# haowenz/chromap

Measured on AMD Instinct MI355X. Metric: M paired reads mapped/s (ATAC preset, GRCh38 index), higher is better.
Workload: dtype u64

## Files before the change

### chromap_amd/csrc/cm_api.hip

```cpp
#include <hip/hip_runtime.h>
#include <math.h>
#include <stdio.h>
#include <stdlib.h>
#include <string.h>

#include <string>
#include <vector>

#include "../../include/chromap_amd.h"
#include "cm_barcode_translate.h"
#include "cm_ctx.h"
#include "cm_kernels.h"
#include "cm_classes.h"
#include "cm_summary.h"
#include "cm_coop.h"
#include <chrono>
#include <mutex>
#include "cm_mapq_tables.h"

static thread_local std::string g_last_error;

static bool cm_debug_pool() { static const bool on = getenv("CM_DEBUG_POOL") != nullptr; return on; }
static thread_local std::string t_last_error;
void cm_set_error(cmgpu_ctx *ctx, const std::string &msg) {
// ... 18 lines not shown
    fprintf(stderr, "[alloc] %10.3f MB (had %10.3f) %8.3f ms\n", (double)want / 1e6, (double)had / 1e6,
            std::chrono::duration<double, std::milli>(std::chrono::steady_clock::now() - t0).count());
  if (e != hipSuccess) {
    (void)hipGetLastError();
    want = bytes;
    e = hipMalloc(&p, want);
    if (e != hipSuccess) { p = nullptr; return -1; }
  }
  cap = want;
  return 0;
}
void DevBuf::release() {
  if (p && owned) (void)hipFree(p);
  p = nullptr;
  cap = 0;
}

static int cm_ensure_candidate_arrays(cmgpu_ctx *c, uint64_t n_m) {
  return c->mbuf.ensure((size_t)n_m * 8 + 8) || c->mcnt.ensure((size_t)n_m + 4) || c->fbuf.ensure((size_t)n_m * 8 + 8) ||
         c->fcnt.ensure((size_t)n_m + 4) || c->dpos.ensure((size_t)n_m * 8 + 8) || c->derr.ensure((size_t)n_m * 2 + 4) ||
         c->dsplit.ensure((size_t)n_m * 4 + 4) || c->v_err.ensure((size_t)n_m * 2 + 4) || c->v_end.ensure((size_t)n_m * 2 + 4);
}
extern "C" int cmgpu_set_option(cmgpu_ctx *c, const char *name, int64_t value) {
  if (!c || !name) return CMGPU_EINVAL;
  const std::string n(name);
  if (n == "probe_lookups_per_lane") {
    if (value != 1 && value != 2 && value != 4 && value != 8) { cm_set_error(c, "probe_lookups_per_lane: 1, 2, 4 or 8"); return CMGPU_EINVAL; }
    c->opt.probe_variant = (int)value | (c->opt.probe_variant & 16);
  } else if (n == "probe_pair_prefetch") {
    c->opt.probe_variant = (c->opt.probe_variant & 15) | (value ? 16 : 0);
  } else if (n == "h2d_copy_blocks") {
    if (value < 0 || value > 4096) { cm_set_error(c, "h2d_copy_blocks: 0..4096"); return CMGPU_EINVAL; }
    c->opt.h2d_kernel = (int)value;
  } else if (n == "d2h_copy_blocks") {
    if (value < 0 || value > 4096) { cm_set_error(c, "d2h_copy_blocks: 0..4096"); return CMGPU_EINVAL; }
    c->opt.d2h_kernel = (int)value;
  } else if (n == "mm_chunks") {
    if (value < 1 || value > CM_MM_CHUNKS) { cm_set_error(c, "mm_chunks: 1.." + std::to_string(CM_MM_CHUNKS)); return CMGPU_EINVAL; }
    c->opt.mm_chunks = (int)value;
  } else if (n == "prep_kernel") {
    c->opt.prep_kernel = (int)value;
  } else if (n == "prep_tile_reads") {
    if (value < 8 || value > 128) { cm_set_error(c, "prep_tile_reads: 8..128"); return CMGPU_EINVAL; }
    c->opt.prep_tile_reads = (int)value;
  } else if (n == "heavy_wave_max" || n == "heavy_block_max" || n == "heavy_big_max") {
    c->opt.heavy_max[n == "heavy_wave_max" ? 0 : n == "heavy_block_max" ? 1 : 2] = (int)value;
  } else if (n == "s3b_lane_cap") {
    if (value < 0 || value > 64) { cm_set_error(c, "s3b_lane_cap: 0 (by read length) or 1..64"); return CMGPU_EINVAL; }
    c->opt.s3b_cap = (int)value;
  } else if (n == "exchange_overlap") {
    c->opt.exchange_overlap = value ? 1 : 0;
  } else if (n == "lanes") {
    if (value < 1 || value > 8) { cm_set_error(c, "lanes: 1..8"); return CMGPU_EINVAL; }
    c->opt.lanes = (int)value;
  } else if (n == "first_read_id") {
    if (value < 0 || value > 0xffffffffll) { cm_set_error(c, "first_read_id: 0..2^32-1"); return CMGPU_EINVAL; }
    c->first_read_id = (uint32_t)value;
  } else if (n == "heavy_mid_max") {
    c->opt.heavy_mid = (int)value;
  } else if (n == "heavy_last") {
    c->opt.heavy_last = (int)value;
  } else if (n == "probe_table_shift") {
    if (value < 0 || value > 4) { cm_set_error(c, "probe_table_shift: 0..4"); return CMGPU_EINVAL; }
    return cm_build_fast_table(c, (int)value);
  } else if (n == "long_read_fused") {
    c->opt.long_fused = value ? 1 : 0;
  } else if (n == "sam_format_group") {
    if (value != 8 && value != 16 && value != 64) { cm_set_error(c, "sam_format_group: 8, 16 or 64"); return CMGPU_EINVAL; }
    c->opt.sam_group = (int)value;
  } else if (n == "verify_planes") {
    c->opt.planes = value ? 1 : 0;
  } else if (n == "speculative_sizes") {
    c->opt.spec = value ? 1 : 0;
    if (value < 0) { c->cls_seen = 0; memset(c->cls_age, 0, sizeof(c->cls_age)); }
  } else if (n == "debug_candidate_capacity") {
    if (value > 0 && cm_ensure_candidate_arrays(c, (uint64_t)value)) { cm_set_error(c, "out of device memory (candidates)"); return CMGPU_ENOMEM; }
    c->pred_m_ok = value > 0; c->m_cap = (uint64_t)value; c->pred_n = 0xffffffffu;
  } else if (n == "coop_profile") {
    if (value) { if (c->coop_prof.ensure(64 * 8)) return CMGPU_ENOMEM; CM_HIPCHECK(c, hipMemset(c->coop_prof.p, 0, 64 * 8)); } else c->coop_prof.release();
  } else if (n == "coop_run_table") {
    c->opt.coop_rb = (int)value;
  } else if (n == "coop") {
    c->opt.coop = (int)value;
  } else if (n == "item_limit") {
    c->opt.item_limit = value > 0 ? (uint64_t)value : 0xfffffff0ull;
  } else {
    cm_set_error(c, "unknown option " + n);
    return CMGPU_EINVAL;
  }
  return CMGPU_OK;
}

extern "C" int cmgpu_get_option(const cmgpu_ctx *c, const char *name, int64_t *value) {
  if (!c || !name || !value) return CMGPU_EINVAL;
  const std::string n(name);
  if (n == "probe_lookups_per_lane") *value = c->opt.probe_variant & 15;
  else if (n == "probe_pair_prefetch") *value = (c->opt.probe_variant & 16) ? 1 : 0;
  else if (n == "mm_chunks") *value = c->opt.mm_chunks;
  else if (n == "h2d_copy_blocks") *value = c->opt.h2d_kernel;
  else if (n == "d2h_copy_blocks") *value = c->opt.d2h_kernel;
  else if (n == "prep_kernel") *value = c->opt.prep_kernel;
  else if (n == "prep_tile_reads") *value = c->opt.prep_tile_reads;
  else if (n == "item_limit") *value = (int64_t)c->opt.item_limit;
  else if (n == "lanes") *value = c->opt.lanes;
  else if (n == "coop") *value = c->opt.coop;
  else if (n.rfind("coop_profile_", 0) == 0) {
    const int k = atoi(n.c_str() + 13);
    unsigned long long v = 0;
    if (k < 0 || k > 63 || !c->coop_prof.p || hipMemcpy(&v, (const unsigned long long *)c->coop_prof.p + k, 8, hipMemcpyDeviceToHost) != hipSuccess) return CMGPU_EINVAL;
    *value = (int64_t)v;
  }
  else if (n == "probe_table_buckets") *value = c->fmask ? (int64_t)c->fmask + 1 : (int64_t)c->bmask + 1;
  else return CMGPU_EINVAL;
  return CMGPU_OK;
}

extern "C" const char *cmgpu_last_error(const cmgpu_ctx *ctx) { return ctx ? ctx->err.c_str() : g_last_error.c_str(); }

__global__ void k_repack(const uint32_t *__restrict__ flags, const uint64_t *__restrict__ keys,
                         const uint64_t *__restrict__ vals, uint64_t *__restrict__ bkt, uint32_t i0, uint32_t n) {
  const uint32_t j = blockIdx.x * 256 + threadIdx.x;
  if (j >= n) return;
  const uint32_t i = i0 + j;
  const uint32_t f = (flags[i >> 4] >> ((i & 0xfU) << 1)) & 3u;
  uint64_t k = keys[j], v = vals[j];
  if (f & 2u) { k = CM_EMPTY_KEY; v = 0; }
  else if (f & 1u) { k = CM_DELETED_KEY; v = 0; }
  bkt[2 * (uint64_t)i] = k;
  bkt[2 * (uint64_t)i + 1] = v;
}

__global__ __launch_bounds__(256) void k_rehash(const uint64_t *__restrict__ src, uint64_t n_src, uint64_t *__restrict__ dst, uint32_t mask) {
  const uint64_t i = (uint64_t)blockIdx.x * 256 + threadIdx.x;
  if (i >= n_src) return;
  const uint64_t key = src[2 * i], val = src[2 * i + 1];
  if (key == CM_EMPTY_KEY || key == CM_DELETED_KEY) return;
  uint32_t b = (uint32_t)(key >> 1) & mask, step = 0;
  for (;;) {
    const unsigned long long old = atomicCAS(reinterpret_cast<unsigned long long *>(dst + 2 * (uint64_t)b), (unsigned long long)CM_EMPTY_KEY, (unsigned long long)key);
    if (old == CM_EMPTY_KEY) { dst[2 * (uint64_t)b + 1] = val; return; }
    b = (b + (++step)) & mask;
  }
}
int cm_build_fast_table(cmgpu_ctx *c, int shift) {
  CM_HIPCHECK(c, cm_enter(c));
  CM_HIPCHECK(c, cm_stream_sync(c->stream));
  if (c->shared_children > (int)c->lanes.size()) { cm_set_error(c, "probe_table_shift: set it before cmgpu_create_shared (contexts that share this index view the table)"); return CMGPU_EINVAL; }
  c->bkt_fast.release();
  c->fmask = 0;
  if (shift <= 0) return CMGPU_OK;
  if (!c->bkt.p || !c->bkt.owned) { cm_set_error(c, "probe_table_shift: set it on the context that owns the index"); return CMGPU_EINVAL; }
  const uint64_t nb = (uint64_t)c->bmask + 1;
  uint64_t nf = nb << shift;
  if (nf > (1ull << 32)) nf = 1ull << 32;
  if (nf <= nb) return CMGPU_OK;
  if (c->bkt_fast.ensure((size_t)nf * 16)) { cm_set_error(c, "out of device memory (re-hashed index table)"); return CMGPU_ENOMEM; }
  CM_HIPCHECK(c, hipMemsetAsync(c->bkt_fast.p, 0xff, (size_t)nf * 16, c->stream));
  hipLaunchKernelGGL(k_rehash, dim3((unsigned)((nb + 255) / 256)), dim3(256), 0, c->stream, (const uint64_t *)c->bkt.p, nb, (uint64_t *)c->bkt_fast.p,
                     (uint32_t)(nf - 1));
  CM_HIPCHECK(c, cm_stream_sync(c->stream));
  c->fmask = (uint32_t)(nf - 1);
  return CMGPU_OK;
}

static int build_mapq_tables(cmgpu_ctx *c) {
  std::vector<double> coef;
  std::vector<uint32_t> brk;
  cm_build_len_coef(coef);
  cm_build_nsec_break(brk);
  c->n_break = (int)brk.size();
  if (c->len_coef.ensure(coef.size() * 8) || c->nsec_break.ensure(brk.size() * 4)) return CMGPU_ENOMEM;
  CM_HIPCHECK(c, hipMemcpy(c->len_coef.p, coef.data(), coef.size() * 8, hipMemcpyHostToDevice));
  CM_HIPCHECK(c, hipMemcpy(c->nsec_break.p, brk.data(), brk.size() * 4, hipMemcpyHostToDevice));
  return CMGPU_OK;
}

static void cm_load_device_code(hipStream_t s);
int cm_ctx_init_common(cmgpu_ctx *c, const cmgpu_params *params, int kmer, int window, int device_id) {
  c->device = device_id;
  c->hp = *params;
  if (params->max_num_best_mappings < 1 || params->max_num_best_mappings > CM_MAX_BEST) {
    cm_set_error(c, "max_num_best_mappings must be in [1, " + std::to_string(CM_MAX_BEST) + "]"); return CMGPU_EINVAL;
  }
  if (params->max_num_best_mappings > 1 && params->output_format == 1) {
    cm_set_error(c, "--SAM with more than one best mapping per read is outside this build"); return CMGPU_EINVAL;
  }
  if (kmer < 1 || kmer > 28 || window < 1 || window > CM_MAX_W_HOST) { cm_set_error(c, "unsupported k/w"); return CMGPU_EINVAL; }
  if (params->error_threshold < 1 || params->error_threshold > 15) { cm_set_error(c, "error_threshold must be 1..15"); return CMGPU_EINVAL; }
// ... 434 lines not shown
  }
  CM_HIPCHECK(c, hipMemcpyAsync(c->rb0.p, in->read1_bases, c->bases0, hipMemcpyHostToDevice, c->stream));
  CM_HIPCHECK(c, hipMemcpyAsync(c->rb1.p, in->read2_bases, c->bases1, hipMemcpyHostToDevice, c->stream));
  CM_HIPCHECK(c, hipMemcpyAsync(c->ro0.p, in->read1_offsets, ((size_t)n + 1) * 4, hipMemcpyHostToDevice, c->stream));
  CM_HIPCHECK(c, hipMemcpyAsync(c->ro1.p, in->read2_offsets, ((size_t)n + 1) * 4, hipMemcpyHostToDevice, c->stream));
  const int rc = launch_max_len(c, c->ro0, &c->ro1, n, c->stream);
  if (rc) return rc;
  CM_HIPCHECK(c, cm_stream_sync(c->stream));
  c->max_read_len = *c->h_maxlen ? *c->h_maxlen : 1;
  return CMGPU_OK;
}

extern "C" int cmgpu_swap_resident_batch(cmgpu_ctx *c, int slot) {
  if (!c || slot < 0 || slot >= CM_BATCH_SLOTS) return CMGPU_EINVAL;
  if (c->in_flight) { cm_set_error(c, "a batch is in flight"); return CMGPU_EINVAL; }
  if (c->has_barcodes || c->single) { cm_set_error(c, "only bulk paired-end batches can be parked"); return CMGPU_EINVAL; }
  CM_HIPCHECK(c, cm_enter(c));
  CM_HIPCHECK(c, cm_stream_sync(c->stream));
  CmBatchSlot &sl = c->slots[slot];
  std::swap(c->rb0, sl.rb0); std::swap(c->rb1, sl.rb1); std::swap(c->ro0, sl.ro0); std::swap(c->ro1, sl.ro1);
  std::swap(c->n_pairs, sl.n_pairs); std::swap(c->first_read_id, sl.first_read_id); std::swap(c->max_read_len, sl.max_read_len);
  std::swap(c->bases0, sl.bases0); std::swap(c->bases1, sl.bases1);
  c->n_records = 0;
  return CMGPU_OK;
}


static void cm_ensure_goff(cmgpu_ctx *c) {
  if (c->goff_tried) return;
  c->goff_tried = true;
  std::vector<uint32_t> go(c->n_seq + 1);
  uint64_t acc = 0;
  const bool lens_ok = c->n_seq && c->h_ref_len.size() == c->n_seq;
  for (uint32_t i = 0; lens_ok && i < c->n_seq; ++i) { go[i] = (uint32_t)acc; acc += (uint64_t)c->h_ref_len[i] + CM_GOFF_GAP; if (acc >= 0xffff0000ull) break; }
  if (lens_ok && acc < 0xffff0000ull && !getenv("CM_NO_KEY32")) {
    go[c->n_seq] = (uint32_t)acc;
    if (c->goff.ensure(go.size() * 4) == 0 && hipMemcpy(c->goff.p, go.data(), go.size() * 4, hipMemcpyHostToDevice) != hipSuccess) c->goff.release();
  }
}
static void cm_set_classes(const cmgpu_ctx *c, CmDev &d) {
  CmClassIn in = {};
  for (int q = 0; q < 3; ++q) in.heavy_max[q] = c->opt.heavy_max[q];
  in.heavy_mid = c->opt.heavy_mid; in.s3b_cap = c->opt.s3b_cap;
  in.max_read_len = c->max_read_len; in.n_seq = c->n_seq; in.has_goff = c->goff.p != nullptr;
  in.lane_cap = cm_s3b_lane_cap(c->max_read_len);
  cm_s3b_heavy_classes(in.hv_max, &in.hv_big);
  cm_size_classes(in, d);
}
static void cm_bind_dev(cmgpu_ctx *c, CmDev &d, uint32_t lo, uint32_t hi) {
  d.bkt = (const uint64_t *)(c->fmask ? c->bkt_fast.p : c->bkt.p); d.bmask = c->fmask ? c->fmask : c->bmask; d.occ = (const uint64_t *)c->occ.p; d.n_occ = c->n_occ;
  d.ref = (const uint8_t *)c->ref.p; d.ref_off = (const uint64_t *)c->ref_off.p; d.ref_len = (const uint32_t *)c->ref_len.p;
  d.goff = (const uint32_t *)c->goff.p; d.n_seq = c->n_seq;
  d.ref_pl = c->ref_pl_words && c->opt.planes ? (const CmPlRec *)c->ref_planes.p + CM_PL_LEAD : nullptr; d.ref_pl_words = c->ref_pl_words;
  d.p = c->p; d.p.single = c->single ? 1 : 0;
  d.mq.len_coef = (const double *)c->len_coef.p; d.mq.nsec_break = (const uint32_t *)c->nsec_break.p; d.mq.n_break = c->n_break;
  d.n_pairs = hi - lo; d.first_read_id = c->first_read_id + lo;
  d.rb0 = (const uint8_t *)c->rb0.p; d.rb1 = (const uint8_t *)c->rb1.p;
  d.ro0 = (const uint32_t *)c->ro0.p + lo; d.ro1 = (const uint32_t *)c->ro1.p + lo;
#define PTR(f, T) d.f = (T *)c->f.p;
  PTR(rlen, uint32_t) PTR(mm_cnt, uint32_t)
  PTR(mm_off, uint32_t) PTR(mm_hash, uint64_t) PTR(mm_ps, uint32_t) PTR(pr_val, uint64_t) PTR(pr_kind, uint8_t)
  PTR(hit_tot, uint32_t) PTR(hit_off, uint32_t) PTR(round2, uint8_t) PTR(rep_cnt, uint32_t) PTR(rep_len, uint32_t)
  PTR(hbuf, uint64_t) PTR(hcnt, uint8_t) PTR(n_pos_hit, uint32_t) PTR(ncp, uint32_t) PTR(ncn, uint32_t)
  PTR(aug, uint8_t) PTR(res_neg, int32_t) PTR(res_pos, int32_t) PTR(resc_n, uint32_t) PTR(resc_p, uint32_t)
  PTR(m_tot, uint32_t) PTR(m_off, uint32_t) PTR(mbuf, uint64_t) PTR(mcnt, uint8_t) PTR(mcp, uint32_t) PTR(mcn, uint32_t)
  PTR(force0, uint8_t) PTR(fbuf, uint64_t) PTR(fcnt, uint8_t) PTR(fcp, uint32_t) PTR(fcn, uint32_t) PTR(alive, uint8_t)
  PTR(dpos, uint64_t) PTR(derr, int16_t) PTR(dsplit, uint32_t) PTR(nv, uint32_t) PTR(v_off, uint32_t) PTR(v_err, int16_t) PTR(v_end, int16_t) PTR(ndp, uint32_t) PTR(ndn, uint32_t)
  PTR(min_err, int32_t) PTR(second_err, int32_t) PTR(n_best, int32_t) PTR(n_second, int32_t)
  PTR(pe_min, int32_t) PTR(pe_second, int32_t) PTR(pe_nbest, int32_t) PTR(pe_nsecond, int32_t)
  PTR(pe_first, uint32_t) PTR(pe_i1, uint32_t) PTR(pe_i2, uint32_t) PTR(pe_choice, uint32_t)
  PTR(stats, unsigned long long) PTR(srt_cnt, uint32_t) PTR(srt_list, uint32_t) PTR(hv_cnt, uint32_t) PTR(hv_list, uint32_t) PTR(rs_cnt, uint32_t) PTR(rs_list, uint32_t)
#undef PTR
  d.rec = (uint8_t *)c->rec.p + (size_t)lo * 24 * cm_rec_per_pair(c);
  d.rec_ok = (uint8_t *)c->rec_ok.p + (size_t)lo * cm_rec_per_pair(c);
  d.hv_stride = 2 * (hi - lo) + 1;
  d.perm_reads = c->use_perm ? (const uint32_t *)c->perm_reads.p : nullptr; d.perm_pairs = c->use_perm ? (const uint32_t *)c->perm_pairs.p : nullptr;
  d.coop_slab = (uint8_t *)c->coop_slab.p; d.coop_slab_cap = CM_SLAB_CAP; d.coop_slab_blocks = CM_SLAB_BLOCKS;
  d.cls_mask = c->cls_all || !c->opt.spec ? ~0ull : c->cls_seen;
  d.prof = (unsigned long long *)c->coop_prof.p;
  d.rs_pool = (uint64_t *)c->rs_pool.p; d.rs_pool_cap = c->rs_pool.p ? c->rs_pool_cap : 0u; d.rs_pool_off = (uint32_t *)c->rs_pool_off.p;
  d.abort = (const unsigned long long *)c->stats.p + CM_ST_ABORT;
  d.coop_rb = c->opt.coop_rb > 0 ? (uint32_t)c->opt.coop_rb : 0u;
  d.wq_dynamic = ((uint32_t)c->opt.coop >> 16) & 1u;
  if (c->has_rank) {
    d.rid_rank = (const uint32_t *)c->rid_rank.p;
    d.ref_off = (const uint64_t *)c->ref_off_r.p;
    d.ref_len = (const uint32_t *)c->ref_len_r.p;
  }
  if (c->has_pairs_rank) d.pairs_rank = (const uint32_t *)c->pairs_rank.p;
  if (c->has_barcodes) {
    d.bcb = (const uint8_t *)c->bcb.p; d.bcq = (const uint8_t *)c->bcq.p; d.bco = (const uint32_t *)c->bco.p + lo;
    d.wl = (const uint64_t *)c->wl.p; d.wl_mask = c->wl_mask; d.wl_num_sample = (double)c->wl_num_sample;
    d.pow10_tab = (const double *)c->pow10_tab.p;
    d.bc_key = c->bc_key.p ? (uint64_t *)c->bc_key.p + lo : nullptr; d.bc_ok = c->bc_ok.p ? (uint8_t *)c->bc_ok.p + lo : nullptr;
  }
}
static inline void mark(cmgpu_ctx *c, const char *name) {
  if (c->n_ev < CM_MAX_EVENTS) {
    (void)hipEventRecord(c->ev[c->n_ev], c->stream);
    c->ev_name[c->n_ev] = name;
    ++c->n_ev;
  }
}
static int scan_with_total(cmgpu_ctx *c, const uint32_t *in, uint32_t *out, uint32_t n, unsigned long long *total, bool wait = true) {
  hipStream_t s = c->stream;
  unsigned long long *acc = (unsigned long long *)c->stats.p + CM_ST_TOTAL;
  CM_HIPCHECK(c, hipMemsetAsync(acc, 0, 8, s));
  cm_launch_k_sum_u32(in, n, acc, s);
  cm_scan_u32(in, out, n, (uint32_t *)c->scan_tmp.p, s);
  CM_HIPCHECK(c, hipMemcpyAsync(total, acc, 8, hipMemcpyDeviceToHost, s));
  if (wait) CM_HIPCHECK(c, cm_stream_sync(s));
  return CMGPU_OK;
}
#define CM_RC_SPLIT (-100)
#define CM_RC_AGAIN_ALL_CLASSES (-101)
#define CM_RC_AGAIN_EXACT_SIZES (-102)
struct RangeRun {
  cmgpu_ctx *c;
  uint32_t rlo, rhi, n, n2;
  bool allow_spec;
  uint64_t limit;
  hipStream_t s;
  CmDev d;
  uint32_t n_mm = 0;
  bool s3a_done = false;
  uint32_t n_heavy[CM_HV_LISTS] = {};
  unsigned long long hits_total = 0;
  uint32_t n_hits = 0;
  bool planes = false;
  bool spec = false;
  uint32_t n_m = 0;
  void bind() { cm_bind_dev(c, d, rlo, rhi); }
};
static int stage_begin(RangeRun &r) {
  cmgpu_ctx *c = r.c;
  c->n_ev = 0;
  c->use_perm = false;
  const int rc = ensure_pair_arrays(c, r.n);
  if (rc) return rc;
  CM_HIPCHECK(c, hipMemsetAsync(c->stats.p, 0, CM_ST_N * 8, r.s));
  memset(&r.d, 0, sizeof(r.d));
  cm_ensure_goff(c);
  cm_set_classes(c, r.d);
  r.bind();
  mark(c, "begin");
  if (c->has_barcodes) {
    cm_launch_k_s0b_barcode(r.d, r.n, r.s);
    mark(c, "s0b_barcode");
  }
  return CMGPU_OK;
}
struct MmChunks {
  uint32_t n_chunks;
  uint32_t lo[CM_MM_CHUNKS + 1];
  uint64_t entries[CM_MM_CHUNKS];
  uint32_t part_off[CM_MM_CHUNKS + 1];
};
static uint32_t mm_chunk_count(const RangeRun &r) { return r.n >= (1u << 20) ? (uint32_t)r.c->opt.mm_chunks : (r.n >= (1u << 17) ? 2 : 1); }
static void mm_probe_grids(const cmgpu_ctx *c, MmChunks &k) {
  k.part_off[0] = 0;
  for (uint32_t ch = 0; ch < k.n_chunks; ++ch) k.part_off[ch + 1] = k.part_off[ch] + cm_probe_range_blocks(k.entries[ch], c->opt.probe_variant);
}
template <class Fill>
static int mm_fill_and_probe(RangeRun &r, const MmChunks &k, uint32_t mm_cap, Fill fill) {
  cmgpu_ctx *c = r.c;
  const unsigned long long *marks = (const unsigned long long *)c->mm_marks.p;
// ... 1146 lines not shown
```

### chromap_amd/csrc/cm_ctx.h

```cpp
#ifndef CM_CTX_H_
#define CM_CTX_H_
#include <hip/hip_runtime.h>

#include <string>
#include <thread>
#include <vector>

#include "../../include/chromap_amd.h"
#include "../../include/chromap_amd_debug.h"
#include "cm_types.h"

#define CM_MAX_EVENTS 32
#define CM_MAX_W_HOST 32

struct DevBuf {
  void *p = nullptr;
  size_t cap = 0;
  bool owned = true;
  int ensure(size_t bytes);
  void release();
};

struct CmTmpBuf : private DevBuf {
  using DevBuf::p;
// ... 17 lines not shown
  DevBuf scan_tmp;
  hipStream_t hs = nullptr;
  DevBuf red_tmp;
  DevBuf text2, comp, btab, toks, ntok;
  bool dev_mode = false;
  uint64_t dev_len = 0;
  uint64_t n_bytes = 0;
  uint32_t n_nl = 0, n_raw = 0, n_rec = 0, taken = 0, taken_bases = 0, taken_max_len = 0;
  bool final_chunk = false;
  int n_ranges = 0;
  int rng_start[4] = {0, 0, 0, 0}, rng_end[4] = {-1, -1, -1, -1};
  bool minus = false;
  bool keep_names = false;
  DevBuf nm_len, nm_off, st_nm;
  uint32_t taken_name_bytes = 0;
  bool keep_reads = false;
  DevBuf st_q;
  int layout = 0;
  bool general = false;
  uint32_t fx_seen = 0;
  uint32_t fx_lines = 0, fx_stop = 0;
  DevBuf fx_li, fx_nxt, fx_send, fx_sl, fx_exit, fx_entry, fx_res;
};

struct CmReadMate {
  DevBuf names, name_offs, bases, quals, offs;
  uint64_t name_bytes = 0, base_bytes = 0;
};
struct CmSamStore {
  DevBuf rec, var, var_offs, bc;
  DevBuf vlen, voff, scan_tmp, flags;
  uint64_t n = 0, var_bytes = 0;
  bool has_bc = false, paired = false;
};

struct CmSummary {
  bool on = false;
  DevBuf keys, first, cnt, meta;
  uint32_t cap = 0;
  uint64_t key_bound = 0;
  uint32_t slot0 = ~0u;
};

struct CmExchange {
  int transport = 0;
  int rank = 0, world = 0;
  void *comm = nullptr;
  cmgpu_exchange_transport ext = {};
  std::vector<uint8_t> h_owner;
  DevBuf owner, send, counts , stage;
  unsigned long long *h_matrix = nullptr;
  hipStream_t stream = nullptr;
  hipEvent_t ev_part = nullptr, ev_payload = nullptr;
  bool payload_pending = false;
  uint64_t sent_total = 0, recv_total = 0, steps = 0;
  uint64_t owned_by[64] = {};
};

#define CM_BATCH_SLOTS 8
struct CmBatchSlot {
  DevBuf rb0, rb1, ro0, ro1;
  uint32_t n_pairs = 0, first_read_id = 0, max_read_len = 1;
  size_t bases0 = 0, bases1 = 0;
};

struct CmOptions {
  int long_fused = 1;
  int planes = 1;
  int sam_group = 8;
  int d2h_kernel = 0;
  int h2d_kernel = 0;
  int probe_variant = 1;
  int mm_chunks = CM_MM_CHUNKS;
  int prep_tile_reads = 32;
  int prep_kernel = 0;
  uint64_t item_limit = 0xfffffff0ull;
  int exchange_overlap = 0;
  int s3b_cap = 0;
  int lanes = 1;
  int heavy_mid = 0;
  int heavy_max[3] = {0, 0, 0};
  int heavy_last = 0;
  int spec = 1;
  int coop_rb = 0;
  int coop = 0xff;
};

struct cmgpu_ctx {
  CmOptions opt;
  int device = 0;
  hipStream_t stream = nullptr;
  hipStream_t stream2 = nullptr;
  hipStream_t stream_pack = nullptr;
  hipEvent_t chunk_ev[CM_MM_CHUNKS + 1] = {};
  std::string err;
  cmgpu_params hp;
  CmParams p;
  DevBuf bkt, occ, ref, ref_off, ref_len, len_coef, nsec_break;
  uint32_t bmask = 0, n_occ = 0, n_seq = 0;
  DevBuf bkt_fast, coop_prof;
  uint32_t fmask = 0;
  DevBuf ref_planes, read_planes;
  DevBuf mm_stage;
  uint64_t ref_pl_words = 0;
  int n_break = 0;
  uint64_t ref_bytes = 0;
  std::vector<uint64_t> h_ref_off;
  std::vector<uint32_t> h_ref_len;
  uint32_t n_pairs = 0, first_read_id = 0;
  size_t bases0 = 0, bases1 = 0;
  uint32_t max_read_len = 1;
  DevBuf rb0, rb1, ro0, ro1;
  DevBuf st_rb0, st_rb1, st_ro0, st_ro1, st_bcb, st_bcq, st_bco;
  DevBuf rlen, scratch_a, scratch_b , mm_cnt, mm_off, mm_hash, mm_ps, pr_val, pr_kind;
  DevBuf hit_tot, hit_off, round2, rep_cnt, rep_len, hbuf, hcnt, n_pos_hit, ncp, ncn;
  DevBuf aug, res_neg, res_pos, resc_n, resc_p, m_tot, m_off, mbuf, mcnt, mcp, mcn, force0;
  DevBuf fbuf, fcnt, fcp, fcn, alive, dpos, derr, dsplit, nv, v_off, v_err, v_end, ndp, ndn, min_err, second_err, n_best, n_second;
  DevBuf pe_min, pe_second, pe_nbest, pe_nsecond, pe_first, pe_i1, pe_i2, pe_choice, rec, rec_ok;
  DevBuf scan_tmp, stats, partials;
  DevBuf wl, pow10_tab, bcb, bcq, bco, bc_key, bc_ok, wl_num;
  uint32_t wl_mask = 0, wl_size = 0, bc_len = 0;
  uint64_t wl_num_sample = 0;
  bool skip_barcode_check = false;
  bool has_barcodes = false;
  DevBuf bt_tab, bt_blob;
  uint32_t bt_mask = 0, bt_entries = 0, bt_from = 0;
  uint64_t bt_blob_bytes = 0;
  bool single = false;
  DevBuf store, store_bc, text;
  uint64_t store_n = 0, store_cap = 0, text_bytes = 0, text_lines = 0;
  bool store_has_bc = false;
  bool store_pairs_rec = false;
  CmFqStream fq[3];
  DevBuf nm_blob, nm_offs;
  uint64_t nm_n = 0, nm_bytes = 0, nm_cap_n = 0;
  uint32_t nm_base = 0;
  CmReadMate rd[2];
  uint64_t rd_n = 0;
  uint32_t rd_base = 0;
  bool rd_paired = false;
  CmSamStore ss;
  DevBuf sam_rec, sam_cigar, sam_md, sam_z;
  DevBuf pairs_rank;
  bool has_pairs_rank = false;
  DevBuf rid_rank, ref_off_r, ref_len_r;
  bool has_rank = false;
  DevBuf mm_cursor;
  DevBuf mm_marks;
  DevBuf part_cnt;
  unsigned long long cls_seen = ~0ull;
  uint8_t cls_age[64] = {};
  bool cls_all = false;
  DevBuf rs_pool, rs_pool_off;
  DevBuf goff;
  bool goff_tried = false;
  uint32_t rs_pool_cap = 0;
  uint64_t rs_pool_want = 0;
  DevBuf coop_slab, hv_cnt, hv_list, perm_reads, perm_pairs, hv_tmp, srt_cnt, srt_list, rs_list, rs_cnt;
  bool use_perm = false;
  CmSummary sm;
  CmExchange ex;
  bool batch_exchanged = false;
  CmBatchSlot slots[CM_BATCH_SLOTS];
  hipStream_t stream_h2d = nullptr;
  hipEvent_t ev_h2d[2] = {nullptr, nullptr};
  uint32_t sub_total = 0, sub_count = 0;
// ... 102 lines not shown
```

### chromap_amd/csrc/cm_kernels.hip

```cpp
#include <hip/hip_runtime.h>
#include <stdio.h>
#include <string.h>
#include <cstring>
#include <atomic>
#include <map>
#include <mutex>
#include <utility>
#include <rocprim/rocprim.hpp>

#include "cm_kernels.h"
#include "cm_stages.h"
#include "cm_coop.h"

#define CM_BLOCK 256

#define CM_ITEM_KERNEL(kname, fn, perm)                                      \
  __global__ __launch_bounds__(CM_BLOCK) void kname(CmDev d, uint32_t n) {   \
    if (d.abort && *d.abort) return;                                         \
    const uint32_t i = blockIdx.x * CM_BLOCK + threadIdx.x;                  \
    if (i < n) fn(d, d.perm ? d.perm[i] : i);                                \
  }



// ... 551 lines not shown
    __syncthreads();
    return mx;
  }
  __device__ __forceinline__ uint64_t min64(uint64_t v) { return ~max64(~v); }
  __device__ __forceinline__ uint32_t sum(uint32_t v) { uint32_t tot; (void)scan(v, &tot); return tot; }
};
#define CM_XW_BYTES 256
__host__ __device__ inline size_t cm_coop_group_bytes(uint32_t P, uint32_t MM, uint32_t RB, bool own_oc, bool key32 = false) { return ((cm_coop_mem_bytes(P, MM, RB, own_oc, key32) + 15) & ~(size_t)15) + CM_XW_BYTES; }

template <int G, bool K32>
__global__ __launch_bounds__(G < CM_BLOCK ? CM_BLOCK : G, CM_WPE_S3B) void k_s3b_coop(CmDev d, const uint32_t *__restrict__ list, uint32_t n_list, uint32_t P, uint32_t MM, uint32_t RB,
                                                                      uint32_t *__restrict__ fb_list, uint32_t *__restrict__ fb_cnt, uint32_t use_slab) {
  const uint32_t gpb = blockDim.x / G, grp = threadIdx.x / G;
  const size_t gb = cm_coop_group_bytes(P, MM, RB, false, K32);
  uint8_t *base = cm_lds + (size_t)grp * gb;
  CmCoopMem m = cm_coop_mem_at(base, P, MM, RB, false, K32);
  if (use_slab) cm_coop_slab_at(m, d.coop_slab + (size_t)blockIdx.x * cm_coop_slab_bytes(d.coop_slab_cap), d.coop_slab_cap);
  CmDevGroup<G> g;
  g.t = threadIdx.x % G;
  g.xw = reinterpret_cast<uint32_t *>(base + gb - CM_XW_BYTES);
  for (uint32_t gid = blockIdx.x * gpb + grp; gid < n_list; gid += gridDim.x * gpb) {
    const uint32_t r = list[gid];
    bool done;
    if constexpr (K32) done = cm_coop_s3b_k32(d, r, g, m);
    else done = use_slab ? cm_coop_s3b<true>(d, r, g, m) : cm_coop_s3b<false>(d, r, g, m);
    if (!done && g.t == 0) fb_list[atomicAdd(fb_cnt, 1u)] = r;
    g.sync();
  }
}

__global__ __launch_bounds__(64) void k_s3b_serial(CmDev d, const uint32_t *__restrict__ list, uint32_t n_list, const uint32_t *__restrict__ n_list_dev) {
  if (n_list_dev) n_list = *n_list_dev;
  for (uint32_t i = blockIdx.x * 64 + threadIdx.x; i < n_list; i += gridDim.x * 64) cm_s3b_candidates(d, list[i]);
}

__device__ __forceinline__ void cm_wave_append(uint32_t *__restrict__ list, uint32_t *__restrict__ counter, bool pred, uint32_t value) {
  const unsigned long long m = __ballot(pred);
  if (m == 0) return;
  const uint32_t lane = threadIdx.x & 63u, leader = (uint32_t)(__ffsll((long long)m) - 1);
  uint32_t base = 0;
  if (lane == leader) base = atomicAdd(counter, (uint32_t)__popcll(m));
  base = __shfl(base, (int)leader, 64);
  if (pred) list[base + (uint32_t)__popcll(m & ((1ull << lane) - 1ull))] = value;
}

#define CM_WQ_CHUNK 4u
enum { CM_WQ_S4A_SMALL = 32, CM_WQ_S4A_BIG, CM_WQ_S4B_SMALL, CM_WQ_S4B_BIG, CM_WQ_S5_SORT_SMALL, CM_WQ_S5_SORT_WAVE, CM_WQ_S5_SORT_BLOCK };
struct CmWaveQueue {
  uint32_t *cur;
  uint32_t cnt, j, jend, stride;
  __device__ __forceinline__ CmWaveQueue(uint32_t *cursor, uint32_t n, uint32_t dynamic = 0) : cur(cursor), cnt(n), j(0), jend(0), stride(0) {
    if (!dynamic) {
      const uint32_t wpb = blockDim.x >> 6;
      stride = gridDim.x * wpb;
      j = blockIdx.x * wpb + (threadIdx.x >> 6);
      jend = 0xffffffffu;
    }
  }
  __device__ __forceinline__ bool next(uint32_t *item) {
    if (stride) {
      if (j >= cnt) return false;
      *item = j;
      j += stride;
      return true;
    }
    if (j == jend) {
      uint32_t b = 0;
      if ((threadIdx.x & 63u) == 0) b = atomicAdd(cur, CM_WQ_CHUNK);
      b = __shfl(b, 0, 64);
      if (b >= cnt) return false;
      j = b;
      jend = b + CM_WQ_CHUNK < cnt ? b + CM_WQ_CHUNK : cnt;
    }
    *item = j++;
    return true;
  }
};

#define CM_RS_WAVE 4u
__device__ __forceinline__ bool cm_rescue_is_wave(const CmDev &d, uint32_t r, uint32_t coop) {
  const uint32_t o = r ^ 1u;
  return coop && (d.ncp[o] >= CM_RS_WAVE || d.ncn[o] >= CM_RS_WAVE);
}
__global__ __launch_bounds__(CM_BLOCK) void k_s4a_rescue_count(CmDev d, uint32_t n, uint32_t seg_cap, uint32_t coop) {
  __shared__ uint32_t sh_cnt, sh_base;
  if (threadIdx.x == 0) sh_cnt = 0;
  __syncthreads();
  const uint32_t i0 = blockIdx.x * CM_BLOCK + threadIdx.x;
  const uint32_t i = i0 < n && d.perm_reads ? d.perm_reads[i0] : i0;
  const bool aug0 = i0 < n && cm_s4a_decide(d, i);
  const bool wv = aug0 && cm_rescue_is_wave(d, i, coop);
  cm_wave_append(d.hv_list + (size_t)CM_L_SEARCH_WAVE * d.hv_stride, d.hv_cnt + CM_L_SEARCH_WAVE, wv, i);
  const bool aug = aug0 && !wv;
  const unsigned long long m = __ballot(aug);
  const uint32_t lane = threadIdx.x & 63u;
  uint32_t wbase = 0;
  if (m) {
    const uint32_t leader = (uint32_t)(__ffsll((long long)m) - 1);
    if (lane == leader) wbase = atomicAdd(&sh_cnt, (uint32_t)__popcll(m));
    wbase = __shfl(wbase, (int)leader, 64);
  }
  __syncthreads();
  const uint32_t seg = blockIdx.x % CM_RS_SEGS;
  if (threadIdx.x == 0 && sh_cnt) sh_base = atomicAdd(&d.rs_cnt[seg * 16], sh_cnt);
  __syncthreads();
  if (aug) d.rs_list[(uint64_t)seg * seg_cap + sh_base + wbase + (uint32_t)__popcll(m & ((1ull << lane) - 1ull))] = i;
}
#define CM_RS_HEAVY 8u
#define CM_RS_G 16
#define CM_RS_MAXMM 192
__device__ __forceinline__ bool cm_rescue_is_heavy(const CmDev &d, uint32_t r, uint32_t coop) {
  const uint32_t o = r ^ 1u;
  return (d.ncp[o] >= CM_RS_HEAVY || d.ncn[o] >= CM_RS_HEAVY) && d.mm_cnt[r] <= CM_RS_MAXMM && !cm_rescue_is_wave(d, r, coop);
}
__device__ __forceinline__ void cm_group_best(const uint8_t *mc, uint32_t mn, uint32_t t, int *max_count, int *best_num) {
  int lmax = 0, lnum = 0;
  for (uint32_t i = t; i < mn; i += CM_RS_G) {
    const int c = mc[i];
    if (c > lmax) { lmax = c; lnum = 1; } else if (c == lmax) ++lnum;
  }
  for (int off = CM_RS_G / 2; off > 0; off >>= 1) {
    const int om = __shfl_xor(lmax, off, CM_RS_G), on = __shfl_xor(lnum, off, CM_RS_G);
    if (om > lmax) { lmax = om; lnum = on; } else if (om == lmax) lnum += on;
  }
  *max_count = lmax;
  *best_num = lnum;
}
__device__ __forceinline__ int cm_group_rescue_count(const CmDev &d, uint32_t r, int strand, const uint64_t *mp, const uint8_t *mc, uint32_t mn,
                                                     uint32_t t, uint32_t *cnt, uint32_t *rl) {
  int max_count, best_num;
  cm_group_best(mc, mn, t, &max_count, &best_num);
  *cnt = 0;
  if (cm_rescue_bails(d, max_count, best_num, mn)) {
    if (d.prof && t == 0) atomicAdd(&d.prof[26], 1ull);
    return -max_count;
  }
  const uint32_t b = d.mm_off[r], n = d.mm_cnt[r];
  if (d.prof && t == 0) {
    unsigned long long so = 0;
    for (uint32_t mi = 0; mi < n; ++mi) if (d.pr_kind[b + mi] == CM_PR_MULTI) so += (uint32_t)d.pr_val[b + mi];
    atomicAdd(&d.prof[16], 1ull); atomicAdd(&d.prof[17], (unsigned long long)best_num); atomicAdd(&d.prof[18], (unsigned long long)mn);
    atomicAdd(&d.prof[19], so); atomicAdd(&d.prof[20], (unsigned long long)n);
    atomicAdd(&d.prof[best_num < 4 ? 22 : best_num < 16 ? 23 : best_num < 64 ? 24 : 25], 1ull);
  }
  uint32_t lc = 0;
  for (uint32_t mi = t; mi < n; mi += CM_RS_G)
    lc += cm_rescue_minimizer(d, strand, mp, mc, mn, max_count, d.pr_kind[b + mi], d.pr_val[b + mi], d.mm_ps[b + mi], nullptr, nullptr);
  for (int off = CM_RS_G / 2; off > 0; off >>= 1) lc += __shfl_xor(lc, off, CM_RS_G);
  uint32_t rep_len = 0;
  if (t == 0) {
    uint32_t prev_rep = ~0u;
    for (uint32_t mi = 0; mi < n; ++mi) cm_rescue_rep(d, d.pr_kind[b + mi], d.pr_val[b + mi], d.mm_ps[b + mi], &rep_len, &prev_rep);
  }
  *rl = __shfl(rep_len, 0, CM_RS_G);
  *cnt = lc;
  if (d.prof && t == 0) atomicAdd(&d.prof[21], (unsigned long long)lc);
  return max_count;
}
__global__ __launch_bounds__(64) void k_s4a_rescue_list(CmDev d, uint32_t seg_cap, uint32_t coop) {
  const uint32_t cnt = d.rs_cnt[blockIdx.y * 16];
  const uint32_t *list = d.rs_list + (uint64_t)blockIdx.y * seg_cap;
  const long long t1 = d.prof ? clock64() : 0;
  for (uint32_t j = blockIdx.x * 64 + threadIdx.x; j < cnt; j += gridDim.x * 64) {
    const uint32_t r = list[j];
    if (!cm_rescue_is_heavy(d, r, coop)) cm_s4a_rescue(d, r);
  }
  const long long t2 = d.prof ? clock64() : 0;
  if (d.prof && threadIdx.x == 0) { const unsigned long long dt = (unsigned long long)(t2 - t1); atomicAdd(&d.prof[29], dt); atomicMax(&d.prof[30], dt); }
  const uint32_t t = threadIdx.x % CM_RS_G, grp = threadIdx.x / CM_RS_G, gpb = 64 / CM_RS_G;
  for (uint32_t j = blockIdx.x * gpb + grp; j < cnt; j += gridDim.x * gpb) {
    const uint32_t r = list[j];
    if (!cm_rescue_is_heavy(d, r, coop)) continue;
    const uint32_t o = r ^ 1u;
// ... 106 lines not shown
  __shared__ __attribute__((aligned(16))) uint8_t rmem[SMALL ? CM_RESCUE_MEM_BYTES_S : CM_RESCUE_MEM_BYTES];
  const uint32_t li = SMALL ? CM_L_SEARCH_WAVE : CM_L_SEARCH_WAVE_BIG;
  const uint32_t cnt = d.hv_cnt[li];
  if (blockIdx.x >= cnt) return;
  const uint32_t *list = d.hv_list + (size_t)li * d.hv_stride;
  const CmCoopRescueMem m = SMALL ? cm_coop_rescue_mem_at(rmem, CM_RESCUE_WMAX_S, CM_RESCUE_PAIRS_S) : cm_coop_rescue_mem_at(rmem);
  CmDevGroup<64> g;
  g.t = threadIdx.x;
  g.xw = nullptr;
  cm_coop_rescue_mem_reset(g, m);
  const long long t0 = d.prof ? clock64() : 0;
  CmWaveQueue wq(d.hv_cnt + (SMALL ? CM_WQ_S4A_SMALL : CM_WQ_S4A_BIG), cnt, d.wq_dynamic);
  for (uint32_t j; wq.next(&j);) {
    const uint32_t r = list[j];
    if (SMALL && d.prof) {
      const uint32_t o = r ^ 1u;
      const uint32_t a = cm_coop_rescue_best_num(g, cm_c0_pcnt(d, o), d.ncp[o]), b = cm_coop_rescue_best_num(g, cm_c0_ncnt(d, o), d.ncn[o]);
      const uint32_t mx = a > b ? a : b;
      if (threadIdx.x == 0) atomicAdd(&d.prof[mx < 16 ? 40 : mx < 32 ? 41 : mx < 64 ? 42 : mx < 128 ? 43 : mx < 200 ? 44 : mx < 300 ? 45 : 46], 1ull);
    }
    if (SMALL && !cm_coop_rescue_fits(d, r, g, CM_RESCUE_WMAX_S)) {
      if (threadIdx.x == 0) d.hv_list[(size_t)CM_L_SEARCH_WAVE_BIG * d.hv_stride + atomicAdd(d.hv_cnt + CM_L_SEARCH_WAVE_BIG, 1u)] = r;
      continue;
    }
    const long long ti = d.prof ? clock64() : 0;
    cm_coop_s4a_rescue(d, r, g, m);
    g.sync();
    if (d.prof && threadIdx.x == 0) atomicMax(&d.prof[22], (unsigned long long)(clock64() - ti));
  }
  cm_coop_rescue_mem_flush(d, g, m);
  if (d.prof && threadIdx.x == 0) { const unsigned long long dt = (unsigned long long)(clock64() - t0); atomicAdd(&d.prof[27], dt); atomicMax(&d.prof[28], dt); }
}
template <bool SMALL>
__global__ __launch_bounds__(64) void k_s4b_rescue_wave(CmDev d, uint32_t coop) {
  if (d.abort && *d.abort) return;
  __shared__ __attribute__((aligned(16))) uint8_t rmem[SMALL ? CM_RESCUE_MEM_BYTES_S : CM_RESCUE_MEM_BYTES];
  const uint32_t li = SMALL ? CM_L_SEARCH_WAVE : CM_L_SEARCH_WAVE_BIG;
  const uint32_t cnt = d.hv_cnt[li];
  if (blockIdx.x >= cnt) return;
  const uint32_t *list = d.hv_list + (size_t)li * d.hv_stride;
  const CmCoopRescueMem m = SMALL ? cm_coop_rescue_mem_at(rmem, CM_RESCUE_WMAX_S, CM_RESCUE_PAIRS_S) : cm_coop_rescue_mem_at(rmem);
  CmDevGroup<64> g;
  g.t = threadIdx.x;
  g.xw = nullptr;
  const long long t0 = d.prof ? clock64() : 0;
  CmWaveQueue wq(d.hv_cnt + (SMALL ? CM_WQ_S4B_SMALL : CM_WQ_S4B_BIG), cnt, d.wq_dynamic);
  for (uint32_t j; wq.next(&j);) {
    const uint32_t r = list[j];
    if (d.resc_n[r] + d.resc_p[r] == 0) continue;
    if (SMALL && !cm_coop_rescue_fits(d, r, g, CM_RESCUE_WMAX_S)) continue;
    cm_coop_s4b_fill(d, r, g, m);
    g.sync();
    const uint32_t cls = cm_rescue_coop_class(d, r, coop);
    if (threadIdx.x == 0) {
      if (cls) d.hv_list[(size_t)cls * d.hv_stride + atomicAdd(d.hv_cnt + cls, 1u)] = r;
      else cm_s4b_rescue_merge(d, r, CM_S4B_PREFILLED);
    }
  }
  if (d.prof && threadIdx.x == 0) { const unsigned long long dt = (unsigned long long)(clock64() - t0); atomicAdd(&d.prof[32], dt); atomicMax(&d.prof[33], dt); }
}
template <int G>
__global__ __launch_bounds__(G < CM_BLOCK ? CM_BLOCK : G) void k_s4b_coop(CmDev d, const uint32_t *__restrict__ list, const uint32_t *__restrict__ n_list_dev, uint32_t P, uint32_t RB,
                                                                      uint32_t use_slab) {
  if (d.abort && *d.abort) return;
  const uint32_t gpb = blockDim.x / G, grp = threadIdx.x / G;
  const uint32_t n_list = *n_list_dev;
  const size_t gb = cm_coop_group_bytes(P, 1, RB, true);
  uint8_t *base = cm_lds + (size_t)grp * gb;
  CmCoopMem m = cm_coop_mem_at(base, P, 1, RB, true);
  if (use_slab) cm_coop_slab_at(m, d.coop_slab + (size_t)blockIdx.x * cm_coop_slab_bytes(d.coop_slab_cap), d.coop_slab_cap);
  CmDevGroup<G> g;
  g.t = threadIdx.x % G;
  g.xw = reinterpret_cast<uint32_t *>(base + gb - CM_XW_BYTES);
  for (uint32_t gid = blockIdx.x * gpb + grp; gid < n_list; gid += gridDim.x * gpb) {
    if (use_slab) cm_coop_rescue_merge<true>(d, list[gid], g, m); else cm_coop_rescue_merge<false>(d, list[gid], g, m);
    g.sync();
  }
}
#define CM_S4C_COOP_MIN 48u
#define CM_S5C_COOP_MIN 48u
#define CM_S5C_P_SMALL 512u
#define CM_S5C_P_WAVE 2048u
#define CM_S5C_P_BLOCK 16384u
__device__ __forceinline__ void cm_s4c_queue_sort(const CmDev &d, uint32_t pair, bool live, uint32_t coop) {
  for (uint32_t q = 0; q < 4; ++q) {
    const uint32_t r = 2 * pair + (q >> 1);
    uint32_t cnt = live ? ((q & 1u) ? d.fcn[r] : d.fcp[r]) : 0u;
    if ((coop & 8u) && !d.p.split && live && d.fcp[r] + d.fcn[r] > CM_S5C_COOP_MIN) cnt = 0;
    cm_wave_append(d.srt_list, &d.srt_cnt[0], cnt > CM_SORT_SERIAL_MAX && cnt <= CM_SORT_WAVE_MAX, (r << 1) | (q & 1u));
  }
}
#define CM_S4C_P_SMALL 256u
#define CM_S4C_P_WAVE 1024u
#define CM_S4C_P_BLOCK 4096u
#define CM_S4C_P_BIG 15360u
__global__ __launch_bounds__(CM_BLOCK) void k_s4c_reduce(CmDev d, uint32_t n, uint32_t coop) {
  if (d.abort && *d.abort) return;
  const uint32_t i = blockIdx.x * CM_BLOCK + threadIdx.x;
  const uint32_t pair = i < n ? (d.perm_pairs ? d.perm_pairs[i] : i) : 0u;
  uint32_t cls = 0;
  if (i < n && cm_s4c_pre(d, pair)) {
    const uint32_t r1 = 2 * pair, r2 = r1 + 1;
    uint32_t big = d.mcp[r1] > d.mcn[r1] ? d.mcp[r1] : d.mcn[r1];
    big = d.mcp[r2] > big ? d.mcp[r2] : big;
    big = d.mcn[r2] > big ? d.mcn[r2] : big;
    if ((coop & 4u) && big > CM_S4C_COOP_MIN) cls = big <= CM_S4C_P_SMALL ? CM_L_PF_WAVE : big <= CM_S4C_P_WAVE ? CM_L_PF_BLOCK : big <= CM_S4C_P_BLOCK ? CM_L_PF_BLOCK_BIG : big <= d.s4c_pbig ? CM_L_PF_HUGE : 0u;
    if (!cls) { cm_s4c_filter(d, pair); cm_s4c_post(d, pair); }
  }
  if (coop & 4u) {
    cm_wave_append(d.hv_list + CM_L_PF_BLOCK * (size_t)d.hv_stride, d.hv_cnt + CM_L_PF_BLOCK, cls == CM_L_PF_BLOCK, pair);
    cm_wave_append(d.hv_list + CM_L_PF_WAVE * (size_t)d.hv_stride, d.hv_cnt + CM_L_PF_WAVE, cls == CM_L_PF_WAVE, pair);
    cm_wave_append(d.hv_list + CM_L_PF_BLOCK_BIG * (size_t)d.hv_stride, d.hv_cnt + CM_L_PF_BLOCK_BIG, cls == CM_L_PF_BLOCK_BIG, pair);
    cm_wave_append(d.hv_list + CM_L_PF_HUGE * (size_t)d.hv_stride, d.hv_cnt + CM_L_PF_HUGE, cls == CM_L_PF_HUGE, pair);
  }
  if (!d.perm_pairs) return;
  cm_s4c_queue_sort(d, pair, i < n && !cls && d.alive[pair], coop);
}
template <int G, bool STAGED>
__global__ __launch_bounds__(G < CM_BLOCK ? CM_BLOCK : G) void k_s4c_coop(CmDev d, uint32_t P, uint32_t lid, uint32_t coop) {
  if (d.abort && *d.abort) return;
  const uint32_t gpb = blockDim.x / G, grp = threadIdx.x / G;
  const uint32_t n_list = d.hv_cnt[lid];
  const uint32_t *list = d.hv_list + (size_t)lid * d.hv_stride;
  const size_t gb = ((cm_coop_pair_mem_bytes(P, STAGED) + 15) & ~(size_t)15) + CM_XW_BYTES;
  uint8_t *base = cm_lds + (size_t)grp * gb;
  const CmCoopPairMem m = cm_coop_pair_mem_at(base, P, STAGED);
  CmDevGroup<G> g;
  g.t = threadIdx.x % G;
  g.xw = reinterpret_cast<uint32_t *>(base + gb - CM_XW_BYTES);
  for (uint32_t j0 = blockIdx.x * gpb; j0 < n_list; j0 += gridDim.x * gpb) {
    const uint32_t j = j0 + grp;
    const uint32_t pair = j < n_list ? list[j] : 0u;
    if (j < n_list) cm_coop_s4c<STAGED>(d, pair, g, m);
    g.sync();
    if (d.perm_pairs) {
      const bool live = j < n_list && d.alive[pair];
      for (uint32_t q = 0; q < 4; ++q) {
        const uint32_t r = 2 * pair + (q >> 1);
        uint32_t cnt = live ? ((q & 1u) ? d.fcn[r] : d.fcp[r]) : 0u;
        if ((coop & 8u) && live && d.fcp[r] + d.fcn[r] > CM_S5C_COOP_MIN) cnt = 0;
        if (g.t == 0 && cnt > CM_SORT_SERIAL_MAX && cnt <= CM_SORT_WAVE_MAX) d.srt_list[atomicAdd(&d.srt_cnt[0], 1u)] = (r << 1) | (q & 1u);
      }
    }
  }
}
__global__ __launch_bounds__(CM_BLOCK) void k_s5a_prepare(CmDev d, uint32_t n, uint32_t coop) {
  if (d.abort && *d.abort) return;
  const uint32_t i = blockIdx.x * CM_BLOCK + threadIdx.x;
  const uint32_t r = i < n ? (d.perm_reads ? d.perm_reads[i] : i) : 0u;
  const bool to_wave = i < n && cm_s5a_prepare(d, r, coop ? CM_S5C_COOP_MIN : 0u);
  const bool big = to_wave && (d.fcp[r] > CM_S5C_P_WAVE || d.fcn[r] > CM_S5C_P_WAVE);
  const bool small = to_wave && d.fcp[r] <= CM_S5C_P_SMALL && d.fcn[r] <= CM_S5C_P_SMALL;
  if (coop) {
    cm_wave_append(d.hv_list + (size_t)CM_L_S5_SMALL * d.hv_stride, d.hv_cnt + CM_L_S5_SMALL, small, r);
    cm_wave_append(d.hv_list + (size_t)CM_L_S5_WAVE * d.hv_stride, d.hv_cnt + CM_L_S5_WAVE, to_wave && !big && !small, r);
    cm_wave_append(d.hv_list + (size_t)CM_L_S5_BLOCK * d.hv_stride, d.hv_cnt + CM_L_S5_BLOCK, big, r);
  }
}
__global__ __launch_bounds__(CM_BLOCK) void k_s5c_finalize(CmDev d, uint32_t n, uint32_t coop) {
  if (d.abort && *d.abort) return;
  const uint32_t i = blockIdx.x * CM_BLOCK + threadIdx.x;
  const uint32_t r = i < n ? (d.perm_reads ? d.perm_reads[i] : i) : 0u;
  const uint32_t cmin = coop ? CM_S5C_COOP_MIN : 0u;
  if (i < n) cm_s5c_finalize(d, r, cmin);
  if (!d.perm_reads || d.p.split || d.p.single) return;
  const bool live = i < n && !(cmin && d.nv[r] > cmin) && d.alive[r >> 1];
  const uint32_t a = live ? d.ndp[r] : 0u, b = live ? d.ndn[r] : 0u;
  cm_wave_append(d.srt_list, &d.srt_cnt[0], a > CM_SORT_SERIAL_MAX && a <= CM_SORT_WAVE_MAX, r << 1);
  cm_wave_append(d.srt_list, &d.srt_cnt[0], b > CM_SORT_SERIAL_MAX && b <= CM_SORT_WAVE_MAX, (r << 1) | 1u);
}
#define CM_SORT_NB 64u
#define CM_SORT_STAGE 512u
__global__ __launch_bounds__(CM_BLOCK, 8) void k_s5_sort_coop(CmDev d, uint32_t lid) {
  if (d.abort && *d.abort) return;
  __shared__ uint64_t stage_p[(CM_BLOCK / 64) * CM_SORT_STAGE];
  __shared__ uint8_t stage_c[(CM_BLOCK / 64) * CM_SORT_STAGE];
  const uint32_t grp = threadIdx.x / 64;
  const uint32_t n_list = d.hv_cnt[lid];
  const uint32_t *list = d.hv_list + (size_t)lid * d.hv_stride;
  CmDevGroup<64> g;
  g.t = threadIdx.x % 64;
  g.xw = nullptr;
  const long long t0 = d.prof ? clock64() : 0;
  uint32_t mine = 0;
  CmWaveQueue wq(d.hv_cnt + (lid == CM_L_S5_SMALL ? CM_WQ_S5_SORT_SMALL : lid == CM_L_S5_WAVE ? CM_WQ_S5_SORT_WAVE : CM_WQ_S5_SORT_BLOCK), n_list, d.wq_dynamic);
  for (uint32_t j; wq.next(&j); ++mine)
    cm_coop_s5_sort(d, list[j], g, nullptr, CM_SORT_NB, stage_p + (size_t)grp * CM_SORT_STAGE, stage_c + (size_t)grp * CM_SORT_STAGE, CM_SORT_STAGE);
  if (d.prof && g.t == 0 && mine) {
    const unsigned long long dt = (unsigned long long)(clock64() - t0);
    atomicAdd(&d.prof[38], dt); atomicMax(&d.prof[39], dt); atomicAdd(&d.prof[6], (unsigned long long)mine);
  }
}
#define CM_S5C_SORT_P 1024u
#define CM_S5C_SORT_RB 130u
template <int G>
__global__ __launch_bounds__(CM_BLOCK) void k_s5c_coop(CmDev d, uint32_t P, uint32_t lid) {
  if (d.abort && *d.abort) return;
  const uint32_t gpb = blockDim.x / G, grp = threadIdx.x / G;
  const uint32_t n_list = d.hv_cnt[lid];
  const uint32_t *list = d.hv_list + (size_t)lid * d.hv_stride;
  const size_t b1 = cm_coop_ver_mem_bytes(P), b2 = cm_coop_sort_mem_bytes(CM_S5C_SORT_P, CM_S5C_SORT_RB);
  const size_t gb = (((b1 > b2 ? b1 : b2) + 15) & ~(size_t)15) + CM_XW_BYTES;
  uint8_t *base = cm_lds + (size_t)grp * gb;
  const CmCoopVerMem m = cm_coop_ver_mem_at(base, P);
  const CmCoopSortMem sm = cm_coop_sort_mem_at(base, CM_S5C_SORT_P, CM_S5C_SORT_RB);
  CmDevGroup<G> g;
  g.t = threadIdx.x % G;
  g.xw = reinterpret_cast<uint32_t *>(base + gb - CM_XW_BYTES);
  for (uint32_t j = blockIdx.x * gpb + grp; j < n_list; j += gridDim.x * gpb) {
    cm_coop_s5c(d, list[j], g, m, sm);
    g.sync();
  }
}

template <int MODE>
__global__ __launch_bounds__(CM_BLOCK) void k_sort_lists(CmDev d) {
  if (d.abort && *d.abort) return;
  const uint32_t wv = threadIdx.x >> 6, t = threadIdx.x & 63;
  uint64_t *K = reinterpret_cast<uint64_t *>(cm_lds) + (size_t)wv * CM_SORT_WAVE_MAX;
  uint16_t *V = reinterpret_cast<uint16_t *>(cm_lds + (size_t)(CM_BLOCK / 64) * CM_SORT_WAVE_MAX * 8) + (size_t)wv * CM_SORT_WAVE_MAX;
  const uint32_t n_items = d.srt_cnt[0];
  for (;;) {
    uint32_t item = 0;
    if (t == 0) item = atomicAdd(&d.srt_cnt[1], 1u);
    item = __shfl(item, 0, 64);
    if (item >= n_items) return;
    const uint32_t code = d.srt_list[item], r = code >> 1, strand = code & 1u;
    const uint32_t base = d.m_off[r] + (strand ? d.ncp[r] + d.resc_p[r] : 0);
    const uint32_t n = MODE == 0 ? (strand ? d.fcn[r] : d.fcp[r]) : (strand ? d.ndn[r] : d.ndp[r]);
    uint64_t *gk = (MODE == 0 ? d.fbuf : d.dpos) + base;
    uint32_t P2 = 2;
    while (P2 < n) P2 <<= 1;
    for (uint32_t i = t; i < P2; i += 64) {
      if (i < n) {
        K[i] = gk[i];
        V[i] = MODE == 0 ? (uint16_t)(255u - d.fcnt[base + i]) : (uint16_t)d.derr[base + i];
      } else {
        K[i] = ~0ull;
        V[i] = 0xffffu;
      }
    }
    cm_group_sync<64>();
    for (uint32_t k2 = 2; k2 <= P2; k2 <<= 1) {
      for (uint32_t j = k2 >> 1, lj = 31u - (uint32_t)__clz(k2 >> 1); j > 0; j >>= 1, --lj) {
        for (uint32_t i = t; i < (P2 >> 1); i += 64) {
          const uint32_t a = ((i >> lj) << (lj + 1)) | (i & (j - 1)), c = a + j;
          const uint64_t xa = K[a], xc = K[c];
          const uint16_t va = V[a], vc = V[c];
          const bool gt = MODE == 0 ? (va != vc ? va > vc : xa > xc) : (xa != xc ? xa > xc : va > vc);
          const bool up = (a & k2) == 0;
          if (gt == up && (xa != xc || va != vc)) { K[a] = xc; K[c] = xa; V[a] = vc; V[c] = va; }
        }
        cm_group_sync<64>();
      }
    }
    for (uint32_t i = t; i < n; i += 64) {
      gk[i] = K[i];
      if (MODE == 0) d.fcnt[base + i] = (uint8_t)(255u - V[i]); else d.derr[base + i] = (int16_t)V[i];
    }
    cm_group_sync<64>();
  }
}
void cm_launch_k_sort_lists(const CmDev &d, int mode, hipStream_t s) {
  const size_t lds = (size_t)(CM_BLOCK / 64) * CM_SORT_WAVE_MAX * 10;
  if (mode == 0) hipLaunchKernelGGL(k_sort_lists<0>, dim3(1024), dim3(CM_BLOCK), lds, s, d);
  else hipLaunchKernelGGL(k_sort_lists<1>, dim3(1024), dim3(CM_BLOCK), lds, s, d);
}
__global__ __launch_bounds__(CM_BLOCK) void k_s5b_verify(CmDev d, uint32_t n_reads) {
  if (d.abort && *d.abort) return;
  const uint32_t n_items = d.v_off[n_reads];
  for (uint32_t j = blockIdx.x * CM_BLOCK + threadIdx.x; j < n_items; j += gridDim.x * CM_BLOCK) cm_s5b_verify_item(d, j, n_reads);
}
#define CM_S6A_COOP_MIN 48u
#define CM_S6A_P_SMALL 256u
#define CM_S6A_P_WAVE 1024u
#define CM_S6A_P_BLOCK 8192u
__device__ __forceinline__ uint32_t cm_s6_class(const CmDev &d, uint32_t pair, uint32_t small_list, uint32_t wave_list, uint32_t block_list) {
  const uint32_t r1 = 2 * pair, r2 = r1 + 1;
  uint32_t big2 = d.ndp[r2] > d.ndn[r2] ? d.ndp[r2] : d.ndn[r2], big = big2;
  big = d.ndp[r1] > big ? d.ndp[r1] : big;
  big = d.ndn[r1] > big ? d.ndn[r1] : big;
  if (big <= CM_S6A_COOP_MIN) return 0;
  return big2 <= CM_S6A_P_SMALL ? small_list : big2 <= CM_S6A_P_WAVE ? wave_list : block_list;
}
__global__ __launch_bounds__(CM_BLOCK) void k_s6a_pair(CmDev d, uint32_t n, uint32_t coop) {
  if (d.abort && *d.abort) return;
  const uint32_t i = blockIdx.x * CM_BLOCK + threadIdx.x;
  const uint32_t pair = i < n ? (d.perm_pairs ? d.perm_pairs[i] : i) : 0u;
  uint32_t cls = 0;
  if (i < n && cm_s6a_pre<false>(d, pair)) {
    cls = coop ? cm_s6_class(d, pair, CM_L_S6A_SMALL, CM_L_S6A_WAVE, CM_L_S6A_BLOCK) : 0u;
    if (!cls) cm_s6a_sweeps<false>(d, pair);
  }
  if (coop) {
    cm_wave_append(d.hv_list + (size_t)CM_L_S6A_SMALL * d.hv_stride, d.hv_cnt + CM_L_S6A_SMALL, cls == CM_L_S6A_SMALL, pair);
    cm_wave_append(d.hv_list + (size_t)CM_L_S6A_WAVE * d.hv_stride, d.hv_cnt + CM_L_S6A_WAVE, cls == CM_L_S6A_WAVE, pair);
    cm_wave_append(d.hv_list + (size_t)CM_L_S6A_BLOCK * d.hv_stride, d.hv_cnt + CM_L_S6A_BLOCK, cls == CM_L_S6A_BLOCK, pair);
  }
}
template <int G>
__global__ __launch_bounds__(CM_BLOCK, 6) void k_s6a_coop(CmDev d, uint32_t P, uint32_t lid) {
  if (d.abort && *d.abort) return;
  const uint32_t gpb = blockDim.x / G, grp = threadIdx.x / G;
  const uint32_t n_list = d.hv_cnt[lid];
  const uint32_t *list = d.hv_list + (size_t)lid * d.hv_stride;
  const size_t gb = ((cm_coop_pe_mem_bytes(P) + 15) & ~(size_t)15) + CM_XW_BYTES;
  uint8_t *base = cm_lds + (size_t)grp * gb;
  const CmCoopPeMem m = cm_coop_pe_mem_at(base, P);
  CmDevGroup<G> g;
  g.t = threadIdx.x % G;
  g.xw = reinterpret_cast<uint32_t *>(base + gb - CM_XW_BYTES);
  for (uint32_t j = blockIdx.x * gpb + grp; j < n_list; j += gridDim.x * gpb) cm_coop_s6a<false>(d, list[j], g, m);
}
__global__ __launch_bounds__(CM_BLOCK) void k_s6c_multi(CmDev d, uint32_t n, uint32_t coop) {
  if (d.abort && *d.abort) return;
  const uint32_t i = blockIdx.x * CM_BLOCK + threadIdx.x;
  const uint32_t pair = i < n ? (d.perm_pairs ? d.perm_pairs[i] : i) : 0u;
  uint32_t cls = 0;
  if (i < n) {
    if (coop && !d.p.single && !d.p.split && d.pe_nbest[pair] > 1) cls = cm_s6_class(d, pair, CM_L_S6C_SMALL, CM_L_S6C_WAVE, CM_L_S6C_BLOCK);
    if (!cls) cm_s6c_multi<false>(d, pair);
  }
  if (coop) {
    cm_wave_append(d.hv_list + (size_t)CM_L_S6C_SMALL * d.hv_stride, d.hv_cnt + CM_L_S6C_SMALL, cls == CM_L_S6C_SMALL, pair);
    cm_wave_append(d.hv_list + (size_t)CM_L_S6C_WAVE * d.hv_stride, d.hv_cnt + CM_L_S6C_WAVE, cls == CM_L_S6C_WAVE, pair);
    cm_wave_append(d.hv_list + (size_t)CM_L_S6C_BLOCK * d.hv_stride, d.hv_cnt + CM_L_S6C_BLOCK, cls == CM_L_S6C_BLOCK, pair);
  }
}
template <int G>
__global__ __launch_bounds__(CM_BLOCK) void k_s6c_coop(CmDev d, uint32_t P, uint32_t lid) {
  if (d.abort && *d.abort) return;
  const uint32_t gpb = blockDim.x / G, grp = threadIdx.x / G;
  const uint32_t n_list = d.hv_cnt[lid];
  const uint32_t *list = d.hv_list + (size_t)lid * d.hv_stride;
  const size_t gb = ((cm_coop_pe_mem_bytes(P) + 15) & ~(size_t)15) + CM_XW_BYTES;
  uint8_t *base = cm_lds + (size_t)grp * gb;
  const CmCoopPeMem m = cm_coop_pe_mem_at(base, P);
  CmDevGroup<G> g;
  g.t = threadIdx.x % G;
  g.xw = reinterpret_cast<uint32_t *>(base + gb - CM_XW_BYTES);
  for (uint32_t j = blockIdx.x * gpb + grp; j < n_list; j += gridDim.x * gpb) cm_coop_s6c<false>(d, list[j], g, m);
}
CM_ITEM_KERNEL(k_s6a_pair_sam, cm_s6a_pair<true>, perm_pairs)
CM_ITEM_KERNEL(k_s6c_multi_sam, cm_s6c_multi<true>, perm_pairs)

__global__ __launch_bounds__(64) void k_s6b_sample(CmDev d, uint32_t n_chunks) {
  if (d.abort && *d.abort) return;
  const uint32_t chunk = blockIdx.x;
  if (chunk >= n_chunks) return;
  __shared__ CmMt g;
  uint32_t lo, hi;
  cm_chunk_range(d.n_pairs, (uint32_t)d.p.ref_batch, (uint32_t)d.p.grain, chunk, &lo, &hi);
  bool seeded = false;
  for (uint32_t base = lo; base < hi; base += 64) {
    const uint32_t pair = base + threadIdx.x;
    int nb = 0;
    if (pair < hi) nb = d.pe_nbest[pair];
    const bool multi = nb > 1 && (d.p.single || nb <= d.p.drop_rep);
    unsigned long long m = __ballot(multi);
    if (m == 0) continue;
    if (threadIdx.x == 0) {
      while (m) {
        if (!seeded || d.p.single) { cm_mt_seed(g, 11); seeded = true; }
        const int l = __ffsll((long long)m) - 1;
        m &= m - 1;
        const uint32_t pr = base + (uint32_t)l;
        cm_reservoir(d, pr, d.pe_nbest[pr], g);
      }
    }
    seeded = __shfl((int)seeded, 0, 64) != 0;
  }
}

__global__ __launch_bounds__(CM_BLOCK) void k_s0b_barcode(CmDev d, uint32_t n) {
  const uint32_t i = blockIdx.x * CM_BLOCK + threadIdx.x;
  uint32_t a = 0, b = 0;
  if (i < n) cm_s0b_barcode(d, i, &a, &b);
  for (int off = 32; off > 0; off >>= 1) {
    a += __shfl_down(a, off, 64);
    b += __shfl_down(b, off, 64);
  }
  __shared__ uint32_t sa[CM_BLOCK / 64], sb[CM_BLOCK / 64];
  if ((threadIdx.x & 63) == 0) { sa[threadIdx.x >> 6] = a; sb[threadIdx.x >> 6] = b; }
  __syncthreads();
  if (threadIdx.x == 0) {
    for (int j = 1; j < CM_BLOCK / 64; ++j) { a += sa[j]; b += sb[j]; }
    if (a) atomicAdd(&d.stats[CM_ST_BC_INWL], (unsigned long long)a);
    if (b) atomicAdd(&d.stats[CM_ST_BC_CORR], (unsigned long long)b);
  }
}

__global__ __launch_bounds__(CM_BLOCK) void k_bc_abundance(const uint8_t *__restrict__ bcb, const uint32_t *__restrict__ bco,
                                                            uint32_t lo, uint32_t hi, uint64_t *__restrict__ wl,
                                                            uint32_t wl_mask, unsigned long long *__restrict__ num_sample) {
  const uint32_t i = lo + blockIdx.x * CM_BLOCK + threadIdx.x;
  uint32_t hit = 0;
  if (i < hi) {
    const uint8_t *s = bcb + bco[i];
    const uint32_t l = bco[i + 1] - bco[i];
    bool has_n = false;
    for (uint32_t j = 0; j < l; ++j) has_n |= s[j] == 'N';
    if (!has_n) {
      const uint64_t key = cm_seed_from_sequence(s, l);
      const uint64_t x = key * 0x9E3779B97F4A7C15ull;
      uint32_t b = (uint32_t)(x >> 32) & wl_mask;
      for (;;) {
        const uint64_t k = wl[2 * (uint64_t)b];
        if (k == ~0ull) break;
        if (k == key) { atomicAdd(reinterpret_cast<unsigned long long *>(wl + 2 * (uint64_t)b + 1), 1ull); hit = 1; break; }
// ... 358 lines not shown
#define CM_S3B_OPTIN(G_, LDS_) (k32 ? cm_lds_optin(&k_s3b_coop<G_, true>, LDS_) : cm_lds_optin(&k_s3b_coop<G_, false>, LDS_))
    if (n_cls[CM_L_HIT_WAVE]) {
      const size_t lds = 2 * cm_coop_group_bytes(d.hv_max[0], MM, RB, false, k32);
      if (CM_S3B_OPTIN(64, lds)) {
        CM_S3B_LAUNCH(64, dim3((n_cls[CM_L_HIT_WAVE] + 1) / 2), dim3(128), lds, d, lst(CM_L_HIT_WAVE), n_cls[CM_L_HIT_WAVE], d.hv_max[0], MM, RB, fb_list, fb_cnt, 0u);
        rest[CM_L_HIT_WAVE] = 0; any_coop = true;
      }
    }
    if (n_cls[CM_L_HIT_WAVE_SMALL] && d.hv_sub) {
      const size_t lds = 4 * cm_coop_group_bytes(d.hv_sub, MM, RB, false, k32);
      if (CM_S3B_OPTIN(64, lds)) {
        CM_S3B_LAUNCH(64, dim3((n_cls[CM_L_HIT_WAVE_SMALL] + 3) / 4), dim3(256), lds, d, lst(CM_L_HIT_WAVE_SMALL), n_cls[CM_L_HIT_WAVE_SMALL], d.hv_sub, MM, RB, fb_list, fb_cnt, 0u);
        rest[CM_L_HIT_WAVE_SMALL] = 0; any_coop = true;
      }
    }
#define CM_S3B_COOP_CLASS(C_, Q_, G_)                                                                                                              \
    if (n_cls[C_] && d.hv_max[Q_] > d.hv_max[Q_ - 1]) {                                                                                            \
      const size_t lds = cm_coop_group_bytes(d.hv_max[Q_], MM, RB, false, k32);                                                                    \
      if (CM_S3B_OPTIN(G_, lds)) {                                                                                                                 \
        CM_S3B_LAUNCH(G_, dim3(n_cls[C_]), dim3(G_), lds, d, lst(C_), n_cls[C_], d.hv_max[Q_], MM, RB, fb_list, fb_cnt, 0u);                      \
        rest[C_] = 0; any_coop = true;                                                                                                             \
      }                                                                                                                                            \
    }
    CM_S3B_COOP_CLASS(CM_L_HIT_B256A, 1, 256)
    CM_S3B_COOP_CLASS(CM_L_HIT_B256B, 2, 256)
    CM_S3B_COOP_CLASS(CM_L_HIT_B512, 3, 512)
#undef CM_S3B_COOP_CLASS
    if (n_cls[CM_L_HIT_B1024] && d.hv_big > d.hv_max[3]) {
      const size_t lds = cm_coop_group_bytes(d.hv_big, MM, RB, false, k32);
      if (CM_S3B_OPTIN(1024, lds)) {
        CM_S3B_LAUNCH(1024, dim3(n_cls[CM_L_HIT_B1024]), dim3(1024), lds, d, lst(CM_L_HIT_B1024), n_cls[CM_L_HIT_B1024], d.hv_big, MM, RB, fb_list, fb_cnt, 0u);
        rest[CM_L_HIT_B1024] = 0; any_coop = true;
      }
    }
    if (n_cls[CM_L_HIT_SLAB] && d.coop_slab && d.hv_max[3]) {
      const size_t lds = cm_coop_group_bytes(d.hv_max[3], MM, RB, false);
      if (cm_lds_optin(&k_s3b_coop<1024, false>, lds)) {
        const uint32_t blocks = n_cls[CM_L_HIT_SLAB] < d.coop_slab_blocks ? n_cls[CM_L_HIT_SLAB] : d.coop_slab_blocks;
        uint32_t *sl = d.hv_list + CM_L_HIT_SERIAL * (size_t)d.hv_stride, *sc = d.hv_cnt + CM_L_HIT_SERIAL;
        hipLaunchKernelGGL((k_s3b_coop<1024, false>), dim3(blocks), dim3(1024), lds, s, d, lst(CM_L_HIT_SLAB), n_cls[CM_L_HIT_SLAB], d.hv_max[3], MM, RB, sl, sc, 1u);
        hipLaunchKernelGGL(k_s3b_serial, dim3(64), dim3(64), 0, s, d, (const uint32_t *)sl, 0u, (const uint32_t *)sc);
        rest[CM_L_HIT_SLAB] = 0;
      }
    }
    if (any_coop) {
      const uint32_t P = pow2(d.hv_big > d.hv_max[3] ? d.hv_big : d.hv_max[3]);
      hipLaunchKernelGGL(k_s3b_heavy<CM_BLOCK>, dim3(512), dim3(CM_BLOCK), (size_t)P * 10 + (CM_BLOCK + 8) * 4, s, d, (const uint32_t *)fb_list, 0u, P, (const uint32_t *)fb_cnt);
    }
  }
  if (rest[CM_L_HIT_WAVE_SMALL]) {
    const uint32_t P = pow2(d.hv_max[0]), gpb = CM_BLOCK / 64;
    hipLaunchKernelGGL(k_s3b_heavy<64>, dim3((rest[CM_L_HIT_WAVE_SMALL] + gpb - 1) / gpb), dim3(CM_BLOCK), (size_t)gpb * P * 10 + gpb * (64 + 8) * 4, s, d, lst(CM_L_HIT_WAVE_SMALL), rest[CM_L_HIT_WAVE_SMALL], P, (const uint32_t *)nullptr);
  }
  if (rest[CM_L_HIT_WAVE]) {
    const uint32_t P = pow2(d.hv_max[0]), gpb = CM_BLOCK / 64;
    hipLaunchKernelGGL(k_s3b_heavy<64>, dim3((rest[CM_L_HIT_WAVE] + gpb - 1) / gpb), dim3(CM_BLOCK), (size_t)gpb * P * 10 + gpb * (64 + 8) * 4, s, d, lst(CM_L_HIT_WAVE), rest[CM_L_HIT_WAVE], P, (const uint32_t *)nullptr);
  }
  const uint32_t blk[3][2] = {{1, 1}, {2, 2}, {10, 3}};
  for (int q = 0; q < 3; ++q) {
    const uint32_t c = blk[q][0];
    if (!rest[c]) continue;
    const uint32_t P = pow2(d.hv_max[blk[q][1]]);
    hipLaunchKernelGGL(k_s3b_heavy<CM_BLOCK>, dim3(rest[c]), dim3(CM_BLOCK), (size_t)P * 10 + (CM_BLOCK + 8) * 4, s, d, lst(c), rest[c], P, (const uint32_t *)nullptr);
  }
  if (rest[CM_L_HIT_B1024]) {
    const uint32_t P = pow2(d.hv_big);
    hipLaunchKernelGGL(k_s3b_heavy<CM_BLOCK>, dim3(rest[CM_L_HIT_B1024]), dim3(CM_BLOCK), (size_t)P * 10 + (CM_BLOCK + 8) * 4, s, d, lst(CM_L_HIT_B1024), rest[CM_L_HIT_B1024], P, (const uint32_t *)nullptr);
  }
  if (rest[CM_L_HIT_SLAB]) hipLaunchKernelGGL(k_s3b_serial, dim3((rest[CM_L_HIT_SLAB] + 63) / 64), dim3(64), 0, s, d, lst(CM_L_HIT_SLAB), rest[CM_L_HIT_SLAB], (const uint32_t *)nullptr);
  if (rest[CM_L_HIT_G16]) {
    const uint32_t P = pow2(d.hv_mid), gpb = CM_BLOCK / 16;
    hipLaunchKernelGGL(k_s3b_heavy<16>, dim3((rest[CM_L_HIT_G16] + gpb - 1) / gpb), dim3(CM_BLOCK), (size_t)gpb * P * 10 + gpb * (16 + 8) * 4, s, d, lst(CM_L_HIT_G16), rest[CM_L_HIT_G16], P, (const uint32_t *)nullptr);
  }
}
void cm_launch_k_s3b_candidates(const CmDev &d, uint32_t n, uint32_t max_read_len, hipStream_t s) {
  if (!n) return;
  const uint32_t cap = d.s3b_cap;
  (void)max_read_len;
  uint32_t threads = 256;
  while (threads > 64 && (size_t)cap * threads * 9 > 36 * 1024 + 1024) threads >>= 1;
  hipLaunchKernelGGL(k_s3b_candidates, dim3((n + threads - 1) / threads), dim3(threads), (size_t)cap * threads * 9, s, d, n, cap);
}
uint32_t cm_rescue_seg_cap(uint32_t n_reads) { return ((n_reads + CM_BLOCK - 1) / CM_BLOCK / CM_RS_SEGS + 1) * CM_BLOCK; }
void cm_launch_k_s4a_rescue_count(const CmDev &d, uint32_t n, hipStream_t s, bool coop) {
  if (n) hipLaunchKernelGGL(k_s4a_rescue_count, grid_for(n), dim3(CM_BLOCK), 0, s, d, n, cm_rescue_seg_cap(n), coop ? 1u : 0u);
}
static inline uint32_t rescue_wave_blocks(uint32_t n_reads) {
  uint32_t b = n_reads / 512 + 64;
  return b > 8192u ? 8192u : b;
}
static inline dim3 rescue_list_grid(uint32_t n_reads) {
  uint32_t b = n_reads / 64 / CM_RS_SEGS / 4 + 1;
  if (b > 256u) b = 256u;
  return dim3(b, CM_RS_SEGS);
}
void cm_launch_k_s4a_rescue_list(const CmDev &d, uint32_t n_reads, hipStream_t s, bool coop) {
  if (!n_reads) return;
  hipLaunchKernelGGL(k_s4a_rescue_list, rescue_list_grid(n_reads), dim3(64), 0, s, d, cm_rescue_seg_cap(n_reads), coop ? 1u : 0u);
  if ((coop) && cm_cls_on(d, CM_L_SEARCH_WAVE)) {
    hipLaunchKernelGGL(k_s4a_rescue_wave<true>, dim3(rescue_wave_blocks(n_reads)), dim3(64), 0, s, d);
    hipLaunchKernelGGL(k_s4a_rescue_wave<false>, dim3(rescue_wave_blocks(n_reads)), dim3(64), 0, s, d);
  }
}
static bool cm_s4b_coop_ready(const CmDev &d, uint32_t RB, size_t *lds) {
  if (!d.hv_max[0]) return false;
  lds[0] = 2 * cm_coop_group_bytes(d.hv_max[0], 1, RB, true);
  lds[1] = cm_coop_group_bytes(d.hv_max[1], 1, RB, true);
  lds[2] = cm_coop_group_bytes(d.hv_max[2], 1, RB, true);
  lds[3] = cm_coop_group_bytes(d.rs_max3, 1, RB, true);
  lds[4] = cm_coop_group_bytes(d.rs_big > d.rs_max3 ? d.rs_big : d.rs_max3, 1, RB, true);
  const bool ok = cm_lds_optin(&k_s4b_coop<64>, lds[0]) && cm_lds_optin(&k_s4b_coop<256>, lds[1] > lds[2] ? lds[1] : lds[2]) && cm_lds_optin(&k_s4b_coop<512>, lds[3]) &&
                  cm_lds_optin(&k_s4b_coop<1024>, lds[4]);
  if (!ok) {
    static std::atomic<int> told{0};
    if (!told.exchange(1)) fprintf(stderr, "chromap_amd: the cooperative rescue kernels do not fit this device's shared memory (%zu / %zu / %zu / %zu bytes); using the one-lane forms\n", lds[0], lds[1], lds[2], lds[4]);
  }
  return ok;
}
static inline uint32_t cm_s4b_rb(const CmDev &d, uint32_t max_read_len) {
  return d.coop_rb ? d.coop_rb : 2 * cm_coop_mm(d, max_read_len) + 2;
}
void cm_launch_k_s4b_rescue_merge(const CmDev &d, uint32_t n, hipStream_t s, bool coop, uint32_t max_read_len) {
  if (!n) return;
  size_t lds[5];
  const bool all = coop && cm_s4b_coop_ready(d, cm_s4b_rb(d, max_read_len), lds);
  hipLaunchKernelGGL(k_s4b_rescue_merge, grid_for(n), dim3(CM_BLOCK), 0, s, d, n, all ? 1u : 0u);
}
void cm_launch_k_s4b_rescue_list(const CmDev &d, uint32_t n_reads, hipStream_t s, bool coop, uint32_t max_read_len) {
  if (!n_reads) return;
  const uint32_t RB = cm_s4b_rb(d, max_read_len);
  size_t lds[5];
  const bool all = coop && cm_s4b_coop_ready(d, RB, lds);
  hipLaunchKernelGGL(k_s4b_rescue_list, rescue_list_grid(n_reads), dim3(64), 0, s, d, cm_rescue_seg_cap(n_reads), all ? 1u : 0u);
  if ((coop) && cm_cls_on(d, CM_L_SEARCH_WAVE)) {
    hipLaunchKernelGGL(k_s4b_rescue_wave<true>, dim3(rescue_wave_blocks(n_reads)), dim3(64), 0, s, d, all ? 1u : 0u);
    hipLaunchKernelGGL(k_s4b_rescue_wave<false>, dim3(rescue_wave_blocks(n_reads)), dim3(64), 0, s, d, all ? 1u : 0u);
  }
  if (!all) return;
  uint32_t blocks = n_reads / 2048 + 64;
  if (blocks > 2048) blocks = 2048;
  auto lst = [&](uint32_t c) { return (const uint32_t *)(d.hv_list + (size_t)c * d.hv_stride); };
  if (cm_cls_on(d, CM_L_RS_WAVE)) hipLaunchKernelGGL(k_s4b_coop<64>, dim3(blocks), dim3(128), lds[0], s, d, lst(CM_L_RS_WAVE), (const uint32_t *)(d.hv_cnt + CM_L_RS_WAVE), d.hv_max[0], RB, 0u);
  if ((d.hv_max[1] > d.hv_max[0]) && cm_cls_on(d, CM_L_RS_B256A)) hipLaunchKernelGGL(k_s4b_coop<256>, dim3(blocks), dim3(256), lds[1], s, d, lst(CM_L_RS_B256A), (const uint32_t *)(d.hv_cnt + CM_L_RS_B256A), d.hv_max[1], RB, 0u);
  if ((d.hv_max[2] > d.hv_max[1]) && cm_cls_on(d, CM_L_RS_B256B)) hipLaunchKernelGGL(k_s4b_coop<256>, dim3(blocks), dim3(256), lds[2], s, d, lst(CM_L_RS_B256B), (const uint32_t *)(d.hv_cnt + CM_L_RS_B256B), d.hv_max[2], RB, 0u);
  if ((d.rs_max3 > d.hv_max[2]) && cm_cls_on(d, CM_L_RS_B512)) hipLaunchKernelGGL(k_s4b_coop<512>, dim3(blocks > 512 ? 512 : blocks), dim3(512), lds[3], s, d, lst(CM_L_RS_B512), (const uint32_t *)(d.hv_cnt + CM_L_RS_B512), d.rs_max3, RB, 0u);
  if ((d.rs_big > d.rs_max3) && cm_cls_on(d, CM_L_RS_B1024)) hipLaunchKernelGGL(k_s4b_coop<1024>, dim3(blocks > 256 ? 256 : blocks), dim3(1024), lds[4], s, d, lst(CM_L_RS_B1024), (const uint32_t *)(d.hv_cnt + CM_L_RS_B1024), d.rs_big, RB, 0u);
  if (d.coop_slab && cm_cls_on(d, CM_L_RS_SLAB))
    hipLaunchKernelGGL(k_s4b_coop<1024>, dim3(d.coop_slab_blocks), dim3(1024), lds[4], s, d, lst(CM_L_RS_SLAB), (const uint32_t *)(d.hv_cnt + CM_L_RS_SLAB), d.rs_big > d.rs_max3 ? d.rs_big : d.rs_max3, RB, 1u);
}
void cm_launch_k_s4c_reduce(const CmDev &d, uint32_t n, hipStream_t s, uint32_t coop) {
  if (!n) return;
  const size_t gw = ((cm_coop_pair_mem_bytes(CM_S4C_P_WAVE) + 15) & ~(size_t)15) + CM_XW_BYTES;
  const size_t gbk = ((cm_coop_pair_mem_bytes(CM_S4C_P_BLOCK) + 15) & ~(size_t)15) + CM_XW_BYTES;
  uint32_t pbig = CM_S4C_P_BIG;
  while (pbig > CM_S4C_P_BLOCK && !cm_lds_optin(&k_s4c_coop<1024, false>, ((cm_coop_pair_mem_bytes(pbig, false) + 15) & ~(size_t)15) + CM_XW_BYTES)) pbig >>= 1;
  if (!cm_lds_optin(&k_s4c_coop<CM_BLOCK, true>, gbk)) coop &= ~4u;
  CmDev d2 = d;
  d2.s4c_pbig = pbig > CM_S4C_P_BLOCK ? pbig : 0;
  hipLaunchKernelGGL(k_s4c_reduce, grid_for(n), dim3(CM_BLOCK), 0, s, d2, n, coop);
  if (!(coop & 4u)) return;
  uint32_t blocks = n / 2048 + 64;
  if (blocks > 4096) blocks = 4096;
  const size_t gs = ((cm_coop_pair_mem_bytes(CM_S4C_P_SMALL) + 15) & ~(size_t)15) + CM_XW_BYTES;
  if (cm_cls_on(d, CM_L_PF_WAVE)) hipLaunchKernelGGL((k_s4c_coop<64, true>), dim3(blocks), dim3(CM_BLOCK), (CM_BLOCK / 64) * gs, s, d, CM_S4C_P_SMALL, CM_L_PF_WAVE, coop);
  if (cm_cls_on(d, CM_L_PF_BLOCK)) hipLaunchKernelGGL((k_s4c_coop<CM_BLOCK, true>), dim3(blocks), dim3(CM_BLOCK), gw, s, d, CM_S4C_P_WAVE, CM_L_PF_BLOCK, coop);
  if (cm_cls_on(d, CM_L_PF_BLOCK_BIG)) hipLaunchKernelGGL((k_s4c_coop<CM_BLOCK, true>), dim3(256), dim3(CM_BLOCK), gbk, s, d, CM_S4C_P_BLOCK, CM_L_PF_BLOCK_BIG, coop);
  if (d2.s4c_pbig && cm_cls_on(d, CM_L_PF_HUGE))
    hipLaunchKernelGGL((k_s4c_coop<1024, false>), dim3(128), dim3(1024), ((cm_coop_pair_mem_bytes(pbig, false) + 15) & ~(size_t)15) + CM_XW_BYTES, s, d, pbig, 19u, coop);
}
void cm_launch_k_s5a_prepare(const CmDev &d, uint32_t n, hipStream_t s, bool coop) {
  if (!n) return;
  hipLaunchKernelGGL(k_s5a_prepare, grid_for(n), dim3(CM_BLOCK), 0, s, d, n, coop ? 1u : 0u);
  if (coop) {
    if (cm_cls_on(d, CM_L_S5_SMALL)) hipLaunchKernelGGL(k_s5_sort_coop, dim3(4096), dim3(CM_BLOCK), 0, s, d, CM_L_S5_SMALL);
    if (cm_cls_on(d, CM_L_S5_WAVE)) hipLaunchKernelGGL(k_s5_sort_coop, dim3(2048), dim3(CM_BLOCK), 0, s, d, CM_L_S5_WAVE);
    if (cm_cls_on(d, CM_L_S5_BLOCK)) hipLaunchKernelGGL(k_s5_sort_coop, dim3(64), dim3(CM_BLOCK), 0, s, d, CM_L_S5_BLOCK);
  }
}
void cm_launch_k_s5c_finalize(const CmDev &d, uint32_t n, hipStream_t s, bool coop) {
  if (!n) return;
  hipLaunchKernelGGL(k_s5c_finalize, grid_for(n), dim3(CM_BLOCK), 0, s, d, n, coop ? 1u : 0u);
  if (!coop) return;
  auto gbytes = [](uint32_t P) {
    const size_t b1 = cm_coop_ver_mem_bytes(P), b2 = cm_coop_sort_mem_bytes(CM_S5C_SORT_P, CM_S5C_SORT_RB);
    return (((b1 > b2 ? b1 : b2) + 15) & ~(size_t)15) + CM_XW_BYTES;
  };
  uint32_t blocks = n / 4096 + 64;
  if (blocks > 2048) blocks = 2048;
  if (cm_cls_on(d, CM_L_S5_SMALL)) hipLaunchKernelGGL(k_s5c_coop<64>, dim3(blocks), dim3(CM_BLOCK), (CM_BLOCK / 64) * gbytes(CM_S5C_P_SMALL), s, d, CM_S5C_P_SMALL, CM_L_S5_SMALL);
  if (cm_cls_on(d, CM_L_S5_WAVE)) hipLaunchKernelGGL(k_s5c_coop<64>, dim3(blocks), dim3(192), 3 * gbytes(CM_S5C_P_WAVE), s, d, CM_S5C_P_WAVE, CM_L_S5_WAVE);
  uint32_t pb = CM_S5C_P_BLOCK;
  while (pb > CM_S5C_P_WAVE && !cm_lds_optin(&k_s5c_coop<CM_BLOCK>, gbytes(pb))) pb >>= 1;
  if (cm_cls_on(d, CM_L_S5_BLOCK)) hipLaunchKernelGGL(k_s5c_coop<CM_BLOCK>, dim3(128), dim3(CM_BLOCK), gbytes(pb), s, d, pb, CM_L_S5_BLOCK);
}
CM_LAUNCH(k_s6a_pair_sam)
CM_LAUNCH(k_s6c_multi_sam)
void cm_launch_k_s5b_verify(const CmDev &d, uint32_t max_items, uint32_t n_reads, hipStream_t s) {
  if (!max_items) return;
  uint32_t blocks = (max_items + CM_BLOCK - 1) / CM_BLOCK;
  if (blocks > 65536) blocks = 65536;
  hipLaunchKernelGGL(k_s5b_verify, dim3(blocks), dim3(CM_BLOCK), 0, s, d, n_reads);
}
static inline size_t cm_s6_group_bytes(uint32_t P) { return ((cm_coop_pe_mem_bytes(P) + 15) & ~(size_t)15) + CM_XW_BYTES; }
void cm_launch_k_s6a_pair(const CmDev &d, uint32_t n, hipStream_t s, bool coop) {
  if (!n) return;
  const size_t lw = (CM_BLOCK / 64) * cm_s6_group_bytes(CM_S6A_P_WAVE), lb = cm_s6_group_bytes(CM_S6A_P_BLOCK);
  if (coop && !(cm_lds_optin(&k_s6a_coop<64>, lw) && cm_lds_optin(&k_s6a_coop<CM_BLOCK>, lb))) coop = false;
  hipLaunchKernelGGL(k_s6a_pair, grid_for(n), dim3(CM_BLOCK), 0, s, d, n, coop ? 1u : 0u);
  if (!coop) return;
  uint32_t blocks = n / 4096 + 64;
  if (blocks > 2048) blocks = 2048;
  if (cm_cls_on(d, CM_L_S6A_SMALL)) hipLaunchKernelGGL(k_s6a_coop<64>, dim3(blocks), dim3(CM_BLOCK), (CM_BLOCK / 64) * cm_s6_group_bytes(CM_S6A_P_SMALL), s, d, CM_S6A_P_SMALL, CM_L_S6A_SMALL);
  if (cm_cls_on(d, CM_L_S6A_WAVE)) hipLaunchKernelGGL(k_s6a_coop<64>, dim3(blocks), dim3(CM_BLOCK), lw, s, d, CM_S6A_P_WAVE, CM_L_S6A_WAVE);
  if (cm_cls_on(d, CM_L_S6A_BLOCK)) hipLaunchKernelGGL(k_s6a_coop<CM_BLOCK>, dim3(256), dim3(CM_BLOCK), lb, s, d, CM_S6A_P_BLOCK, CM_L_S6A_BLOCK);
}
void cm_launch_k_s6c_multi(const CmDev &d, uint32_t n, hipStream_t s, bool coop) {
  if (!n) return;
  const size_t lw = (CM_BLOCK / 64) * cm_s6_group_bytes(CM_S6A_P_WAVE), lb = cm_s6_group_bytes(CM_S6A_P_BLOCK);
  if (coop && !(cm_lds_optin(&k_s6c_coop<64>, lw) && cm_lds_optin(&k_s6c_coop<CM_BLOCK>, lb))) coop = false;
  hipLaunchKernelGGL(k_s6c_multi, grid_for(n), dim3(CM_BLOCK), 0, s, d, n, coop ? 1u : 0u);
  if (!coop) return;
  uint32_t blocks = n / 4096 + 64;
  if (blocks > 2048) blocks = 2048;
  if (cm_cls_on(d, CM_L_S6C_SMALL)) hipLaunchKernelGGL(k_s6c_coop<64>, dim3(blocks), dim3(CM_BLOCK), (CM_BLOCK / 64) * cm_s6_group_bytes(CM_S6A_P_SMALL), s, d, CM_S6A_P_SMALL, CM_L_S6C_SMALL);
  if (cm_cls_on(d, CM_L_S6C_WAVE)) hipLaunchKernelGGL(k_s6c_coop<64>, dim3(blocks), dim3(CM_BLOCK), lw, s, d, CM_S6A_P_WAVE, CM_L_S6C_WAVE);
  if (cm_cls_on(d, CM_L_S6C_BLOCK)) hipLaunchKernelGGL(k_s6c_coop<CM_BLOCK>, dim3(256), dim3(CM_BLOCK), lb, s, d, CM_S6A_P_BLOCK, CM_L_S6C_BLOCK);
}

static inline void staging_geometry(uint32_t max_read_len, uint32_t *threads, uint32_t *lds_half) {
  uint32_t pb = 128;
  while (pb > 16 && (uint64_t)pb * max_read_len + 64 > 24 * 1024) pb >>= 1;
  *threads = 2 * pb;
  *lds_half = (uint32_t)(((uint64_t)pb * max_read_len + 64 + 15) & ~15ull);
}
static bool prep_mm_geometry(const CmDev &d, uint32_t max_read_len, uint32_t *threads, uint32_t *half, uint32_t *stg, size_t *lds, bool *gstage = nullptr, bool *e6_out = nullptr) {
  if (d.p.w != 7 || 2 * d.p.k + 12 > 64) return false;
  *stg = max_read_len / 4 + 4;
  const bool g = max_read_len > 69;
  const bool e6 = !g && 2 * d.p.k + 8 <= 48;
  if (gstage) *gstage = g;
  if (e6_out) *e6_out = e6;
  uint32_t t = 256;
  for (;; t >>= 1) {
    *half = (uint32_t)(((uint64_t)(t / 2) * max_read_len + 64 + 15) & ~15ull);
    *lds = 2 * (size_t)*half + (g ? (size_t)(2 * t + 1) * 4 : (size_t)*stg * t * (e6 ? 6 : 8)) + 64;
    if (*lds <= (g ? 48 : 60) * 1024) break;
    if (t == 64) return false;
  }
  *threads = t;
  return true;
}
static bool prep_flat_geometry(const CmDev &d, uint32_t max_read_len, uint32_t tile_reads, uint32_t *half, uint32_t *nt_max, size_t *lds) {
  if (d.p.w != 7 || !(d.p.k & 1) || d.p.k > 26 || max_read_len > 69 || max_read_len < (uint32_t)d.p.k + 6) return false;
  *half = (uint32_t)(((uint64_t)(CM_BLOCK / 2) * max_read_len + 64 + 15) & ~15ull);
  *nt_max = tile_reads * (max_read_len - (uint32_t)d.p.k + 1);
  const size_t region0 = 2 * (size_t)*half > 16 * (size_t)*nt_max ? 2 * (size_t)*half : 16 * (size_t)*nt_max;
  const size_t nw = *half / 16 + 1;
  *lds = region0 + 2 * (nw + 3) * 4 + 2 * (nw + 1) * 2 + 8 + CM_BLOCK * sizeof(CmFlatRead) + (CM_BLOCK + 2) * 4 + ((size_t)*nt_max + 2) * 2 * 2 + 8 + 32 * 4;
  return *lds <= 64 * 1024;
}
bool cm_prep_flat_supported(const CmDev &d, uint32_t max_read_len, uint32_t tile_reads) {
  uint32_t h, n;
  size_t l;
  return prep_flat_geometry(d, max_read_len, tile_reads, &h, &n, &l);
}
void cm_launch_k_prep_flat(const CmDev &d, uint32_t pair_lo, uint32_t pair_hi, uint32_t max_read_len, uint32_t tile_reads, uint32_t mm_cap,
                           unsigned long long *cursor, hipStream_t s) {
  uint32_t half, nt_max;
  size_t lds;
  if (pair_hi <= pair_lo || !prep_flat_geometry(d, max_read_len, tile_reads, &half, &nt_max, &lds)) return;
  const uint32_t pb = CM_BLOCK / 2;
  hipLaunchKernelGGL(k_prep_flat, dim3((pair_hi - pair_lo + pb - 1) / pb), dim3(CM_BLOCK), lds, s, d, pair_lo, pair_hi, half, nt_max, tile_reads, mm_cap, cursor);
}
bool cm_prep_mm_supported(const CmDev &d, uint32_t max_read_len) {
  uint32_t t, h, g;
  size_t l;
  return prep_mm_geometry(d, max_read_len, &t, &h, &g, &l);
}
uint32_t cm_prep_mm_pairs_per_block(const CmDev &d, uint32_t max_read_len) {
  uint32_t threads, half, stg;
  size_t lds;
  return prep_mm_geometry(d, max_read_len, &threads, &half, &stg, &lds) ? threads / 2 : 0;
}
size_t cm_prep_mm_stage_bytes(const CmDev &d, uint32_t max_read_len, uint32_t pairs) {
  uint32_t threads, half, stg;
  size_t lds;
  bool g = false;
  if (!prep_mm_geometry(d, max_read_len, &threads, &half, &stg, &lds, &g) || !g) return 0;
  const uint32_t pb = threads / 2;
  return (size_t)((pairs + pb - 1) / pb) * stg * threads * 8;
}
void cm_launch_k_prep_mm(const CmDev &d, uint32_t pair_lo, uint32_t pair_hi, uint32_t max_read_len, uint32_t mm_cap,
                         unsigned long long *cursor, hipStream_t s, void *gstage) {
  uint32_t threads, half, stg;
  size_t lds;
  bool g = false, e6 = false;
  if (pair_hi <= pair_lo || !prep_mm_geometry(d, max_read_len, &threads, &half, &stg, &lds, &g, &e6)) return;
  const uint32_t pb = threads / 2;
  if (g) hipLaunchKernelGGL((k_prep_mm<true, false>), dim3((pair_hi - pair_lo + pb - 1) / pb), dim3(threads), lds, s, d, pair_lo, pair_hi, half, stg, mm_cap, cursor, (uint64_t *)gstage);
  else if (e6) hipLaunchKernelGGL((k_prep_mm<false, true>), dim3((pair_hi - pair_lo + pb - 1) / pb), dim3(threads), lds, s, d, pair_lo, pair_hi, half, stg, mm_cap, cursor, (uint64_t *)nullptr);
  else hipLaunchKernelGGL((k_prep_mm<false, false>), dim3((pair_hi - pair_lo + pb - 1) / pb), dim3(threads), lds, s, d, pair_lo, pair_hi, half, stg, mm_cap, cursor, (uint64_t *)nullptr);
}
static inline int probe_variant_norm(int variant) {
  if (variant == 0) variant = CM_PROBE_U;
  const int u = variant & 15;
  return ((u == 2 || u == 4 || u == 8) ? u : 1) | (variant & 16);
// ... 80 lines not shown
```

### chromap_amd/csrc/cm_stages.h

```cpp
#ifndef CM_STAGES_H_
#define CM_STAGES_H_

#include "cm_types.h"

CM_HD uint32_t cm_c2u(uint8_t c) {
  const uint32_t u = c & 0xDFu;
  const uint32_t x = (u >> 1) & 3u;
  const uint32_t o = u - 0x41u;
  const bool acgt = o < 20u && ((0x80045u >> (o & 31u)) & 1u);
  return acgt ? x ^ (x >> 1) : 4u;
}
CM_HD uint8_t cm_negchar(uint8_t c) {
  const uint32_t v = 3u ^ cm_c2u(c);
  return v == 0 ? 'A' : v == 1 ? 'C' : v == 2 ? 'G' : v == 3 ? 'T' : 'N';
}

CM_HD uint64_t cm_hash64(uint64_t key, uint64_t mask) {
  key = (~key + (key << 21)) & mask;
  key = key ^ key >> 24;
  key = ((key + (key << 3)) + (key << 8)) & mask;
  key = key ^ key >> 14;
  key = ((key + (key << 2)) + (key << 4)) & mask;
  key = key ^ key >> 28;
  key = (key + (key << 31)) & mask;
  return key;
}

CM_HD uint64_t cm_hash64_split(uint32_t lo, uint32_t hi, uint32_t hm) {
  {
    const uint64_t t = (uint64_t)(uint32_t)~lo + (uint64_t)(uint32_t)(lo << 21);
    hi = ((~hi) + ((hi << 21) | (lo >> 11)) + (uint32_t)(t >> 32)) & hm;
    lo = (uint32_t)t;
  }
  lo ^= (lo >> 24) | (hi << 8);
  hi ^= hi >> 24;
  {
    const uint64_t t = (uint64_t)lo * 265u;
    hi = (hi * 265u + (uint32_t)(t >> 32)) & hm;
    lo = (uint32_t)t;
  }
  lo ^= (lo >> 14) | (hi << 18);
  hi ^= hi >> 14;
  {
    const uint64_t t = (uint64_t)lo * 21u;
    hi = (hi * 21u + (uint32_t)(t >> 32)) & hm;
    lo = (uint32_t)t;
  }
  lo ^= (lo >> 28) | (hi << 4);
  hi ^= hi >> 28;
  {
    const uint64_t t = (uint64_t)lo + (uint64_t)(uint32_t)(lo << 31);
    hi = (hi + ((hi << 31) | (lo >> 1)) + (uint32_t)(t >> 32)) & hm;
    lo = (uint32_t)t;
  }
  return ((uint64_t)hi << 32) | lo;
}
CM_HD uint64_t cm_hash64_split2(uint32_t lo, uint32_t hi, uint32_t hm) {
  {
    const uint64_t t = (uint64_t)(uint32_t)~lo + (uint64_t)(uint32_t)(lo << 21);
    hi = ((~hi) + (lo >> 11) + (uint32_t)(t >> 32)) & hm;
    lo = (uint32_t)t;
  }
  lo ^= (lo >> 24) | (hi << 8);
  {
    const uint64_t t = (uint64_t)lo * 265u;
    hi = (hi + (uint32_t)(t >> 32)) & hm;
    lo = (uint32_t)t;
  }
  lo ^= (lo >> 14) | (hi << 18);
  {
    const uint64_t t = (uint64_t)lo * 21u;
    hi = (hi + (uint32_t)(t >> 32)) & hm;
    lo = (uint32_t)t;
  }
  lo ^= (lo >> 28) | (hi << 4);
  {
    const uint64_t t = (uint64_t)lo + (uint64_t)(uint32_t)(lo << 31);
    hi = (hi + (lo >> 1) + (uint32_t)(t >> 32)) & hm;
    lo = (uint32_t)t;
  }
  return ((uint64_t)hi << 32) | lo;
}
template <int HV>
CM_HD uint64_t cm_hash64_v(uint64_t key, uint64_t mask) {
  if (HV == 0) return cm_hash64_split2((uint32_t)key, (uint32_t)(key >> 32), 3u);
  if (HV == 1) return cm_hash64_split((uint32_t)key, (uint32_t)(key >> 32), (uint32_t)(mask >> 32));
// ... 1073 lines not shown
      ++ci;
      if (!have) { ws = s; we = en; have = true; continue; }
      if (we < s) { es = ws; ee = we; emit = true; ws = s; we = en; break; }
      we = en;
    }
    if (!emit) {
      if (!have) break;
      es = ws; ee = we; have = false; emit = true;
    }
    int32_t l = prev_l, m = 0, rr = (int32_t)(nocc - 1);
    while (l <= rr) {
      m = (l + rr) / 2;
      const uint64_t cp = o[m] >> 1;
      ++reads;
      if (cp < es) l = m + 1;
      else if (cp > es) rr = m - 1;
      else break;
    }
    prev_l = m;
    for (uint32_t oi = (uint32_t)m; oi < nocc; ++oi) {
      const uint64_t rh = o[oi];
      ++reads;
      if ((rh >> 1) > ee) break;
      const uint64_t cp = cm_cand_from_hit(rh, ps, d.p.k, &same);
      if ((same && strand == 0) || (!same && strand == 1)) { if (out) out[cnt] = cp; ++cnt; }
    }
    if (!have && ci >= mn) break;
  }
  if (reads_out) *reads_out += reads;
  return cnt;
}
CM_HD void cm_rescue_rep(const CmDev &d, uint8_t kind, uint64_t val, uint32_t ps, uint32_t *rep_len, uint32_t *prev_rep) {
  if (kind == CM_PR_MISS || kind == CM_PR_SINGLE) return;
  const uint32_t nocc = (uint32_t)val;
  if (nocc >= (uint32_t)d.p.f0) {
    const uint32_t rp = ps >> 1;
    if (*prev_rep > rp) *rep_len += (uint32_t)d.p.k;
    else if (rp < *prev_rep + (uint32_t)d.p.k + (uint32_t)d.p.w - 1) *rep_len += rp - *prev_rep;
    else *rep_len += (uint32_t)d.p.k;
    *prev_rep = rp;
  }
}
CM_HD int cm_rescue(const CmDev &d, uint32_t r, int strand, const uint64_t *mp, const uint8_t *mc, uint32_t mn,
                    uint64_t *out, uint32_t *n_out, uint32_t *rep_len_out, unsigned long long *occ_reads) {
  int max_count = 0, best_num = 0;
  for (uint32_t i = 0; i < mn; ++i) {
    const int c = mc[i];
    if (c > max_count) { max_count = c; best_num = 1; }
    else if (c == max_count) ++best_num;
  }
  *n_out = 0;
  if (cm_rescue_bails(d, max_count, best_num, mn)) return -max_count;
  const uint32_t b = d.mm_off[r], n = d.mm_cnt[r];
  uint32_t cnt = 0, rep_len = 0, prev_rep = ~0u;
  unsigned long long reads = 0;
  for (uint32_t mi0 = 0; mi0 < n; mi0 += CM_S3B_GROUP) {
    uint8_t kind_g[CM_S3B_GROUP];
    uint64_t val_g[CM_S3B_GROUP];
    uint32_t ps_g[CM_S3B_GROUP];
#pragma unroll
    for (int q = 0; q < CM_S3B_GROUP; ++q) {
      const bool in = mi0 + q < n;
      kind_g[q] = in ? d.pr_kind[b + mi0 + q] : (uint8_t)CM_PR_MISS;
      val_g[q] = in ? d.pr_val[b + mi0 + q] : 0;
      ps_g[q] = in ? d.mm_ps[b + mi0 + q] : 0;
    }
#pragma unroll
    for (int q = 0; q < CM_S3B_GROUP; ++q) {
      cnt += cm_rescue_minimizer(d, strand, mp, mc, mn, max_count, kind_g[q], val_g[q], ps_g[q], out ? out + cnt : nullptr, &reads);
      cm_rescue_rep(d, kind_g[q], val_g[q], ps_g[q], &rep_len, &prev_rep);
    }
  }
  *n_out = cnt;
  *rep_len_out = rep_len;
  if (occ_reads) *occ_reads += reads;
  return max_count;
}

CM_HD const uint64_t *cm_c0_pos(const CmDev &d, uint32_t r) { return d.hbuf + d.hit_off[r]; }
CM_HD const uint8_t *cm_c0_pcnt(const CmDev &d, uint32_t r) { return d.hcnt + d.hit_off[r]; }
CM_HD const uint64_t *cm_c0_neg(const CmDev &d, uint32_t r) { return d.hbuf + d.hit_off[r] + d.n_pos_hit[r]; }
CM_HD const uint8_t *cm_c0_ncnt(const CmDev &d, uint32_t r) { return d.hcnt + d.hit_off[r] + d.n_pos_hit[r]; }

CM_HD bool cm_s4a_decide(const CmDev &d, uint32_t r) {
  const uint32_t pair = r >> 1;
  d.aug[r] = 0; d.res_neg[r] = 0; d.res_pos[r] = 0; d.resc_n[r] = 0; d.resc_p[r] = 0;
  const bool live = d.p.single ? ((r & 1) == 0 && d.mm_cnt[r] > 0) : (d.mm_cnt[2 * pair] > 0 && d.mm_cnt[2 * pair + 1] > 0);
  const uint32_t ncp = d.ncp[r], ncn = d.ncn[r];
  d.m_tot[r] = live ? ncp + ncn : 0;
  if (!live) return false;
  const uint32_t mm_count = d.mm_cnt[r];
  bool augment = !d.p.split && !d.p.single;
  const uint8_t *pc = cm_c0_pcnt(d, r), *nc = cm_c0_ncnt(d, r);
  for (uint32_t i = 0; augment && i < ncp; ++i) if (pc[i] >= mm_count / 2) { augment = false; break; }
  if (augment) for (uint32_t i = 0; i < ncn; ++i) if (nc[i] >= mm_count / 2) { augment = false; break; }
  return augment;
}
CM_HD void cm_s4a_rescue(const CmDev &d, uint32_t r) {
  const uint32_t o = r ^ 1u;
  d.aug[r] = 1;
  uint32_t cntn = 0, cntp = 0, rl = 0;
  int res_neg = 0, res_pos = 0;
  bool set_rl = false;
  uint32_t rl_val = 0;
  unsigned long long occ_reads = 0;
  if (d.ncp[o] > 0) {
    res_neg = cm_rescue(d, r, 1, cm_c0_pos(d, o), cm_c0_pcnt(d, o), d.ncp[o], nullptr, &cntn, &rl, &occ_reads);
    if (res_neg >= 0) { set_rl = true; rl_val = rl; }
  }
  if (d.ncn[o] > 0) {
    res_pos = cm_rescue(d, r, 0, cm_c0_neg(d, o), cm_c0_ncnt(d, o), d.ncn[o], nullptr, &cntp, &rl, &occ_reads);
    if (res_pos >= 0) { set_rl = true; rl_val = rl; }
  }
  d.res_neg[r] = res_neg; d.res_pos[r] = res_pos;
  d.resc_n[r] = cntn; d.resc_p[r] = cntp;
  if (set_rl) d.rep_len[r] = rl_val;
  d.m_tot[r] = d.ncp[r] + d.ncn[r] + cntn + cntp;
}
CM_HD void cm_s4a_rescue_count(const CmDev &d, uint32_t r) {
  if (cm_s4a_decide(d, r)) cm_s4a_rescue(d, r);
}

CM_HD uint32_t cm_merge(const uint64_t *p1, const uint8_t *c1, uint32_t n1, uint64_t *out, uint8_t *outc,
                        uint32_t n2, int e) {
  const uint64_t *p2 = out + n1;
  const uint8_t *c2 = outc + n1;
  if (n1 == 0) return n2;
  uint32_t i = 0, j = 0, k = 0;
#define CM_BACK_OK(P) (k == 0 || (P) > out[k - 1] + (uint64_t)(int64_t)e)
  while (i < n1 && j < n2) {
    const uint64_t a = p1[i], b = p2[j];
    if (a == b) {
      if (CM_BACK_OK(a)) {
        const uint8_t ca = c1[i], cb = c2[j];
        if (ca > cb) { out[k] = a; outc[k] = ca; } else { out[k] = b; outc[k] = cb; }
        ++k;
      }
      ++i; ++j;
    } else if (a < b) {
      if (CM_BACK_OK(a)) { const uint8_t ca = c1[i]; out[k] = a; outc[k] = ca; ++k; }
      ++i;
    } else {
      if (CM_BACK_OK(b)) { const uint8_t cb = c2[j]; out[k] = b; outc[k] = cb; ++k; }
      ++j;
    }
  }
  while (i < n1) { const uint64_t a = p1[i]; if (CM_BACK_OK(a)) { const uint8_t ca = c1[i]; out[k] = a; outc[k] = ca; ++k; } ++i; }
  while (j < n2) { const uint64_t b = p2[j]; if (CM_BACK_OK(b)) { const uint8_t cb = c2[j]; out[k] = b; outc[k] = cb; ++k; } ++j; }
#undef CM_BACK_OK
  return k;
}

#define CM_S4B_ALL 0
#define CM_S4B_PREFILLED 1
#define CM_S4B_FILL_ONLY 2
CM_HD void cm_s4b_rescue_merge(const CmDev &d, uint32_t r, int mode = CM_S4B_ALL) {
  const bool prefilled = mode == CM_S4B_PREFILLED;
  const uint32_t o = r ^ 1u;
  d.mcp[r] = 0; d.mcn[r] = 0;
  if (d.m_tot[r] == 0) return;
  const uint32_t ncp = d.ncp[r], ncn = d.ncn[r], rp = d.resc_p[r], rn = d.resc_n[r];
  uint64_t *P = d.mbuf + d.m_off[r];
  uint8_t *PC = d.mcnt + d.m_off[r];
  uint64_t *N = P + ncp + rp;
  uint8_t *NC = PC + ncp + rp;
  const uint64_t *p0 = cm_c0_pos(d, r), *n0 = cm_c0_neg(d, r);
  const uint8_t *pc0 = cm_c0_pcnt(d, r), *nc0 = cm_c0_ncnt(d, r);
  uint32_t naug_p = 0, naug_n = 0;
  if (d.aug[r]) {
    uint32_t cnt = 0, rl = 0;
    if (d.ncp[o] > 0 && d.res_neg[r] >= 0 && rn > 0) {
      if (prefilled) cnt = rn; else cm_rescue(d, r, 1, cm_c0_pos(d, o), cm_c0_pcnt(d, o), d.ncp[o], N + ncn, &cnt, &rl, nullptr);
      if (mode != CM_S4B_FILL_ONLY) {
        cm_sort_u64(N + ncn, cnt);
        naug_n = cm_sweep(N + ncn, NC + ncn, cnt, d.p.e, 1, d.mm_cnt[r]);
      }
    }
    if (d.ncn[o] > 0 && d.res_pos[r] >= 0 && rp > 0) {
      if (prefilled) cnt = rp; else cm_rescue(d, r, 0, cm_c0_neg(d, o), cm_c0_ncnt(d, o), d.ncn[o], P + ncp, &cnt, &rl, nullptr);
      if (mode != CM_S4B_FILL_ONLY) {
        cm_sort_u64(P + ncp, cnt);
        naug_p = cm_sweep(P + ncp, PC + ncp, cnt, d.p.e, 1, d.mm_cnt[r]);
      }
    }
  }
  if (mode == CM_S4B_FILL_ONLY) return;
  if (naug_p > 0) {
    d.mcp[r] = cm_merge(p0, pc0, ncp, P, PC, naug_p, d.p.e);
  } else {
    for (uint32_t i = 0; i < ncp; ++i) { P[i] = p0[i]; PC[i] = pc0[i]; }
    d.mcp[r] = ncp;
  }
  if (naug_n > 0) {
    d.mcn[r] = cm_merge(n0, nc0, ncn, N, NC, naug_n, d.p.e);
  } else {
    for (uint32_t i = 0; i < ncn; ++i) { N[i] = n0[i]; NC[i] = nc0[i]; }
    d.mcn[r] = ncn;
  }
}

CM_HD uint64_t *cm_m_pos(const CmDev &d, uint32_t r) { return d.mbuf + d.m_off[r]; }
CM_HD uint8_t *cm_m_pcnt(const CmDev &d, uint32_t r) { return d.mcnt + d.m_off[r]; }
CM_HD uint64_t *cm_m_neg(const CmDev &d, uint32_t r) { return d.mbuf + d.m_off[r] + d.ncp[r] + d.resc_p[r]; }
CM_HD uint8_t *cm_m_ncnt(const CmDev &d, uint32_t r) { return d.mcnt + d.m_off[r] + d.ncp[r] + d.resc_p[r]; }
CM_HD uint64_t *cm_f_pos(const CmDev &d, uint32_t r) { return d.fbuf + d.m_off[r]; }
CM_HD uint8_t *cm_f_pcnt(const CmDev &d, uint32_t r) { return d.fcnt + d.m_off[r]; }
CM_HD uint64_t *cm_f_neg(const CmDev &d, uint32_t r) { return d.fbuf + d.m_off[r] + d.ncp[r] + d.resc_p[r]; }
CM_HD uint8_t *cm_f_ncnt(const CmDev &d, uint32_t r) { return d.fcnt + d.m_off[r] + d.ncp[r] + d.resc_p[r]; }

CM_HD void cm_reduce_dir(uint32_t dist, const uint64_t *p1, const uint8_t *c1, uint32_t n1, const uint64_t *p2,
                         const uint8_t *c2, uint32_t n2, uint64_t *f1, uint8_t *fc1, uint32_t *nf1, uint64_t *f2,
                         uint8_t *fc2, uint32_t *nf2) {
  uint32_t i1 = 0, i2 = 0, o1 = 0, o2 = 0;
  int unpaired1 = 0, unpaired2 = 0;
  int max1 = 6, max2 = 6;
  uint32_t prev_end_i2 = 0;
  while (i1 < n1 && i2 < n2) {
    const uint64_t a = p1[i1], b = p2[i2];
    if (a > b + dist) {
      if (i2 >= prev_end_i2 && unpaired2 < 5 && (a >> 32) == (b >> 32) && (int)c2[i2] >= max2) {
        f2[o2] = b; fc2[o2] = c2[i2]; ++o2;
        ++unpaired2;
      }
      ++i2;
    } else if (b > a + dist) {
      if (unpaired1 < 5 && (a >> 32) == (b >> 32) && (int)c1[i1] >= max1) {
        f1[o1] = a; fc1[o1] = c1[i1]; ++o1;
        ++unpaired1;
      }
      ++i1;
    } else {
      f1[o1] = a; fc1[o1] = c1[i1]; ++o1;
      if ((int)c1[i1] > max1) max1 = c1[i1];
      uint32_t cur = i2;
      while (cur < n2 && p2[cur] <= a + dist) {
        if (cur >= prev_end_i2) {
          f2[o2] = p2[cur]; fc2[o2] = c2[cur]; ++o2;
          if ((int)c2[cur] > max2) max2 = c2[cur];
        }
        ++cur;
      }
      prev_end_i2 = cur;
      ++i1;
    }
  }
  *nf1 = o1;
  *nf2 = o2;
}

CM_HD void cm_rerank(const CmDev &d, uint32_t r) {
  if (!d.rid_rank) return;
  uint64_t *fp = cm_f_pos(d, r), *fn = cm_f_neg(d, r);
  for (uint32_t i = 0; i < d.fcp[r]; ++i) fp[i] = (fp[i] & 0xffffffffull) | ((uint64_t)d.rid_rank[(uint32_t)(fp[i] >> 32)] << 32);
  for (uint32_t i = 0; i < d.fcn[r]; ++i) fn[i] = (fn[i] & 0xffffffffull) | ((uint64_t)d.rid_rank[(uint32_t)(fn[i] >> 32)] << 32);
}

CM_HD bool cm_s4c_pre(const CmDev &d, uint32_t pair) {
  const uint32_t r1 = 2 * pair, r2 = r1 + 1;
  d.fcp[r1] = d.fcn[r1] = d.fcp[r2] = d.fcn[r2] = 0;
  d.alive[pair] = 0;
  d.force0[pair] = 0;
  if (d.p.single) {
    if (d.mm_cnt[r1] == 0 || d.mcp[r1] + d.mcn[r1] == 0) return false;
    const uint64_t *mp = cm_m_pos(d, r1), *mn = cm_m_neg(d, r1);
    const uint8_t *mpc = cm_m_pcnt(d, r1), *mnc = cm_m_ncnt(d, r1);
    uint64_t *fp = cm_f_pos(d, r1), *fn = cm_f_neg(d, r1);
    uint8_t *fpc = cm_f_pcnt(d, r1), *fnc = cm_f_ncnt(d, r1);
    for (uint32_t i = 0; i < d.mcp[r1]; ++i) { fp[i] = mp[i]; fpc[i] = mpc[i]; }
    for (uint32_t i = 0; i < d.mcn[r1]; ++i) { fn[i] = mn[i]; fnc[i] = mnc[i]; }
    d.fcp[r1] = d.mcp[r1]; d.fcn[r1] = d.mcn[r1];
    d.alive[pair] = 1;
    cm_rerank(d, r1);
    return false;
  }
  if (!(d.mm_cnt[r1] > 0 && d.mm_cnt[r2] > 0)) return false;
  int ret = 0;
  for (uint32_t r = r1; r <= r2; ++r) {
    if (!d.aug[r]) continue;
    const int pr = d.res_neg[r], nr = d.res_pos[r];
    if (((pr < 0 && nr > 0 && -pr >= nr) || (pr > 0 && nr < 0 && pr <= -nr)) && d.ncp[r] + d.ncn[r] == 0) ret = 1;
  }
  d.force0[pair] = (uint8_t)ret;
  const uint32_t nc1 = d.mcp[r1] + d.mcn[r1], nc2 = d.mcp[r2] + d.mcn[r2];
  if (!(nc1 > 0 && nc2 > 0)) return false;
  if (d.p.split) {
    for (uint32_t r = r1; r <= r2; ++r) {
      const uint64_t *mp = cm_m_pos(d, r), *mn = cm_m_neg(d, r);
      const uint8_t *mpc = cm_m_pcnt(d, r), *mnc = cm_m_ncnt(d, r);
      uint64_t *fp = cm_f_pos(d, r), *fn = cm_f_neg(d, r);
      uint8_t *fpc = cm_f_pcnt(d, r), *fnc = cm_f_ncnt(d, r);
      for (uint32_t i = 0; i < d.mcp[r]; ++i) { fp[i] = mp[i]; fpc[i] = mpc[i]; }
      for (uint32_t i = 0; i < d.mcn[r]; ++i) { fn[i] = mn[i]; fnc[i] = mnc[i]; }
      d.fcp[r] = d.mcp[r]; d.fcn[r] = d.mcn[r];
    }
    d.alive[pair] = 1;
    cm_rerank(d, r1); cm_rerank(d, r2);
    return false;
  }
  return true;
}
CM_HD void cm_s4c_filter(const CmDev &d, uint32_t pair) {
  const uint32_t r1 = 2 * pair, r2 = r1 + 1;
  uint32_t a, b;
  cm_reduce_dir((uint32_t)d.p.max_insert, cm_m_pos(d, r1), cm_m_pcnt(d, r1), d.mcp[r1], cm_m_neg(d, r2),
                cm_m_ncnt(d, r2), d.mcn[r2], cm_f_pos(d, r1), cm_f_pcnt(d, r1), &a, cm_f_neg(d, r2), cm_f_ncnt(d, r2), &b);
  d.fcp[r1] = a; d.fcn[r2] = b;
  cm_reduce_dir((uint32_t)d.p.max_insert, cm_m_neg(d, r1), cm_m_ncnt(d, r1), d.mcn[r1], cm_m_pos(d, r2),
                cm_m_pcnt(d, r2), d.mcp[r2], cm_f_neg(d, r1), cm_f_ncnt(d, r1), &a, cm_f_pos(d, r2), cm_f_pcnt(d, r2), &b);
  d.fcn[r1] = a; d.fcp[r2] = b;
}
CM_HD void cm_s4c_post(const CmDev &d, uint32_t pair) {
  const uint32_t r1 = 2 * pair, r2 = r1 + 1;
  const uint32_t f1 = d.fcp[r1] + d.fcn[r1], f2 = d.fcp[r2] + d.fcn[r2];
  d.alive[pair] = (f1 > 0 && f2 > 0) ? 1 : 0;
  if (d.alive[pair]) { cm_rerank(d, r1); cm_rerank(d, r2); }
}
CM_HD void cm_s4c_reduce(const CmDev &d, uint32_t pair) {
  if (!cm_s4c_pre(d, pair)) return;
  cm_s4c_filter(d, pair);
  cm_s4c_post(d, pair);
}

CM_HD uint32_t cm_text_code(const uint8_t *read, int L, int i, bool neg) {
  if (!neg) return cm_c2u(read[i]);
  const uint32_t c = cm_c2u(read[L - 1 - i]);
  return c < 4 ? 3u ^ c : 4u;
}
CM_HD uint8_t cm_text_char(const uint8_t *read, int L, int i, bool neg) {
  return neg ? cm_negchar(read[L - 1 - i]) : read[i];
}

CM_HD uint32_t cm_peq_get(const uint32_t *P, uint32_t c) {
  return c == 0 ? P[0] : c == 1 ? P[1] : c == 2 ? P[2] : c == 3 ? P[3] : P[4];
}
CM_HD void cm_peq_or(uint32_t *P, uint32_t c, uint32_t bit) {
  P[0] |= c == 0 ? bit : 0u; P[1] |= c == 1 ? bit : 0u; P[2] |= c == 2 ? bit : 0u;
  P[3] |= c == 3 ? bit : 0u; P[4] |= c == 4 ? bit : 0u;
}

struct CmFwdReader {
  const uint64_t *ap;
  uint64_t cur, nxt;
  uint32_t left, words;
  CM_HD void init(const uint8_t *p, uint32_t n) {
    const uintptr_t a = reinterpret_cast<uintptr_t>(p);
    const uint32_t sh = (uint32_t)(a & 7);
    ap = reinterpret_cast<const uint64_t *>(a & ~(uintptr_t)7);
    words = n ? (sh + n + 7) >> 3 : 0;
    cur = 0; nxt = 0; left = 0;
    if (words) { cur = *ap++ >> (sh * 8); left = 8 - sh; --words; }
    if (words) { nxt = *ap++; --words; }
  }
  CM_HD uint8_t next() {
    if (left == 0) {
      cur = nxt; left = 8;
      if (words) { nxt = *ap++; --words; }
    }
    const uint8_t b = (uint8_t)cur;
    cur >>= 8; --left;
    return b;
  }
};
struct CmBwdReader {
  const uint64_t *ap;
  uint64_t cur, nxt;
  uint32_t left, words;
  CM_HD void init(const uint8_t *p, uint32_t n) {
    const uintptr_t a = reinterpret_cast<uintptr_t>(p);
    const uint32_t pos = (uint32_t)(a & 7);
    ap = reinterpret_cast<const uint64_t *>(a & ~(uintptr_t)7);
    words = n ? ((7 - pos) + n + 7) >> 3 : 0;
    cur = 0; nxt = 0; left = 0;
    if (words) { cur = *ap-- << ((7 - pos) * 8); left = pos + 1; --words; }
    if (words) { nxt = *ap--; --words; }
  }
  CM_HD uint8_t next() {
    if (left == 0) {
      cur = nxt; left = 8;
      if (words) { nxt = *ap--; --words; }
    }
    const uint8_t b = (uint8_t)(cur >> 56);
    cur <<= 8; --left;
    return b;
  }
};

template <bool NEG>
CM_HD int cm_banded_align_stream(int e, const uint8_t *pattern, const uint8_t *read, int Lfull, int toff, int L, int *end_pos) {
  CmFwdReader pr;
  pr.init(pattern, (uint32_t)(L + 2 * e));
  CmFwdReader tf;
  CmBwdReader tb;
  if (NEG) tb.init(read + (Lfull - 1 - toff), (uint32_t)L); else tf.init(read + toff, (uint32_t)L);
  uint32_t P[5] = {0, 0, 0, 0, 0};
  for (int i = 0; i < 2 * e; i++) cm_peq_or(P, cm_c2u(pr.next()), 1u << i);
  const uint32_t hi = 1u << (2 * e);
  uint32_t VP = 0, VN = 0;
  int err = 0;
  for (int i = 0; i < L; i++) {
    cm_peq_or(P, cm_c2u(pr.next()), hi);
    uint32_t tc;
// ... 408 lines not shown
    uint32_t X = cm_peq_get(P, tc) | VN;
    const uint32_t D0 = ((VP + (X & VP)) ^ VP) | X;
    const uint32_t HN = VP & D0;
    const uint32_t HP = VN | ~(VP | D0);
    X = D0 >> 1;
    prev_VN = VN; prev_VP = VP;
    VN = X & HP;
    VP = HN | ~(X | HP);
    prev_err = err;
    err += 1 - (int)(D0 & 1u);
    if (err > 2 * e) {
      if (i < 4 * e && i < L / 2) fail_beginning = true;
      break;
    }
    P[0] >>= 1; P[1] >>= 1; P[2] >>= 1; P[3] >>= 1; P[4] >>= 1;
  }
  if (i < L) { err = prev_err; VN = prev_VN; VP = prev_VP; }
  const int band_start = i - 1;
  int min_err = err;
  *read_mapping_length = i;
  *end_pos = band_start;
  for (i = 0; i < 2 * e; i++) {
    err += (int)((VP >> i) & 1u);
    err -= (int)((VN >> i) & 1u);
    if (err < min_err || (err == min_err && i + 1 == e)) {
      min_err = err;
      *end_pos = band_start + 1 + i;
    }
  }
  if (fail_beginning || (L > 60 && *end_pos + 1 - e - min_err < 30)) *end_pos = -*end_pos;
  return min_err;
}
CM_HD int cm_banded_align_dropoff(int e, const uint8_t *pattern, const uint8_t *read, int Lfull, bool neg, int toff, int L,
                                  bool from3, int *end_pos, int *read_mapping_length) {
  if (from3) return neg ? cm_banded_align_dropoff_stream<true, true>(e, pattern, read, Lfull, toff, L, end_pos, read_mapping_length)
                        : cm_banded_align_dropoff_stream<true, false>(e, pattern, read, Lfull, toff, L, end_pos, read_mapping_length);
  return neg ? cm_banded_align_dropoff_stream<false, true>(e, pattern, read, Lfull, toff, L, end_pos, read_mapping_length)
             : cm_banded_align_dropoff_stream<false, false>(e, pattern, read, Lfull, toff, L, end_pos, read_mapping_length);
}

CM_HD int cm_adjust_gap_beginning(int strand, const uint8_t *ref, uint32_t ref_len, const uint8_t *read, int Lfull, bool neg,
                                  int toff, int *gap_beginning, int read_end, int ref_start_position, int ref_end_position) {
  int i, j;
  if (strand == 0) {
    if (*gap_beginning <= 0) return ref_start_position;
    for (i = *gap_beginning - 1, j = ref_start_position - 1; i >= 0 && j >= 0; --i, --j) {
      const uint8_t rc = cm_text_char(read, Lfull, toff + i, neg), fc = ref[j];
      if (rc != fc && (int)rc != (int)fc - 'a' + 'A') break;
    }
    *gap_beginning = i + 1;
    return j + 1;
  }
  if (*gap_beginning <= 0) return ref_end_position;
  for (i = read_end + 1, j = ref_end_position + 1; toff + i < Lfull && (uint32_t)j < ref_len; ++i, ++j) {
    const uint8_t rc = cm_text_char(read, Lfull, toff + i, neg), fc = ref[j];
    if (rc != fc && (int)rc != (int)fc - 'a' + 'A') break;
  }
  *gap_beginning = *gap_beginning + i - (read_end + 1);
  return j - 1;
}

CM_HD bool cm_valid_candidate(const CmDev &d, uint32_t rid, uint32_t position, uint32_t L) {
  const uint32_t rl = d.ref_len[rid];
  return !(position < (uint32_t)d.p.e || position >= rl || position + L + (uint32_t)d.p.e >= rl);
}

struct CmBest { int min_err, second_err, n_best, n_second; };
CM_HD void cm_update_best(CmBest &m, int ne) {
  if (ne < m.min_err) { m.second_err = m.min_err; m.n_second = m.n_best; m.min_err = ne; m.n_best = 1; }
  else if (ne == m.min_err) m.n_best++;
  else if (ne == m.second_err) m.n_second++;
  else if (ne < m.second_err) { m.n_second = 1; m.second_err = ne; }
}

CM_HD int cm_verify_compute(const CmDev &d, const uint8_t *read, uint32_t L, int strand, uint64_t cpos, int *end_pos) {
  const int e = d.p.e;
  const uint32_t rid = (uint32_t)(cpos >> 32);
  uint32_t position = (uint32_t)cpos;
  if (strand == 1) position = position - L + 1;
  *end_pos = (int)L;
  return cm_banded_align(e, d.ref + d.ref_off[rid] + position - e, read, (int)L, strand == 1, 0, (int)L, end_pos);
}

CM_HD bool cm_verify_one(const CmDev &d, const uint8_t *read, uint32_t L, int strand, uint64_t cpos, CmBest &bst,
                         uint64_t *dp, int16_t *de, uint32_t *nd, const int16_t *pre_err, const int16_t *pre_end,
                         uint32_t ci) {
  const int e = d.p.e;
  int end_pos = (int)L;
  int ne;
  if (pre_err) { ne = pre_err[ci]; end_pos = pre_end[ci]; }
  else ne = cm_verify_compute(d, read, L, strand, cpos, &end_pos);
  if (ne <= e) {
    cm_update_best(bst, ne);
    dp[*nd] = strand == 0 ? cpos - (uint64_t)e + (uint64_t)(int64_t)end_pos
                          : cpos - L + 1 - (uint64_t)e + (uint64_t)(int64_t)end_pos;
    de[*nd] = (int16_t)ne;
    ++*nd;
    return true;
  }
  return false;
}

CM_HD uint32_t cm_draft_strand(const CmDev &d, const uint8_t *read, uint32_t L, int strand, const uint64_t *cp,
                               const uint8_t *cc, uint32_t nc, CmBest &bst, uint64_t *dp, int16_t *de,
                               const int16_t *pre_err = nullptr, const int16_t *pre_end = nullptr) {
  uint32_t nd = 0;
  const int lanes = d.p.lanes;
  if (lanes == 0 || nc < (uint32_t)lanes) {
    for (uint32_t ci = 0; ci < nc; ++ci) {
      const uint32_t rid = (uint32_t)(cp[ci] >> 32);
      uint32_t position = (uint32_t)cp[ci];
      if (strand == 1) position = position - L + 1;
      if (!cm_valid_candidate(d, rid, position, L)) continue;
      cm_verify_one(d, read, L, strand, cp[ci], bst, dp, de, &nd, pre_err, pre_end, ci);
    }
    return nd;
  }
  uint64_t vpos[8];
  uint8_t vcnt[8];
  uint32_t vidx[8];
  uint32_t nvalid = 0, thr = 0, ci = 0;
  while (ci < nc) {
    if (cc[ci] < thr) break;
    const uint32_t rid = (uint32_t)(cp[ci] >> 32);
    uint32_t position = (uint32_t)cp[ci];
    if (strand == 1) position = position - L + 1;
    if (!cm_valid_candidate(d, rid, position, L)) { ++ci; continue; }
    vpos[nvalid] = cp[ci];
    vcnt[nvalid] = cc[ci];
    vidx[nvalid] = ci;
    ++nvalid;
    ++ci;
    if (nvalid < (uint32_t)lanes) continue;
    for (int mi = 0; mi < lanes; ++mi)
      if (!cm_verify_one(d, read, L, strand, vpos[mi], bst, dp, de, &nd, pre_err, pre_end, vidx[mi])) thr = vcnt[mi];
    nvalid = 0;
  }
  for (uint32_t i = 0; i < nvalid; ++i) cm_verify_one(d, read, L, strand, vpos[i], bst, dp, de, &nd, pre_err, pre_end, vidx[i]);
  return nd;
}


CM_HD uint32_t cm_draft_strand_split(const CmDev &d, const uint8_t *read, uint32_t L, int strand, const uint64_t *cp,
                                     const uint8_t *cc, uint32_t nc, CmBest &bst, uint64_t *dp, int16_t *de, uint32_t *ds,
                                     const uint32_t *tp = nullptr) {
  const int e = d.p.e;
  uint32_t nd = 0, thr = 0;
  for (uint32_t ci = 0; ci < nc; ++ci) {
    if (cc[ci] < thr) break;
    const uint32_t rid = (uint32_t)(cp[ci] >> 32);
    uint32_t position = (uint32_t)cp[ci];
    if (strand == 1) position = position - L + 1;
    if (!cm_valid_candidate(d, rid, position, L)) continue;
    int mep = (int)L, gap_beginning = 0, num_errors = 0, actual = 0, rml = 0;
    const int allow = 20 - e;
    const uint64_t gpat = d.ref_off[rid] + position - (uint32_t)e;
    const uint8_t *pat = d.ref + gpat;
    const bool pl = tp != nullptr && d.ref_pl != nullptr;
    if (strand == 0) {
      num_errors = pl ? cm_banded_align_dropoff_planes<false>(e, d.ref_pl, gpat, tp, d.read_pl_w, 0u, (int)L, &mep, &rml)
                      : cm_banded_align_dropoff(e, pat, read, (int)L, false, 0, (int)L, false, &mep, &rml);
      if (mep < 0 && allow > 0) {
        const int b_err = num_errors, b_mep = -mep, b_rml = rml;
        num_errors = pl ? cm_banded_align_dropoff_planes<false>(e, d.ref_pl, gpat + (uint32_t)allow, tp, d.read_pl_w, (uint32_t)allow, (int)L - allow, &mep, &rml)
                        : cm_banded_align_dropoff(e, pat + allow, read, (int)L, false, allow, (int)L - allow, false, &mep, &rml);
        if (num_errors > e || mep < 0) { num_errors = b_err; mep = b_mep; rml = b_rml; }
        else { gap_beginning = allow; mep += gap_beginning; rml += gap_beginning; }
      }
    } else {
      num_errors = pl ? cm_banded_align_dropoff_planes<true>(e, d.ref_pl, gpat + L + 2 * (uint32_t)e - 1, tp, d.read_pl_w, 0u, (int)L, &mep, &rml)
                      : cm_banded_align_dropoff(e, pat, read, (int)L, true, 0, (int)L, true, &mep, &rml);
      if (mep < 0 && allow > 0) {
        const int b_err = num_errors, b_mep = -mep, b_rml = rml;
        num_errors = pl ? cm_banded_align_dropoff_planes<true>(e, d.ref_pl, gpat + (L - (uint32_t)allow) + 2 * (uint32_t)e - 1, tp, d.read_pl_w, (uint32_t)allow,
                                                               (int)L - allow, &mep, &rml)
                        : cm_banded_align_dropoff(e, pat, read, (int)L, true, 0, (int)L - allow, true, &mep, &rml);
        if (num_errors > e || mep < 0) { num_errors = b_err; mep = b_mep; rml = b_rml; }
        else { gap_beginning = allow; mep += gap_beginning; rml += gap_beginning; }
      }
    }
    if (mep + 1 - e - num_errors - gap_beginning >= 30) {
      actual = num_errors;
      num_errors = -(mep - e - num_errors - gap_beginning);
    } else {
      num_errors = e + 1;
      actual = e + 1;
    }
    if (num_errors <= e) {
      if (num_errors < bst.min_err) {
        bst.second_err = bst.min_err; bst.n_second = bst.n_best; bst.min_err = num_errors; bst.n_best = 1;
        thr = nc > 50 ? cc[ci] : cc[ci] / 2;
      } else if (num_errors == bst.min_err) bst.n_best++;
      else if (num_errors == bst.second_err) bst.n_second++;
      else if (num_errors < bst.second_err) { bst.n_second = 1; bst.second_err = num_errors; }
      dp[nd] = strand == 0 ? cp[ci] - (uint64_t)e + (uint64_t)(int64_t)mep
                           : (d.p.sam ? cp[ci] - (uint64_t)L + 1 - (uint64_t)e + (uint64_t)(int64_t)mep : cp[ci] - (uint64_t)(int64_t)gap_beginning);
      de[nd] = (int16_t)num_errors;
      ds[nd] = (uint32_t)(((actual & 0xff) << 24) | ((gap_beginning & 0xff) << 16) | (rml & 0xffff));
      ++nd;
    }
  }
  return nd;
}

CM_HD void cm_s5_verify(const CmDev &d, uint32_t r) {
  const uint32_t pair = r >> 1;
  d.ndp[r] = 0; d.ndn[r] = 0;
  const int e = d.p.e;
  CmBest bst = {e + 1, e + 1, 0, 0};
  if (d.alive[pair]) {
    const uint32_t L = d.rlen[r];
    const uint8_t *read = cm_read_ptr(d, r);
    uint64_t *pp = cm_f_pos(d, r), *np = cm_f_neg(d, r);
    uint8_t *pc = cm_f_pcnt(d, r), *nc = cm_f_ncnt(d, r);
    const uint32_t ncp = d.fcp[r], ncn = d.fcn[r];
    uint64_t *dpp = d.dpos + d.m_off[r], *dpn = d.dpos + d.m_off[r] + d.ncp[r] + d.resc_p[r];
    int16_t *dep = d.derr + d.m_off[r], *den = d.derr + d.m_off[r] + d.ncp[r] + d.resc_p[r];
    bool done = false;
    if (d.p.split) {
      uint32_t *dsp = d.dsplit + d.m_off[r], *dsn = d.dsplit + d.m_off[r] + d.ncp[r] + d.resc_p[r];
      cm_sort_cand(pp, pc, ncp);
      cm_sort_cand(np, nc, ncn);
      const uint32_t *tp = d.read_pl ? cm_read_pl_of(d, r) : nullptr;
      d.ndp[r] = cm_draft_strand_split(d, read, L, 0, pp, pc, ncp, bst, dpp, dep, dsp, tp);
      d.ndn[r] = cm_draft_strand_split(d, read, L, 1, np, nc, ncn, bst, dpn, den, dsn, tp);
      done = true;
    } else if (ncp + ncn == 1) {
      const int strand = ncp == 1 ? 0 : 1;
      const uint64_t cpos = strand == 0 ? pp[0] : np[0];
      const uint8_t cnt = strand == 0 ? pc[0] : nc[0];
      if ((uint32_t)cnt == d.mm_cnt[r]) {
        bst.min_err = 0; bst.n_best = 1; bst.n_second = 0;
        const uint32_t rid = (uint32_t)(cpos >> 32);
        const uint32_t position = strand == 0 ? (uint32_t)cpos : (uint32_t)cpos - L + 1;
        if (cm_valid_candidate(d, rid, position, L)) {
          if (strand == 0) { dpp[0] = cpos + L - 1; dep[0] = 0; d.ndp[r] = 1; }
          else { dpn[0] = cpos; den[0] = 0; d.ndn[r] = 1; }
          done = true;
        }
      }
    }
    if (!done) {
      cm_sort_cand(pp, pc, ncp);
      cm_sort_cand(np, nc, ncn);
      d.ndp[r] = cm_draft_strand(d, read, L, 0, pp, pc, ncp, bst, dpp, dep);
      d.ndn[r] = cm_draft_strand(d, read, L, 1, np, nc, ncn, bst, dpn, den);
    }
  }
  d.min_err[r] = bst.min_err; d.second_err[r] = bst.second_err;
  d.n_best[r] = bst.n_best; d.n_second[r] = bst.n_second;
}


CM_HD bool cm_s5a_prepare(const CmDev &d, uint32_t r, uint32_t coop_min = 0) {
  const uint32_t pair = r >> 1;
  d.nv[r] = 0;
  if (d.p.split || !d.alive[pair]) { cm_s5_verify(d, r); return false; }
  d.ndp[r] = 0; d.ndn[r] = 0;
  const int e = d.p.e;
  CmBest bst = {e + 1, e + 1, 0, 0};
  const uint32_t L = d.rlen[r];
  uint64_t *pp = cm_f_pos(d, r), *np = cm_f_neg(d, r);
  uint8_t *pc = cm_f_pcnt(d, r), *nc = cm_f_ncnt(d, r);
  const uint32_t ncp = d.fcp[r], ncn = d.fcn[r];
  bool done = false;
  if (ncp + ncn == 1) {
    const int strand = ncp == 1 ? 0 : 1;
    const uint64_t cpos = strand == 0 ? pp[0] : np[0];
    const uint8_t cnt = strand == 0 ? pc[0] : nc[0];
    if ((uint32_t)cnt == d.mm_cnt[r]) {
      bst.min_err = 0; bst.n_best = 1; bst.n_second = 0;
      const uint32_t rid = (uint32_t)(cpos >> 32);
      const uint32_t position = strand == 0 ? (uint32_t)cpos : (uint32_t)cpos - L + 1;
      if (cm_valid_candidate(d, rid, position, L)) {
        if (strand == 0) { d.dpos[d.m_off[r]] = cpos + L - 1; d.derr[d.m_off[r]] = 0; d.ndp[r] = 1; }
        else { const uint32_t o = d.m_off[r] + d.ncp[r] + d.resc_p[r]; d.dpos[o] = cpos; d.derr[o] = 0; d.ndn[r] = 1; }
        done = true;
      }
    }
  }
  bool to_group = false;
  if (!done) {
    to_group = coop_min > 0 && ncp + ncn > coop_min;
    if (!to_group) {
      cm_sort_cand(pp, pc, ncp);
      cm_sort_cand(np, nc, ncn);
    }
    d.nv[r] = ncp + ncn;
  }
  d.min_err[r] = bst.min_err; d.second_err[r] = bst.second_err;
  d.n_best[r] = bst.n_best; d.n_second[r] = bst.n_second;
  return to_group;
}

CM_HD void cm_s5b_verify_at(const CmDev &d, uint32_t r, int strand, uint32_t ci);
CM_HD void cm_s5b_verify_item(const CmDev &d, uint32_t j, uint32_t n_reads) {
  uint32_t lo = 0, hi = n_reads;
  while (hi - lo > 1) {
    const uint32_t mid = lo + ((hi - lo) >> 1);
    if (d.v_off[mid] <= j) lo = mid; else hi = mid;
  }
  const uint32_t r = lo, li = j - d.v_off[r];
  const uint32_t ncp = d.fcp[r];
  const int strand = li < ncp ? 0 : 1;
  const uint32_t ci = strand ? li - ncp : li;
  cm_s5b_verify_at(d, r, strand, ci);
}
CM_HD void cm_s5b_verify_at(const CmDev &d, uint32_t r, int strand, uint32_t ci) {
  const uint32_t o = d.m_off[r] + (strand ? d.ncp[r] + d.resc_p[r] : 0) + ci;
  const uint64_t cpos = d.fbuf[o];
  const uint32_t L = d.rlen[r];
  const uint32_t rid = (uint32_t)(cpos >> 32);
  const uint32_t position = strand == 0 ? (uint32_t)cpos : (uint32_t)cpos - L + 1;
  if (!cm_valid_candidate(d, rid, position, L)) { d.v_err[o] = CM_V_INVALID; d.v_end[o] = 0; return; }
  int end_pos = (int)L;
  int ne;
  if (d.ref_pl && d.read_pl)
    ne = cm_banded_align_planes(d.p.e, d.ref_pl, d.ref_off[rid] + position - (uint32_t)d.p.e,
                                cm_read_pl_of(d, r) + (size_t)strand * 3 * d.read_pl_w, d.read_pl_w, (int)L, &end_pos);
  else ne = cm_verify_compute(d, cm_read_ptr(d, r), L, strand, cpos, &end_pos);
  d.v_err[o] = (int16_t)ne;
  d.v_end[o] = (int16_t)end_pos;
}

CM_HD void cm_s5c_accept(const CmDev &d, uint32_t r);
CM_HD void cm_s5c_finalize(const CmDev &d, uint32_t r, uint32_t coop_min = 0) {
  if (d.nv[r] == 0) return;
  if (coop_min > 0 && d.nv[r] > coop_min) return;
  cm_s5c_accept(d, r);
}
CM_HD void cm_s5c_accept(const CmDev &d, uint32_t r) {
  CmBest bst = {d.min_err[r], d.second_err[r], d.n_best[r], d.n_second[r]};
  const uint32_t L = d.rlen[r];
  const uint8_t *read = cm_read_ptr(d, r);
  const uint32_t op = d.m_off[r], on = d.m_off[r] + d.ncp[r] + d.resc_p[r];
  d.ndp[r] = cm_draft_strand(d, read, L, 0, d.fbuf + op, d.fcnt + op, d.fcp[r], bst, d.dpos + op, d.derr + op, d.v_err + op, d.v_end + op);
  d.ndn[r] = cm_draft_strand(d, read, L, 1, d.fbuf + on, d.fcnt + on, d.fcn[r], bst, d.dpos + on, d.derr + on, d.v_err + on, d.v_end + on);
  d.min_err[r] = bst.min_err; d.second_err[r] = bst.second_err;
  d.n_best[r] = bst.n_best; d.n_second[r] = bst.n_second;
}

struct CmPe { int min_sum, second_sum, n_best, n_second; uint32_t f_dir, f_i1, f_i2; };

CM_HD bool cm_pair_dir(const CmDev &d, int dir, const uint64_t *ap, const int16_t *ae, uint32_t na,
                       const uint64_t *bp, const int16_t *be, uint32_t nb, uint32_t len1, uint32_t len2, CmPe &pe,
                       int64_t want, int final_min, int64_t *seen) {
  const uint64_t I = (uint64_t)(int64_t)d.p.max_insert;
  const uint64_t mo = (uint32_t)d.p.min_read_len;
  uint32_t i1 = 0, i2 = 0;
  while (i1 < na && i2 < nb) {
    const uint64_t p1 = ap[i1], p2 = bp[i2];
    if ((dir == 1 && p1 > p2 + I - len2) || (dir == 0 && p1 > p2 + len1 - mo)) {
      ++i2;
    } else if ((dir == 0 && p2 > p1 + I - len1) || (dir == 1 && p2 > p1 + len2 - mo)) {
      ++i1;
    } else {
      uint32_t cur = i2;
      while (cur < nb && ((dir == 0 && bp[cur] <= p1 + I - len1) || (dir == 1 && bp[cur] <= p1 + len2 - mo))) {
        const int s = (int)ae[i1] + (int)be[cur];
        if (want >= 0) {
          if (s == final_min) {
            if (*seen == want) { pe.f_dir = (uint32_t)dir; pe.f_i1 = i1; pe.f_i2 = cur; return true; }
            ++*seen;
          }
        } else if (s < pe.min_sum) {
          pe.second_sum = pe.min_sum; pe.n_second = pe.n_best; pe.min_sum = s; pe.n_best = 1;
          pe.f_dir = (uint32_t)dir; pe.f_i1 = i1; pe.f_i2 = cur;
        } else if (s == pe.min_sum) {
          pe.n_best++;
        } else if (s == pe.second_sum) {
          pe.n_second++;
        } else if (s < pe.second_sum) {
          pe.second_sum = s; pe.n_second = 1;
        }
        ++cur;
      }
      ++i1;
    }
  }
  return false;
}

struct CmSpan { uint32_t rid, ref_start, ref_end; };
CM_HD CmSpan cm_ref_start_end(const CmDev &d, uint64_t dpos, int nerr, int strand, const uint8_t *read, int L) {
  const int e = d.p.e;
  const uint32_t rid = (uint32_t)(dpos >> 32), ref_pos = (uint32_t)dpos;
  const uint32_t rl = d.ref_len[rid];
  uint32_t vw = ref_pos + 1 > (uint32_t)(L + e) ? ref_pos + 1 - (uint32_t)L - (uint32_t)e : 0;
  if (ref_pos + (uint32_t)e >= rl) vw = rl - (uint32_t)e - (uint32_t)L;
  const int start = cm_banded_traceback(e, nerr, d.ref + d.ref_off[rid] + vw, read, L, strand == 1, 0, L);
  CmSpan s;
  s.rid = rid;
  s.ref_start = vw + (uint32_t)start;
  s.ref_end = ref_pos;
  return s;
}

template <int W1T>
CM_HD int cm_ksw_sg3(const uint8_t *query, const uint8_t *read, int L, bool neg, int e, uint32_t *z, uint64_t zstride,
                     uint32_t *cigar, int *n_cigar, int *start, int *end, int Lfull = -1, int toff = 0) {
  if (Lfull < 0) Lfull = L;
  const int NEG = -0x40000000, o_del = 6, e_del = 1, e_ins = 1, oe_del = 7, oe_ins = 7;
  const int w = 2 * e + 1, w1 = w + 1, qlen = L + 2 * e;
  constexpr int ZW = (W1T + 3) / 4;
  int h[W1T], ev[W1T];
  uint32_t qc[W1T];
#pragma unroll
  for (int jj = 0; jj < W1T; ++jj) { h[jj] = 0; ev[jj] = NEG; qc[jj] = jj < w1 ? cm_c2u(query[jj]) : 4u; }
  for (int i = 0; i < L; ++i) {
    int f = NEG;
    int h1 = i == 0 ? -(o_del + e_del) : NEG;
    const uint32_t tc = cm_text_code(read, Lfull, toff + i, neg);
    const int cnt = i == L - 1 ? w1 - 1 : w1;
    uint32_t packed = 0;
#pragma unroll
    for (int jj = 0; jj < W1T; ++jj) {
      if (jj < cnt) {
        const int sc = (tc > 3 || qc[jj] > 3) ? 0 : (tc == qc[jj] ? 1 : -4);
        int m = h[jj], ee = ev[jj];
        h[jj] = h1;
// ... 504 lines not shown
    }
    seen += (int64_t)prod;
  }
  pe.n_best = seen > 0x7fffffff ? 0x7fffffff : (int)seen;
}


template <bool SAM>
CM_HD void cm_emit_single_split_at(const CmDev &d, uint32_t pair, uint64_t slot, int strand, uint32_t mi) {
  const uint32_t r = 2 * pair;
  const uint32_t L = d.rlen[r];
  const uint64_t dp = cm_d_pos(d, r, strand)[mi];
  const int err = cm_d_err(d, r, strand)[mi];
  const uint32_t w = (d.dsplit + d.m_off[r] + (strand ? d.ncp[r] + d.resc_p[r] : 0))[mi];
  CmSamAln sa;
  CmSpan sp;
  if constexpr (SAM) sp = cm_ref_start_end_split_sam(d, pair, pair, dp, w, strand, cm_read_ptr(d, r), (int)L, &sa);
  else sp = cm_ref_start_end_split(d, dp, w, strand, cm_read_ptr(d, r), (int)L);
  const uint16_t al = (uint16_t)(sp.ref_end - sp.ref_start + 1);
  const uint8_t mapq = cm_mapq_single_split(d, err, al, (int)L, d.p.e, d.second_err[r], d.n_best[r], d.n_second[r], d.rep_len[r],
                                            strand == 0 ? d.fcp[r] : d.fcn[r]);
  const uint8_t is_unique = d.n_best[r] == 1 ? 1 : 0;
  uint8_t *o = d.rec + slot * 24;
  uint32_t *o32 = reinterpret_cast<uint32_t *>(o);
  uint16_t *o16 = reinterpret_cast<uint16_t *>(o);
  o32[0] = d.first_read_id + pair;
  o32[1] = sp.rid;
  o32[2] = sp.ref_start;
  o16[6] = al;
  o[14] = mapq & 63;
  o[15] = strand == 0 ? 1 : 0;
  o[16] = is_unique;
  o[17] = 1;
  o16[9] = 0; o16[10] = 0; o16[11] = 0;
  d.rec_ok[slot] = 1;
  if constexpr (SAM)
    cm_put_sam_record(d, pair, d.first_read_id + pair, sp, 0, -1, 0, strand == 0 ? 0u : 16u, mapq, strand == 0 ? 1 : 0, is_unique, sa, L);
}

template <bool SAM>
CM_HD void cm_emit_single_record(const CmDev &d, uint32_t pair, uint32_t choice, uint32_t nth = 0) {
  const uint32_t r = 2 * pair;
  const uint64_t slot = (uint64_t)pair * (uint32_t)d.p.max_best + nth;
  const int me = d.min_err[r];
  uint32_t idx = 0;
  for (int strand = 0; strand < 2; ++strand) {
    const uint64_t *dp = cm_d_pos(d, r, strand);
    const int16_t *de = cm_d_err(d, r, strand);
    const uint32_t n = strand ? d.ndn[r] : d.ndp[r];
    for (uint32_t mi = 0; mi < n; ++mi) {
      if ((int)de[mi] > me) continue;
      if (idx == choice) {
        if (d.p.split) { cm_emit_single_split_at<SAM>(d, pair, slot, strand, mi); return; }
        const uint32_t L = d.rlen[r];
        CmSamAln sa;
        CmSpan sp;
        if constexpr (SAM) sp = cm_ref_start_end_sam(d, pair, pair, dp[mi], strand, cm_read_ptr(d, r), (int)L, &sa);
        else sp = cm_ref_start_end(d, dp[mi], de[mi], strand, cm_read_ptr(d, r), (int)L);
        const uint16_t al = (uint16_t)(sp.ref_end - sp.ref_start + 1);
        const uint8_t mapq = cm_mapq_single(d, de[mi], al, (int)L, d.p.e, d.second_err[r], d.n_best[r], d.n_second[r], d.rep_len[r]);
        uint8_t *o = d.rec + slot * 24;
        uint32_t *o32 = reinterpret_cast<uint32_t *>(o);
        uint16_t *o16 = reinterpret_cast<uint16_t *>(o);
        o32[0] = d.first_read_id + pair;
        o32[1] = sp.rid;
        o32[2] = sp.ref_start;
        o16[6] = al;
        o[14] = mapq & 63;
        o[15] = strand == 0 ? 1 : 0;
        o[16] = d.n_best[r] == 1 ? 1 : 0;
        o[17] = 1;
        o16[9] = 0; o16[10] = 0; o16[11] = 0;
        d.rec_ok[slot] = 1;
        if constexpr (SAM)
          cm_put_sam_record(d, pair, d.first_read_id + pair, sp, 0, -1, 0, strand == 0 ? 0u : 16u, mapq, strand == 0 ? 1 : 0,
                            d.n_best[r] == 1 ? 1 : 0, sa, L);
        return;
      }
      ++idx;
    }
  }
}

template <bool SAM = false>
CM_HD bool cm_s6a_pre(const CmDev &d, uint32_t pair) {
  const uint32_t r1 = 2 * pair, r2 = r1 + 1;
  for (uint32_t t = 0; t < (uint32_t)d.p.max_best; ++t) d.rec_ok[(uint64_t)pair * (uint32_t)d.p.max_best + t] = 0;
  d.pe_nbest[pair] = 0;
  if (!d.alive[pair]) return false;
  const uint32_t nd1 = d.ndp[r1] + d.ndn[r1], nd2 = d.ndp[r2] + d.ndn[r2];
  if (d.p.single) {
    if (nd1 == 0) return false;
    d.pe_nbest[pair] = d.n_best[r1];
    d.pe_min[pair] = d.min_err[r1]; d.pe_second[pair] = d.second_err[r1]; d.pe_nsecond[pair] = d.n_second[r1];
    if (d.n_best[r1] == 1) cm_emit_single_record<SAM>(d, pair, 0);
    return false;
  }
  if (!(nd1 > 0 && nd2 > 0)) return false;
  if (d.p.split) {
    CmPe sp;
    cm_split_pairing(d, pair, 0, sp);
    d.pe_min[pair] = sp.min_sum; d.pe_second[pair] = sp.second_sum;
    d.pe_nbest[pair] = sp.n_best; d.pe_nsecond[pair] = sp.n_second;
    d.pe_first[pair] = sp.f_dir; d.pe_i1[pair] = sp.f_i1; d.pe_i2[pair] = sp.f_i2;
    if (sp.n_best == 1) cm_emit_pairs_record<SAM>(d, pair, sp);
    return false;
  }
  return true;
}
template <bool SAM = false>
CM_HD void cm_s6a_sweeps(const CmDev &d, uint32_t pair) {
  const uint32_t r1 = 2 * pair, r2 = r1 + 1;
  for (uint32_t r = r1; r <= r2; ++r) {
    cm_sort_draft(const_cast<uint64_t *>(cm_d_pos(d, r, 0)), const_cast<int16_t *>(cm_d_err(d, r, 0)), d.ndp[r]);
    cm_sort_draft(const_cast<uint64_t *>(cm_d_pos(d, r, 1)), const_cast<int16_t *>(cm_d_err(d, r, 1)), d.ndn[r]);
  }
  CmPe pe;
  pe.min_sum = 2 * d.p.e + 1; pe.second_sum = 2 * d.p.e + 1; pe.n_best = 0; pe.n_second = 0;
  pe.f_dir = 0; pe.f_i1 = 0; pe.f_i2 = 0;
  int64_t seen = 0;
  const uint32_t len1 = d.rlen[r1], len2 = d.rlen[r2];
  cm_pair_dir(d, 0, cm_d_pos(d, r1, 0), cm_d_err(d, r1, 0), d.ndp[r1], cm_d_pos(d, r2, 1), cm_d_err(d, r2, 1), d.ndn[r2],
              len1, len2, pe, -1, 0, &seen);
  cm_pair_dir(d, 1, cm_d_pos(d, r1, 1), cm_d_err(d, r1, 1), d.ndn[r1], cm_d_pos(d, r2, 0), cm_d_err(d, r2, 0), d.ndp[r2],
              len1, len2, pe, -1, 0, &seen);
  d.pe_min[pair] = pe.min_sum; d.pe_second[pair] = pe.second_sum;
  d.pe_nbest[pair] = pe.n_best; d.pe_nsecond[pair] = pe.n_second;
  d.pe_first[pair] = pe.f_dir; d.pe_i1[pair] = pe.f_i1; d.pe_i2[pair] = pe.f_i2;
  if (pe.n_best == 1) cm_emit_record<SAM>(d, pair, pe);
}
template <bool SAM = false>
CM_HD void cm_s6a_pair(const CmDev &d, uint32_t pair) {
  if (cm_s6a_pre<SAM>(d, pair)) cm_s6a_sweeps<SAM>(d, pair);
}

struct CmMt { uint32_t mt[624]; int idx; };
CM_HD void cm_mt_seed(CmMt &g, uint32_t s) {
  g.mt[0] = s;
  for (int i = 1; i < 624; ++i) g.mt[i] = 1812433253u * (g.mt[i - 1] ^ (g.mt[i - 1] >> 30)) + (uint32_t)i;
  g.idx = 624;
}
CM_HD uint32_t cm_mt_next(CmMt &g) {
  if (g.idx >= 624) {
    for (int i = 0; i < 624; ++i) {
      const uint32_t y = (g.mt[i] & 0x80000000u) | (g.mt[(i + 1) % 624] & 0x7fffffffu);
      g.mt[i] = g.mt[(i + 397) % 624] ^ (y >> 1) ^ ((y & 1) ? 0x9908b0dfu : 0);
    }
    g.idx = 0;
  }
  uint32_t y = g.mt[g.idx++];
  y ^= y >> 11;
  y ^= (y << 7) & 0x9d2c5680u;
  y ^= (y << 15) & 0xefc60000u;
  y ^= y >> 18;
  return y;
}
CM_HD int cm_mt_uniform(CmMt &g, int hi) {
  const uint32_t range = (uint32_t)hi + 1u;
  uint64_t product = (uint64_t)cm_mt_next(g) * (uint64_t)range;
  uint32_t low = (uint32_t)product;
  if (low < range) {
    const uint32_t threshold = (uint32_t)(0u - range) % range;
    while (low < threshold) {
      product = (uint64_t)cm_mt_next(g) * (uint64_t)range;
      low = (uint32_t)product;
    }
  }
  return (int)(product >> 32);
}

CM_HD uint32_t cm_num_chunks(uint32_t n, uint32_t ref_batch, uint32_t grain) {
  uint32_t tot = 0;
  for (uint32_t b0 = 0; b0 < n; b0 += ref_batch) {
    const uint32_t bn = n - b0 < ref_batch ? n - b0 : ref_batch;
    const uint32_t T = bn / grain;
    tot += T <= 1 ? 1 : T;
  }
  return tot;
}
CM_HD void cm_chunk_range(uint32_t n, uint32_t ref_batch, uint32_t grain, uint32_t c, uint32_t *lo, uint32_t *hi) {
  for (uint32_t b0 = 0; b0 < n; b0 += ref_batch) {
    const uint32_t bn = n - b0 < ref_batch ? n - b0 : ref_batch;
    uint32_t T = bn / grain;
    if (T <= 1) T = 1;
    if (c >= T) { c -= T; continue; }
    if (T == 1) { *lo = b0; *hi = b0 + bn; return; }
    const uint32_t dv = bn / T, md = bn % T;
    const uint32_t s = b0 + c * dv + (c < md ? c : md);
    *lo = s;
    *hi = s + dv + (c < md ? 1 : 0);
    return;
  }
  *lo = *hi = n;
}

CM_HD void cm_reservoir(const CmDev &d, uint32_t pair, int nb, CmMt &g) {
  const int K = d.p.max_best;
  uint32_t *ch = d.pe_choice + (uint64_t)pair * (uint32_t)K;
  for (int i = 0; i < K; ++i) ch[i] = (uint32_t)i;
  if (nb <= K) return;
  for (int i = K; i < nb; ++i) {
    const int j = cm_mt_uniform(g, i);
    if (j < K) ch[j] = (uint32_t)i;
  }
  for (int a = 1; a < K; ++a) {
    const uint32_t v = ch[a];
    int b = a - 1;
    while (b >= 0 && ch[b] > v) { ch[b + 1] = ch[b]; --b; }
    ch[b + 1] = v;
  }
}

CM_HD void cm_s6b_sample(const CmDev &d, uint32_t chunk, CmMt &g) {
  uint32_t lo, hi;
  cm_chunk_range(d.n_pairs, (uint32_t)d.p.ref_batch, (uint32_t)d.p.grain, chunk, &lo, &hi);
  bool seeded = false;
  for (uint32_t pair = lo; pair < hi; ++pair) {
    const int nb = d.pe_nbest[pair];
    if (nb <= 1) continue;
    if (!d.p.single && nb > d.p.drop_rep) continue;
    if (!seeded || d.p.single) { cm_mt_seed(g, 11); seeded = true; }
    cm_reservoir(d, pair, nb, g);
  }
}

template <bool SAM = false>
CM_HD void cm_s6c_multi(const CmDev &d, uint32_t pair) {
  const int nb = d.pe_nbest[pair];
  if (nb <= 1 || (!d.p.single && nb > d.p.drop_rep)) return;
  const uint32_t r1 = 2 * pair, r2 = r1 + 1;
  CmPe pe;
  pe.min_sum = d.pe_min[pair]; pe.second_sum = d.pe_second[pair]; pe.n_best = nb; pe.n_second = d.pe_nsecond[pair];
  pe.f_dir = d.pe_first[pair]; pe.f_i1 = d.pe_i1[pair]; pe.f_i2 = d.pe_i2[pair];
  const uint32_t K = (uint32_t)d.p.max_best;
  const uint32_t to_report = (uint32_t)nb < K ? (uint32_t)nb : K;
  for (uint32_t t = 0; t < to_report; ++t) {
    const int64_t want = (int64_t)d.pe_choice[(uint64_t)pair * K + t];
    if (d.p.single) { cm_emit_single_record<SAM>(d, pair, (uint32_t)want, t); continue; }
    if (d.p.split) {
      CmPe sp;
      cm_split_pairing(d, pair, want, sp);
      cm_emit_pairs_record<SAM>(d, pair, sp, t);
      continue;
    }
    if (want > 0) {
      int64_t seen = 0;
      const uint32_t len1 = d.rlen[r1], len2 = d.rlen[r2];
      bool found = cm_pair_dir(d, 0, cm_d_pos(d, r1, 0), cm_d_err(d, r1, 0), d.ndp[r1], cm_d_pos(d, r2, 1), cm_d_err(d, r2, 1),
                               d.ndn[r2], len1, len2, pe, want, pe.min_sum, &seen);
      if (!found)
        found = cm_pair_dir(d, 1, cm_d_pos(d, r1, 1), cm_d_err(d, r1, 1), d.ndn[r1], cm_d_pos(d, r2, 0), cm_d_err(d, r2, 0),
                            d.ndp[r2], len1, len2, pe, want, pe.min_sum, &seen);
      if (!found) { d.stats[CM_ST_ERR] = 2; return; }
    } else {
      pe.f_dir = d.pe_first[pair]; pe.f_i1 = d.pe_i1[pair]; pe.f_i2 = d.pe_i2[pair];
    }
    cm_emit_record<SAM>(d, pair, pe, t);
  }
}

#endif
```

### chromap_amd/csrc/cm_types.h

```cpp
#ifndef CM_TYPES_H_
#define CM_TYPES_H_

#include <stdint.h>

#if defined(__HIPCC__)
#include <hip/hip_runtime.h>
#define CM_HD __host__ __device__ __forceinline__
#define CM_D __device__ __forceinline__
#else
#define CM_HD inline
#define CM_D inline
#endif

#define CM_EMPTY_KEY 0xFFFFFFFFFFFFFFFFull
#define CM_DELETED_KEY 0xFFFFFFFFFFFFFFFEull

#define CM_PR_MISS 0
#define CM_PR_SINGLE 1
#define CM_PR_MULTI 2
#define CM_V_INVALID 0x7fff
#define CM_MM_CHUNKS 8
enum CmList : uint32_t {
  CM_L_HIT_WAVE = 0, CM_L_HIT_B256A = 1, CM_L_HIT_B256B = 2, CM_L_HIT_SLAB = 3, CM_L_HIT_G16 = 4, CM_L_HIT_DECLINED = 5, CM_L_RS_WAVE = 6, CM_L_RS_B256A = 7,
  CM_L_RS_B256B = 8, CM_L_PF_BLOCK = 9, CM_L_HIT_B512 = 10, CM_L_RS_B512 = 11, CM_L_S5_WAVE = 12, CM_L_S6A_WAVE = 13, CM_L_PF_BLOCK_BIG = 14, CM_L_RS_SLAB = 15,
  CM_L_HIT_SERIAL = 16, CM_L_S6C_WAVE = 17, CM_L_S6A_BLOCK = 18, CM_L_PF_HUGE = 19, CM_L_S6C_BLOCK = 20, CM_L_HIT_WAVE_SMALL = 21, CM_L_S5_BLOCK = 22,
  CM_L_SEARCH_WAVE = 23, CM_L_HIT_B1024 = 25, CM_L_RS_B1024 = 26, CM_L_PF_WAVE = 27, CM_L_S5_SMALL = 28, CM_L_S6A_SMALL = 29, CM_L_S6C_SMALL = 30,
  CM_L_SEARCH_WAVE_BIG = 31
};
#define CM_HV_LISTS 32
#define CM_RS_SEGS 64
#define CM_MAX_BEST 8192
#define CM_SORT_SERIAL_MAX 24
#define CM_SORT_WAVE_MAX 1024

#define CM_SAM_CIGAR_CAP 64
#define CM_GOFF_GAP 2048u
#define CM_MAX_READ_LEN 1400
struct CmParams {
  int32_t e;
  int32_t min_seeds;
  int32_t f0, f1;
  int32_t max_insert;
  int32_t min_read_len;
  int32_t max_best;
  int32_t drop_rep;
  int32_t trim;
  int32_t split;
  int32_t single;
  int32_t bc_err;
  int32_t bc_keep;
  double bc_prob;
  int32_t k, w;
  int32_t lanes;
  int32_t ref_batch;
  int32_t grain;
  int32_t pairs_out;
  int32_t sam;
};

struct CmMapqTables {
  const double *len_coef;
  const uint32_t *nsec_break;
  int32_t n_break;
};

struct alignas(16) CmPlRec { uint32_t p0, p1, pn, pc; };
#define CM_PL_LEAD 4

struct CmDev {
  const uint64_t *bkt;
  uint32_t bmask;
  const uint64_t *occ;
  uint32_t n_occ;
  const uint8_t *ref;
  const uint64_t *ref_off;
  const uint32_t *ref_len;
  uint32_t n_seq;
  const uint32_t *goff;
  const CmPlRec *ref_pl;
  uint64_t ref_pl_words;
  uint32_t *read_pl;
  uint32_t read_pl_w;
  CmParams p;
  CmMapqTables mq;
  uint32_t n_pairs;
  uint32_t first_read_id;
  const uint8_t *rb0, *rb1;
  const uint32_t *ro0, *ro1;
  const uint8_t *bcb, *bcq;
  const uint32_t *bco;
  const uint64_t *wl;
  uint32_t wl_mask;
  double wl_num_sample;
  const double *pow10_tab;
  uint64_t *bc_key;
  uint8_t *bc_ok;
  uint32_t *rlen;
  uint32_t *mm_cnt;
  uint32_t *mm_off;
  uint64_t *mm_hash;
  uint32_t *mm_ps;
  uint64_t *pr_val;
  uint8_t *pr_kind;
  uint32_t *hit_tot;
  uint32_t *hit_off;
  uint8_t *round2;
  uint32_t *rep_cnt;
  uint32_t *rep_len;
  uint64_t *hbuf;
  uint8_t *hcnt;
  uint32_t *n_pos_hit;
  uint32_t *ncp, *ncn;
  const uint32_t *perm_reads, *perm_pairs;
  uint32_t *hv_cnt, *hv_list;
  uint32_t *rs_cnt, *rs_list;
  uint32_t *srt_cnt, *srt_list;
  uint32_t hv_big, rs_max3, rs_big;
  unsigned long long cls_mask;
  uint32_t s4c_pbig;
  uint32_t hv_stride, s3b_cap, hv_max[4];
  uint8_t *coop_slab;
  uint32_t coop_slab_cap;
  uint32_t coop_slab_blocks;
  const unsigned long long *abort;
  uint64_t *rs_pool;
  uint32_t rs_pool_cap;
  uint32_t *rs_pool_off;
  uint32_t wq_dynamic;
  unsigned long long *prof;
  uint32_t mm_cap;
  uint32_t coop_rb;
  uint32_t hv_sub;
  uint32_t hv_mid;
  uint8_t *aug;
  int32_t *res_neg;
  int32_t *res_pos;
  uint32_t *resc_n;
  uint32_t *resc_p;
  uint32_t *m_tot;
  uint32_t *m_off;
  uint64_t *mbuf;
  uint8_t *mcnt;
  uint32_t *mcp, *mcn;
  uint8_t *force0;
  uint64_t *fbuf;
  uint8_t *fcnt;
  uint32_t *fcp, *fcn;
  uint8_t *alive;
  uint64_t *dpos;
  int16_t *derr;
  uint32_t *dsplit;
  uint32_t *ndp, *ndn;
  uint32_t *nv;
  uint32_t *v_off;
  int16_t *v_err;
  int16_t *v_end;
  int32_t *min_err, *second_err, *n_best, *n_second;
  int32_t *pe_min, *pe_second, *pe_nbest, *pe_nsecond;
  uint32_t *pe_first;
  uint32_t *pe_i1, *pe_i2;
  uint32_t *pe_choice;
  uint8_t *rec;
  uint8_t *rec_ok;
  const uint32_t *rid_rank;
  const uint32_t *pairs_rank;
  uint8_t *sam_rec;
  uint32_t *sam_cigar;
  uint8_t *sam_md;
  uint32_t *sam_z;
  uint32_t sam_md_cap;
  unsigned long long *stats;
};

#define CM_ST_CAND 0
#define CM_ST_MAPPINGS 1
#define CM_ST_MAPPED 2
#define CM_ST_UNIQ 3
#define CM_ST_MINIMIZERS 4
#define CM_ST_PROBE_STEPS 5
#define CM_ST_PROBE_HITS 6
#define CM_ST_OCC 7
#define CM_ST_RESCUED 8
#define CM_ST_MULTI 9
#define CM_ST_ERR 10
#define CM_ST_RECORDS 11
#define CM_ST_BC_INWL 12
#define CM_ST_BC_CORR 13
#define CM_ST_TOTAL 14
#define CM_ST_ABORT 15
#define CM_ST_POOL 16
#define CM_ST_N 17

#endif
```

Measured before the change: 539.9.

## Specialize stage kernels for paired-end mode and compact multi-hit pairs into list

```diff
diff --git a/chromap_amd/csrc/cm_api.hip b/chromap_amd/csrc/cm_api.hip
--- a/chromap_amd/csrc/cm_api.hip
+++ b/chromap_amd/csrc/cm_api.hip
@@ -124,6 +124,8 @@
     c->opt.coop_rb = (int)value;
   } else if (n == "coop") {
     c->opt.coop = (int)value;
+  } else if (n == "generic_kernels") {
+    c->opt.generic_kernels = value ? 1 : 0;
   } else if (n == "item_limit") {
     c->opt.item_limit = value > 0 ? (uint64_t)value : 0xfffffff0ull;
   } else {
@@ -146,6 +148,7 @@
   else if (n == "item_limit") *value = (int64_t)c->opt.item_limit;
   else if (n == "lanes") *value = c->opt.lanes;
   else if (n == "coop") *value = c->opt.coop;
+  else if (n == "generic_kernels") *value = c->opt.generic_kernels;
   else if (n.rfind("coop_profile_", 0) == 0) {
     const int k = atoi(n.c_str() + 13);
     unsigned long long v = 0;
@@ -746,6 +749,7 @@
   d.abort = (const unsigned long long *)c->stats.p + CM_ST_ABORT;
   d.coop_rb = c->opt.coop_rb > 0 ? (uint32_t)c->opt.coop_rb : 0u;
   d.wq_dynamic = ((uint32_t)c->opt.coop >> 16) & 1u;
+  d.generic_kernels = c->opt.generic_kernels ? 1u : 0u;
   if (c->has_rank) {
     d.rid_rank = (const uint32_t *)c->rid_rank.p;
     d.ref_off = (const uint64_t *)c->ref_off_r.p;
diff --git a/chromap_amd/csrc/cm_ctx.h b/chromap_amd/csrc/cm_ctx.h
--- a/chromap_amd/csrc/cm_ctx.h
+++ b/chromap_amd/csrc/cm_ctx.h
@@ -123,6 +123,7 @@
   int heavy_max[3] = {0, 0, 0};
   int heavy_last = 0;
   int spec = 1;
+  int generic_kernels = 0;
   int coop_rb = 0;
   int coop = 0xff;
 };
diff --git a/chromap_amd/csrc/cm_kernels.hip b/chromap_amd/csrc/cm_kernels.hip
--- a/chromap_amd/csrc/cm_kernels.hip
+++ b/chromap_amd/csrc/cm_kernels.hip
@@ -657,13 +657,14 @@
   const uint32_t o = r ^ 1u;
   return coop && (d.ncp[o] >= CM_RS_WAVE || d.ncn[o] >= CM_RS_WAVE);
 }
+template <class M>
 __global__ __launch_bounds__(CM_BLOCK) void k_s4a_rescue_count(CmDev d, uint32_t n, uint32_t seg_cap, uint32_t coop) {
   __shared__ uint32_t sh_cnt, sh_base;
   if (threadIdx.x == 0) sh_cnt = 0;
   __syncthreads();
   const uint32_t i0 = blockIdx.x * CM_BLOCK + threadIdx.x;
   const uint32_t i = i0 < n && d.perm_reads ? d.perm_reads[i0] : i0;
-  const bool aug0 = i0 < n && cm_s4a_decide(d, i);
+  const bool aug0 = i0 < n && cm_s4a_decide<M>(d, i);
   const bool wv = aug0 && cm_rescue_is_wave(d, i, coop);
   cm_wave_append(d.hv_list + (size_t)CM_L_SEARCH_WAVE * d.hv_stride, d.hv_cnt + CM_L_SEARCH_WAVE, wv, i);
   const bool aug = aug0 && !wv;
@@ -936,11 +937,12 @@
 #define CM_S5C_P_SMALL 512u
 #define CM_S5C_P_WAVE 2048u
 #define CM_S5C_P_BLOCK 16384u
+template <class M = CmModeAny>
 __device__ __forceinline__ void cm_s4c_queue_sort(const CmDev &d, uint32_t pair, bool live, uint32_t coop) {
   for (uint32_t q = 0; q < 4; ++q) {
     const uint32_t r = 2 * pair + (q >> 1);
     uint32_t cnt = live ? ((q & 1u) ? d.fcn[r] : d.fcp[r]) : 0u;
-    if ((coop & 8u) && !d.p.split && live && d.fcp[r] + d.fcn[r] > CM_S5C_COOP_MIN) cnt = 0;
+    if ((coop & 8u) && !M::split(d) && live && d.fcp[r] + d.fcn[r] > CM_S5C_COOP_MIN) cnt = 0;
     cm_wave_append(d.srt_list, &d.srt_cnt[0], cnt > CM_SORT_SERIAL_MAX && cnt <= CM_SORT_WAVE_MAX, (r << 1) | (q & 1u));
   }
 }
@@ -948,12 +950,13 @@
 #define CM_S4C_P_WAVE 1024u
 #define CM_S4C_P_BLOCK 4096u
 #define CM_S4C_P_BIG 15360u
+template <class M>
 __global__ __launch_bounds__(CM_BLOCK) void k_s4c_reduce(CmDev d, uint32_t n, uint32_t coop) {
   if (d.abort && *d.abort) return;
   const uint32_t i = blockIdx.x * CM_BLOCK + threadIdx.x;
   const uint32_t pair = i < n ? (d.perm_pairs ? d.perm_pairs[i] : i) : 0u;
   uint32_t cls = 0;
-  if (i < n && cm_s4c_pre(d, pair)) {
+  if (i < n && cm_s4c_pre<M>(d, pair)) {
     const uint32_t r1 = 2 * pair, r2 = r1 + 1;
     uint32_t big = d.mcp[r1] > d.mcn[r1] ? d.mcp[r1] : d.mcn[r1];
     big = d.mcp[r2] > big ? d.mcp[r2] : big;
@@ -968,7 +971,7 @@
     cm_wave_append(d.hv_list + CM_L_PF_HUGE * (size_t)d.hv_stride, d.hv_cnt + CM_L_PF_HUGE, cls == CM_L_PF_HUGE, pair);
   }
   if (!d.perm_pairs) return;
-  cm_s4c_queue_sort(d, pair, i < n && !cls && d.alive[pair], coop);
+  cm_s4c_queue_sort<M>(d, pair, i < n && !cls && d.alive[pair], coop);
 }
 template <int G, bool STAGED>
 __global__ __launch_bounds__(G < CM_BLOCK ? CM_BLOCK : G) void k_s4c_coop(CmDev d, uint32_t P, uint32_t lid, uint32_t coop) {
@@ -998,11 +1001,12 @@
     }
   }
 }
+template <class M>
 __global__ __launch_bounds__(CM_BLOCK) void k_s5a_prepare(CmDev d, uint32_t n, uint32_t coop) {
   if (d.abort && *d.abort) return;
   const uint32_t i = blockIdx.x * CM_BLOCK + threadIdx.x;
   const uint32_t r = i < n ? (d.perm_reads ? d.perm_reads[i] : i) : 0u;
-  const bool to_wave = i < n && cm_s5a_prepare(d, r, coop ? CM_S5C_COOP_MIN : 0u);
+  const bool to_wave = i < n && cm_s5a_prepare<M>(d, r, coop ? CM_S5C_COOP_MIN : 0u);
   const bool big = to_wave && (d.fcp[r] > CM_S5C_P_WAVE || d.fcn[r] > CM_S5C_P_WAVE);
   const bool small = to_wave && d.fcp[r] <= CM_S5C_P_SMALL && d.fcn[r] <= CM_S5C_P_SMALL;
   if (coop) {
@@ -1011,13 +1015,14 @@
     cm_wave_append(d.hv_list + (size_t)CM_L_S5_BLOCK * d.hv_stride, d.hv_cnt + CM_L_S5_BLOCK, big, r);
   }
 }
+template <class M>
 __global__ __launch_bounds__(CM_BLOCK) void k_s5c_finalize(CmDev d, uint32_t n, uint32_t coop) {
   if (d.abort && *d.abort) return;
   const uint32_t i = blockIdx.x * CM_BLOCK + threadIdx.x;
   const uint32_t r = i < n ? (d.perm_reads ? d.perm_reads[i] : i) : 0u;
   const uint32_t cmin = coop ? CM_S5C_COOP_MIN : 0u;
   if (i < n) cm_s5c_finalize(d, r, cmin);
-  if (!d.perm_reads || d.p.split || d.p.single) return;
+  if (!d.perm_reads || M::split(d) || M::single(d)) return;
   const bool live = i < n && !(cmin && d.nv[r] > cmin) && d.alive[r >> 1];
   const uint32_t a = live ? d.ndp[r] : 0u, b = live ? d.ndn[r] : 0u;
   cm_wave_append(d.srt_list, &d.srt_cnt[0], a > CM_SORT_SERIAL_MAX && a <= CM_SORT_WAVE_MAX, r << 1);
@@ -1137,15 +1142,18 @@
   if (big <= CM_S6A_COOP_MIN) return 0;
   return big2 <= CM_S6A_P_SMALL ? small_list : big2 <= CM_S6A_P_WAVE ? wave_list : block_list;
 }
+template <class M>
 __global__ __launch_bounds__(CM_BLOCK) void k_s6a_pair(CmDev d, uint32_t n, uint32_t coop) {
   if (d.abort && *d.abort) return;
   const uint32_t i = blockIdx.x * CM_BLOCK + threadIdx.x;
   const uint32_t pair = i < n ? (d.perm_pairs ? d.perm_pairs[i] : i) : 0u;
   uint32_t cls = 0;
-  if (i < n && cm_s6a_pre<false>(d, pair)) {
+  bool multi = false;
+  if (i < n && cm_s6a_pre<false, M>(d, pair)) {
     cls = coop ? cm_s6_class(d, pair, CM_L_S6A_SMALL, CM_L_S6A_WAVE, CM_L_S6A_BLOCK) : 0u;
-    if (!cls) cm_s6a_sweeps<false>(d, pair);
-  }
+    multi = cls != 0 || cm_s6a_sweeps<false>(d, pair) > 1;
+  }
+  if constexpr (M::kPe) cm_wave_append(d.hv_list + (size_t)CM_L_S6C_MULTI * d.hv_stride, d.hv_cnt + CM_L_S6C_MULTI, multi, pair);
   if (coop) {
     cm_wave_append(d.hv_list + (size_t)CM_L_S6A_SMALL * d.hv_stride, d.hv_cnt + CM_L_S6A_SMALL, cls == CM_L_S6A_SMALL, pair);
     cm_wave_append(d.hv_list + (size_t)CM_L_S6A_WAVE * d.hv_stride, d.hv_cnt + CM_L_S6A_WAVE, cls == CM_L_S6A_WAVE, pair);
@@ -1166,19 +1174,31 @@
   g.xw = reinterpret_cast<uint32_t *>(base + gb - CM_XW_BYTES);
   for (uint32_t j = blockIdx.x * gpb + grp; j < n_list; j += gridDim.x * gpb) cm_coop_s6a<false>(d, list[j], g, m);
 }
-__global__ __launch_bounds__(CM_BLOCK) void k_s6c_multi(CmDev d, uint32_t n, uint32_t coop) {
-  if (d.abort && *d.abort) return;
-  const uint32_t i = blockIdx.x * CM_BLOCK + threadIdx.x;
-  const uint32_t pair = i < n ? (d.perm_pairs ? d.perm_pairs[i] : i) : 0u;
+template <class M>
+__device__ __forceinline__ void cm_s6c_item(const CmDev &d, bool mine, uint32_t pair, uint32_t coop) {
   uint32_t cls = 0;
-  if (i < n) {
-    if (coop && !d.p.single && !d.p.split && d.pe_nbest[pair] > 1) cls = cm_s6_class(d, pair, CM_L_S6C_SMALL, CM_L_S6C_WAVE, CM_L_S6C_BLOCK);
-    if (!cls) cm_s6c_multi<false>(d, pair);
+  if (mine) {
+    if (coop && !M::single(d) && !M::split(d) && d.pe_nbest[pair] > 1) cls = cm_s6_class(d, pair, CM_L_S6C_SMALL, CM_L_S6C_WAVE, CM_L_S6C_BLOCK);
+    if (!cls) cm_s6c_multi<false, M>(d, pair);
   }
   if (coop) {
     cm_wave_append(d.hv_list + (size_t)CM_L_S6C_SMALL * d.hv_stride, d.hv_cnt + CM_L_S6C_SMALL, cls == CM_L_S6C_SMALL, pair);
     cm_wave_append(d.hv_list + (size_t)CM_L_S6C_WAVE * d.hv_stride, d.hv_cnt + CM_L_S6C_WAVE, cls == CM_L_S6C_WAVE, pair);
     cm_wave_append(d.hv_list + (size_t)CM_L_S6C_BLOCK * d.hv_stride, d.hv_cnt + CM_L_S6C_BLOCK, cls == CM_L_S6C_BLOCK, pair);
+  }
+}
+__global__ __launch_bounds__(CM_BLOCK) void k_s6c_multi(CmDev d, uint32_t n, uint32_t coop) {
+  if (d.abort && *d.abort) return;
+  const uint32_t i = blockIdx.x * CM_BLOCK + threadIdx.x;
+  cm_s6c_item<CmModeAny>(d, i < n, i < n ? (d.perm_pairs ? d.perm_pairs[i] : i) : 0u, coop);
+}
+__global__ __launch_bounds__(CM_BLOCK) void k_s6c_list(CmDev d, uint32_t coop) {
+  if (d.abort && *d.abort) return;
+  const uint32_t cnt = d.hv_cnt[CM_L_S6C_MULTI];
+  const uint32_t *list = d.hv_list + (size_t)CM_L_S6C_MULTI * d.hv_stride;
+  for (uint32_t j0 = blockIdx.x * CM_BLOCK; j0 < cnt; j0 += gridDim.x * CM_BLOCK) {
+    const uint32_t j = j0 + threadIdx.x;
+    cm_s6c_item<CmModePe>(d, j < cnt, j < cnt ? list[j] : 0u, coop);
   }
 }
 template <int G>
@@ -1703,8 +1723,10 @@
   hipLaunchKernelGGL(k_s3b_candidates, dim3((n + threads - 1) / threads), dim3(threads), (size_t)cap * threads * 9, s, d, n, cap);
 }
 uint32_t cm_rescue_seg_cap(uint32_t n_reads) { return ((n_reads + CM_BLOCK - 1) / CM_BLOCK / CM_RS_SEGS + 1) * CM_BLOCK; }
+static inline bool cm_mode_pe(const CmDev &d) { return !d.p.split && !d.p.single && !d.generic_kernels; }
+#define CM_LAUNCH_MODE(kname, ...) do { if (cm_mode_pe(d)) hipLaunchKernelGGL(kname<CmModePe>, __VA_ARGS__); else hipLaunchKernelGGL(kname<CmModeAny>, __VA_ARGS__); } while (0)
 void cm_launch_k_s4a_rescue_count(const CmDev &d, uint32_t n, hipStream_t s, bool coop) {
-  if (n) hipLaunchKernelGGL(k_s4a_rescue_count, grid_for(n), dim3(CM_BLOCK), 0, s, d, n, cm_rescue_seg_cap(n), coop ? 1u : 0u);
+  if (n) CM_LAUNCH_MODE(k_s4a_rescue_count, grid_for(n), dim3(CM_BLOCK), 0, s, d, n, cm_rescue_seg_cap(n), coop ? 1u : 0u);
 }
 static inline uint32_t rescue_wave_blocks(uint32_t n_reads) {
   uint32_t b = n_reads / 512 + 64;
@@ -1778,7 +1800,7 @@
   if (!cm_lds_optin(&k_s4c_coop<CM_BLOCK, true>, gbk)) coop &= ~4u;
   CmDev d2 = d;
   d2.s4c_pbig = pbig > CM_S4C_P_BLOCK ? pbig : 0;
-  hipLaunchKernelGGL(k_s4c_reduce, grid_for(n), dim3(CM_BLOCK), 0, s, d2, n, coop);
+  CM_LAUNCH_MODE(k_s4c_reduce, grid_for(n), dim3(CM_BLOCK), 0, s, d2, n, coop);
   if (!(coop & 4u)) return;
   uint32_t blocks = n / 2048 + 64;
   if (blocks > 4096) blocks = 4096;
@@ -1791,7 +1813,7 @@
 }
 void cm_launch_k_s5a_prepare(const CmDev &d, uint32_t n, hipStream_t s, bool coop) {
   if (!n) return;
-  hipLaunchKernelGGL(k_s5a_prepare, grid_for(n), dim3(CM_BLOCK), 0, s, d, n, coop ? 1u : 0u);
+  CM_LAUNCH_MODE(k_s5a_prepare, grid_for(n), dim3(CM_BLOCK), 0, s, d, n, coop ? 1u : 0u);
   if (coop) {
     if (cm_cls_on(d, CM_L_S5_SMALL)) hipLaunchKernelGGL(k_s5_sort_coop, dim3(4096), dim3(CM_BLOCK), 0, s, d, CM_L_S5_SMALL);
     if (cm_cls_on(d, CM_L_S5_WAVE)) hipLaunchKernelGGL(k_s5_sort_coop, dim3(2048), dim3(CM_BLOCK), 0, s, d, CM_L_S5_WAVE);
@@ -1800,7 +1822,7 @@
 }
 void cm_launch_k_s5c_finalize(const CmDev &d, uint32_t n, hipStream_t s, bool coop) {
   if (!n) return;
-  hipLaunchKernelGGL(k_s5c_finalize, grid_for(n), dim3(CM_BLOCK), 0, s, d, n, coop ? 1u : 0u);
+  CM_LAUNCH_MODE(k_s5c_finalize, grid_for(n), dim3(CM_BLOCK), 0, s, d, n, coop ? 1u : 0u);
   if (!coop) return;
   auto gbytes = [](uint32_t P) {
     const size_t b1 = cm_coop_ver_mem_bytes(P), b2 = cm_coop_sort_mem_bytes(CM_S5C_SORT_P, CM_S5C_SORT_RB);
@@ -1827,7 +1849,7 @@
   if (!n) return;
   const size_t lw = (CM_BLOCK / 64) * cm_s6_group_bytes(CM_S6A_P_WAVE), lb = cm_s6_group_bytes(CM_S6A_P_BLOCK);
   if (coop && !(cm_lds_optin(&k_s6a_coop<64>, lw) && cm_lds_optin(&k_s6a_coop<CM_BLOCK>, lb))) coop = false;
-  hipLaunchKernelGGL(k_s6a_pair, grid_for(n), dim3(CM_BLOCK), 0, s, d, n, coop ? 1u : 0u);
+  CM_LAUNCH_MODE(k_s6a_pair, grid_for(n), dim3(CM_BLOCK), 0, s, d, n, coop ? 1u : 0u);
   if (!coop) return;
   uint32_t blocks = n / 4096 + 64;
   if (blocks > 2048) blocks = 2048;
@@ -1839,10 +1861,11 @@
   if (!n) return;
   const size_t lw = (CM_BLOCK / 64) * cm_s6_group_bytes(CM_S6A_P_WAVE), lb = cm_s6_group_bytes(CM_S6A_P_BLOCK);
   if (coop && !(cm_lds_optin(&k_s6c_coop<64>, lw) && cm_lds_optin(&k_s6c_coop<CM_BLOCK>, lb))) coop = false;
-  hipLaunchKernelGGL(k_s6c_multi, grid_for(n), dim3(CM_BLOCK), 0, s, d, n, coop ? 1u : 0u);
-  if (!coop) return;
   uint32_t blocks = n / 4096 + 64;
   if (blocks > 2048) blocks = 2048;
+  if (!cm_mode_pe(d)) hipLaunchKernelGGL(k_s6c_multi, grid_for(n), dim3(CM_BLOCK), 0, s, d, n, coop ? 1u : 0u);
+  else if (cm_cls_on(d, CM_L_S6C_MULTI)) hipLaunchKernelGGL(k_s6c_list, dim3(blocks), dim3(CM_BLOCK), 0, s, d, coop ? 1u : 0u);
+  if (!coop) return;
   if (cm_cls_on(d, CM_L_S6C_SMALL)) hipLaunchKernelGGL(k_s6c_coop<64>, dim3(blocks), dim3(CM_BLOCK), (CM_BLOCK / 64) * cm_s6_group_bytes(CM_S6A_P_SMALL), s, d, CM_S6A_P_SMALL, CM_L_S6C_SMALL);
   if (cm_cls_on(d, CM_L_S6C_WAVE)) hipLaunchKernelGGL(k_s6c_coop<64>, dim3(blocks), dim3(CM_BLOCK), lw, s, d, CM_S6A_P_WAVE, CM_L_S6C_WAVE);
   if (cm_cls_on(d, CM_L_S6C_BLOCK)) hipLaunchKernelGGL(k_s6c_coop<CM_BLOCK>, dim3(256), dim3(CM_BLOCK), lb, s, d, CM_S6A_P_BLOCK, CM_L_S6C_BLOCK);
diff --git a/chromap_amd/csrc/cm_stages.h b/chromap_amd/csrc/cm_stages.h
--- a/chromap_amd/csrc/cm_stages.h
+++ b/chromap_amd/csrc/cm_stages.h
@@ -2,6 +2,17 @@
 #define CM_STAGES_H_
 
 #include "cm_types.h"
+
+struct CmModeAny {
+  static constexpr bool kPe = false;
+  static CM_HD bool split(const CmDev &d) { return d.p.split != 0; }
+  static CM_HD bool single(const CmDev &d) { return d.p.single != 0; }
+};
+struct CmModePe {
+  static constexpr bool kPe = true;
+  static CM_HD bool split(const CmDev &) { return false; }
+  static CM_HD bool single(const CmDev &) { return false; }
+};
 
 CM_HD uint32_t cm_c2u(uint8_t c) {
   const uint32_t u = c & 0xDFu;
@@ -1241,15 +1252,16 @@
 CM_HD const uint64_t *cm_c0_neg(const CmDev &d, uint32_t r) { return d.hbuf + d.hit_off[r] + d.n_pos_hit[r]; }
 CM_HD const uint8_t *cm_c0_ncnt(const CmDev &d, uint32_t r) { return d.hcnt + d.hit_off[r] + d.n_pos_hit[r]; }
 
+template <class M = CmModeAny>
 CM_HD bool cm_s4a_decide(const CmDev &d, uint32_t r) {
   const uint32_t pair = r >> 1;
   d.aug[r] = 0; d.res_neg[r] = 0; d.res_pos[r] = 0; d.resc_n[r] = 0; d.resc_p[r] = 0;
-  const bool live = d.p.single ? ((r & 1) == 0 && d.mm_cnt[r] > 0) : (d.mm_cnt[2 * pair] > 0 && d.mm_cnt[2 * pair + 1] > 0);
+  const bool live = M::single(d) ? ((r & 1) == 0 && d.mm_cnt[r] > 0) : (d.mm_cnt[2 * pair] > 0 && d.mm_cnt[2 * pair + 1] > 0);
   const uint32_t ncp = d.ncp[r], ncn = d.ncn[r];
   d.m_tot[r] = live ? ncp + ncn : 0;
   if (!live) return false;
   const uint32_t mm_count = d.mm_cnt[r];
-  bool augment = !d.p.split && !d.p.single;
+  bool augment = !M::split(d) && !M::single(d);
   const uint8_t *pc = cm_c0_pcnt(d, r), *nc = cm_c0_ncnt(d, r);
   for (uint32_t i = 0; augment && i < ncp; ++i) if (pc[i] >= mm_count / 2) { augment = false; break; }
   if (augment) for (uint32_t i = 0; i < ncn; ++i) if (nc[i] >= mm_count / 2) { augment = false; break; }
@@ -1414,12 +1426,13 @@
   for (uint32_t i = 0; i < d.fcn[r]; ++i) fn[i] = (fn[i] & 0xffffffffull) | ((uint64_t)d.rid_rank[(uint32_t)(fn[i] >> 32)] << 32);
 }
 
+template <class M = CmModeAny>
 CM_HD bool cm_s4c_pre(const CmDev &d, uint32_t pair) {
   const uint32_t r1 = 2 * pair, r2 = r1 + 1;
   d.fcp[r1] = d.fcn[r1] = d.fcp[r2] = d.fcn[r2] = 0;
   d.alive[pair] = 0;
   d.force0[pair] = 0;
-  if (d.p.single) {
+  if (M::single(d)) {
     if (d.mm_cnt[r1] == 0 || d.mcp[r1] + d.mcn[r1] == 0) return false;
     const uint64_t *mp = cm_m_pos(d, r1), *mn = cm_m_neg(d, r1);
     const uint8_t *mpc = cm_m_pcnt(d, r1), *mnc = cm_m_ncnt(d, r1);
@@ -1442,7 +1455,7 @@
   d.force0[pair] = (uint8_t)ret;
   const uint32_t nc1 = d.mcp[r1] + d.mcn[r1], nc2 = d.mcp[r2] + d.mcn[r2];
   if (!(nc1 > 0 && nc2 > 0)) return false;
-  if (d.p.split) {
+  if (M::split(d)) {
     for (uint32_t r = r1; r <= r2; ++r) {
       const uint64_t *mp = cm_m_pos(d, r), *mn = cm_m_neg(d, r);
       const uint8_t *mpc = cm_m_pcnt(d, r), *mnc = cm_m_ncnt(d, r);
@@ -1474,8 +1487,9 @@
   d.alive[pair] = (f1 > 0 && f2 > 0) ? 1 : 0;
   if (d.alive[pair]) { cm_rerank(d, r1); cm_rerank(d, r2); }
 }
+template <class M = CmModeAny>
 CM_HD void cm_s4c_reduce(const CmDev &d, uint32_t pair) {
-  if (!cm_s4c_pre(d, pair)) return;
+  if (!cm_s4c_pre<M>(d, pair)) return;
   cm_s4c_filter(d, pair);
   cm_s4c_post(d, pair);
 }
@@ -2050,13 +2064,14 @@
   return cm_banded_align(e, d.ref + d.ref_off[rid] + position - e, read, (int)L, strand == 1, 0, (int)L, end_pos);
 }
 
+template <bool PRE = false>
 CM_HD bool cm_verify_one(const CmDev &d, const uint8_t *read, uint32_t L, int strand, uint64_t cpos, CmBest &bst,
                          uint64_t *dp, int16_t *de, uint32_t *nd, const int16_t *pre_err, const int16_t *pre_end,
                          uint32_t ci) {
   const int e = d.p.e;
   int end_pos = (int)L;
   int ne;
-  if (pre_err) { ne = pre_err[ci]; end_pos = pre_end[ci]; }
+  if (PRE || pre_err) { ne = pre_err[ci]; end_pos = pre_end[ci]; }
   else ne = cm_verify_compute(d, read, L, strand, cpos, &end_pos);
   if (ne <= e) {
     cm_update_best(bst, ne);
@@ -2069,6 +2084,7 @@
   return false;
 }
 
+template <bool PRE = false>
 CM_HD uint32_t cm_draft_strand(const CmDev &d, const uint8_t *read, uint32_t L, int strand, const uint64_t *cp,
                                const uint8_t *cc, uint32_t nc, CmBest &bst, uint64_t *dp, int16_t *de,
                                const int16_t *pre_err = nullptr, const int16_t *pre_end = nullptr) {
@@ -2080,12 +2096,10 @@
       uint32_t position = (uint32_t)cp[ci];
       if (strand == 1) position = position - L + 1;
       if (!cm_valid_candidate(d, rid, position, L)) continue;
-      cm_verify_one(d, read, L, strand, cp[ci], bst, dp, de, &nd, pre_err, pre_end, ci);
+      cm_verify_one<PRE>(d, read, L, strand, cp[ci], bst, dp, de, &nd, pre_err, pre_end, ci);
     }
     return nd;
   }
-  uint64_t vpos[8];
-  uint8_t vcnt[8];
   uint32_t vidx[8];
   uint32_t nvalid = 0, thr = 0, ci = 0;
   while (ci < nc) {
@@ -2094,17 +2108,15 @@
     uint32_t position = (uint32_t)cp[ci];
     if (strand == 1) position = position - L + 1;
     if (!cm_valid_candidate(d, rid, position, L)) { ++ci; continue; }
-    vpos[nvalid] = cp[ci];
-    vcnt[nvalid] = cc[ci];
     vidx[nvalid] = ci;
     ++nvalid;
     ++ci;
     if (nvalid < (uint32_t)lanes) continue;
     for (int mi = 0; mi < lanes; ++mi)
-      if (!cm_verify_one(d, read, L, strand, vpos[mi], bst, dp, de, &nd, pre_err, pre_end, vidx[mi])) thr = vcnt[mi];
+      if (!cm_verify_one<PRE>(d, read, L, strand, cp[vidx[mi]], bst, dp, de, &nd, pre_err, pre_end, vidx[mi])) thr = cc[vidx[mi]];
     nvalid = 0;
   }
-  for (uint32_t i = 0; i < nvalid; ++i) cm_verify_one(d, read, L, strand, vpos[i], bst, dp, de, &nd, pre_err, pre_end, vidx[i]);
+  for (uint32_t i = 0; i < nvalid; ++i) cm_verify_one<PRE>(d, read, L, strand, cp[vidx[i]], bst, dp, de, &nd, pre_err, pre_end, vidx[i]);
   return nd;
 }
 
@@ -2171,6 +2183,7 @@
   return nd;
 }
 
+template <class M = CmModeAny>
 CM_HD void cm_s5_verify(const CmDev &d, uint32_t r) {
   const uint32_t pair = r >> 1;
   d.ndp[r] = 0; d.ndn[r] = 0;
@@ -2185,7 +2198,7 @@
     uint64_t *dpp = d.dpos + d.m_off[r], *dpn = d.dpos + d.m_off[r] + d.ncp[r] + d.resc_p[r];
     int16_t *dep = d.derr + d.m_off[r], *den = d.derr + d.m_off[r] + d.ncp[r] + d.resc_p[r];
     bool done = false;
-    if (d.p.split) {
+    if (M::split(d)) {
       uint32_t *dsp = d.dsplit + d.m_off[r], *dsn = d.dsplit + d.m_off[r] + d.ncp[r] + d.resc_p[r];
       cm_sort_cand(pp, pc, ncp);
       cm_sort_cand(np, nc, ncn);
@@ -2220,12 +2233,22 @@
 }
 
 
+template <class M = CmModeAny>
 CM_HD bool cm_s5a_prepare(const CmDev &d, uint32_t r, uint32_t coop_min = 0) {
   const uint32_t pair = r >> 1;
   d.nv[r] = 0;
-  if (d.p.split || !d.alive[pair]) { cm_s5_verify(d, r); return false; }
+  const int e = d.p.e;
+  if constexpr (M::kPe) {
+    if (!d.alive[pair]) {
+      d.ndp[r] = 0; d.ndn[r] = 0;
+      d.min_err[r] = e + 1; d.second_err[r] = e + 1;
+      d.n_best[r] = 0; d.n_second[r] = 0;
+      return false;
+    }
+  } else {
+    if (M::split(d) || !d.alive[pair]) { cm_s5_verify<M>(d, r); return false; }
+  }
   d.ndp[r] = 0; d.ndn[r] = 0;
-  const int e = d.p.e;
   CmBest bst = {e + 1, e + 1, 0, 0};
   const uint32_t L = d.rlen[r];
   uint64_t *pp = cm_f_pos(d, r), *np = cm_f_neg(d, r);
@@ -2302,8 +2325,8 @@
   const uint32_t L = d.rlen[r];
   const uint8_t *read = cm_read_ptr(d, r);
   const uint32_t op = d.m_off[r], on = d.m_off[r] + d.ncp[r] + d.resc_p[r];
-  d.ndp[r] = cm_draft_strand(d, read, L, 0, d.fbuf + op, d.fcnt + op, d.fcp[r], bst, d.dpos + op, d.derr + op, d.v_err + op, d.v_end + op);
-  d.ndn[r] = cm_draft_strand(d, read, L, 1, d.fbuf + on, d.fcnt + on, d.fcn[r], bst, d.dpos + on, d.derr + on, d.v_err + on, d.v_end + on);
+  d.ndp[r] = cm_draft_strand<true>(d, read, L, 0, d.fbuf + op, d.fcnt + op, d.fcp[r], bst, d.dpos + op, d.derr + op, d.v_err + op, d.v_end + op);
+  d.ndn[r] = cm_draft_strand<true>(d, read, L, 1, d.fbuf + on, d.fcnt + on, d.fcn[r], bst, d.dpos + on, d.derr + on, d.v_err + on, d.v_end + on);
   d.min_err[r] = bst.min_err; d.second_err[r] = bst.second_err;
   d.n_best[r] = bst.n_best; d.n_second[r] = bst.n_second;
 }
@@ -2974,14 +2997,14 @@
   }
 }
 
-template <bool SAM = false>
+template <bool SAM = false, class M = CmModeAny>
 CM_HD bool cm_s6a_pre(const CmDev &d, uint32_t pair) {
   const uint32_t r1 = 2 * pair, r2 = r1 + 1;
   for (uint32_t t = 0; t < (uint32_t)d.p.max_best; ++t) d.rec_ok[(uint64_t)pair * (uint32_t)d.p.max_best + t] = 0;
   d.pe_nbest[pair] = 0;
   if (!d.alive[pair]) return false;
   const uint32_t nd1 = d.ndp[r1] + d.ndn[r1], nd2 = d.ndp[r2] + d.ndn[r2];
-  if (d.p.single) {
+  if (M::single(d)) {
     if (nd1 == 0) return false;
     d.pe_nbest[pair] = d.n_best[r1];
     d.pe_min[pair] = d.min_err[r1]; d.pe_second[pair] = d.second_err[r1]; d.pe_nsecond[pair] = d.n_second[r1];
@@ -2989,7 +3012,7 @@
     return false;
   }
   if (!(nd1 > 0 && nd2 > 0)) return false;
-  if (d.p.split) {
+  if (M::split(d)) {
     CmPe sp;
     cm_split_pairing(d, pair, 0, sp);
     d.pe_min[pair] = sp.min_sum; d.pe_second[pair] = sp.second_sum;
@@ -3001,7 +3024,7 @@
   return true;
 }
 template <bool SAM = false>
-CM_HD void cm_s6a_sweeps(const CmDev &d, uint32_t pair) {
+CM_HD int cm_s6a_sweeps(const CmDev &d, uint32_t pair) {
   const uint32_t r1 = 2 * pair, r2 = r1 + 1;
   for (uint32_t r = r1; r <= r2; ++r) {
     cm_sort_draft(const_cast<uint64_t *>(cm_d_pos(d, r, 0)), const_cast<int16_t *>(cm_d_err(d, r, 0)), d.ndp[r]);
@@ -3020,10 +3043,11 @@
   d.pe_nbest[pair] = pe.n_best; d.pe_nsecond[pair] = pe.n_second;
   d.pe_first[pair] = pe.f_dir; d.pe_i1[pair] = pe.f_i1; d.pe_i2[pair] = pe.f_i2;
   if (pe.n_best == 1) cm_emit_record<SAM>(d, pair, pe);
-}
-template <bool SAM = false>
+  return pe.n_best;
+}
+template <bool SAM = false, class M = CmModeAny>
 CM_HD void cm_s6a_pair(const CmDev &d, uint32_t pair) {
-  if (cm_s6a_pre<SAM>(d, pair)) cm_s6a_sweeps<SAM>(d, pair);
+  if (cm_s6a_pre<SAM, M>(d, pair)) cm_s6a_sweeps<SAM>(d, pair);
 }
 
 struct CmMt { uint32_t mt[624]; int idx; };
@@ -3116,10 +3140,10 @@
   }
 }
 
-template <bool SAM = false>
+template <bool SAM = false, class M = CmModeAny>
 CM_HD void cm_s6c_multi(const CmDev &d, uint32_t pair) {
   const int nb = d.pe_nbest[pair];
-  if (nb <= 1 || (!d.p.single && nb > d.p.drop_rep)) return;
+  if (nb <= 1 || (!M::single(d) && nb > d.p.drop_rep)) return;
   const uint32_t r1 = 2 * pair, r2 = r1 + 1;
   CmPe pe;
   pe.min_sum = d.pe_min[pair]; pe.second_sum = d.pe_second[pair]; pe.n_best = nb; pe.n_second = d.pe_nsecond[pair];
@@ -3128,8 +3152,8 @@
   const uint32_t to_report = (uint32_t)nb < K ? (uint32_t)nb : K;
   for (uint32_t t = 0; t < to_report; ++t) {
     const int64_t want = (int64_t)d.pe_choice[(uint64_t)pair * K + t];
-    if (d.p.single) { cm_emit_single_record<SAM>(d, pair, (uint32_t)want, t); continue; }
-    if (d.p.split) {
+    if (M::single(d)) { cm_emit_single_record<SAM>(d, pair, (uint32_t)want, t); continue; }
+    if (M::split(d)) {
       CmPe sp;
       cm_split_pairing(d, pair, want, sp);
       cm_emit_pairs_record<SAM>(d, pair, sp, t);
diff --git a/chromap_amd/csrc/cm_types.h b/chromap_amd/csrc/cm_types.h
--- a/chromap_amd/csrc/cm_types.h
+++ b/chromap_amd/csrc/cm_types.h
@@ -24,7 +24,7 @@
   CM_L_HIT_WAVE = 0, CM_L_HIT_B256A = 1, CM_L_HIT_B256B = 2, CM_L_HIT_SLAB = 3, CM_L_HIT_G16 = 4, CM_L_HIT_DECLINED = 5, CM_L_RS_WAVE = 6, CM_L_RS_B256A = 7,
   CM_L_RS_B256B = 8, CM_L_PF_BLOCK = 9, CM_L_HIT_B512 = 10, CM_L_RS_B512 = 11, CM_L_S5_WAVE = 12, CM_L_S6A_WAVE = 13, CM_L_PF_BLOCK_BIG = 14, CM_L_RS_SLAB = 15,
   CM_L_HIT_SERIAL = 16, CM_L_S6C_WAVE = 17, CM_L_S6A_BLOCK = 18, CM_L_PF_HUGE = 19, CM_L_S6C_BLOCK = 20, CM_L_HIT_WAVE_SMALL = 21, CM_L_S5_BLOCK = 22,
-  CM_L_SEARCH_WAVE = 23, CM_L_HIT_B1024 = 25, CM_L_RS_B1024 = 26, CM_L_PF_WAVE = 27, CM_L_S5_SMALL = 28, CM_L_S6A_SMALL = 29, CM_L_S6C_SMALL = 30,
+  CM_L_SEARCH_WAVE = 23, CM_L_S6C_MULTI = 24, CM_L_HIT_B1024 = 25, CM_L_RS_B1024 = 26, CM_L_PF_WAVE = 27, CM_L_S5_SMALL = 28, CM_L_S6A_SMALL = 29, CM_L_S6C_SMALL = 30,
   CM_L_SEARCH_WAVE_BIG = 31
 };
 #define CM_HV_LISTS 32
@@ -131,6 +131,7 @@
   uint32_t mm_cap;
   uint32_t coop_rb;
   uint32_t hv_sub;
+  uint32_t generic_kernels;
   uint32_t hv_mid;
   uint8_t *aug;
   int32_t *res_neg;
```

New measurement: 551.2, median of 6. +2.1%, better.
